# cornell-zhang/GraphLily

Measured on AMD Instinct MI355X. Metric: SpMV effective HBM GB/s (fp32 (+,x), orkut stand-in); BFS GTEPS in `bfs`, higher is better.
Workload: dtype f32; 1 GPU; float32 (+,x) SpMV on orkut stand-in (R-MAT seed 6, n=3072512, nnz=211703799), row-sharded x1; graph=orkut, n=3072512, nnz=211703799

## Files before the change

graphlily_amd/capi.py:

```python
import ctypes
import os

import numpy as np

_HERE = os.path.dirname(os.path.abspath(__file__))
LIB_PATH = os.environ.get("GRAPHLILY_HIP_LIB") or os.path.join(_HERE, "lib", "libgraphlily_hip.so")

GL_OP_MULADD, GL_OP_ANDOR, GL_OP_ADDMIN = 0, 1, 2
GL_NOMASK, GL_MASK_WRITETOZERO, GL_MASK_WRITETOONE = 0, 1, 2

GL_OK = 0
GL_ERR_INVALID_ARG = -1
GL_ERR_HIP = -2
GL_ERR_NOT_INITIALIZED = -3
GL_ERR_IO = -4

IDX_VAL = np.dtype([("index", np.uint32), ("val", np.float32)])

EXPORTS = [
    "gl_init", "gl_host_bind_near_device", "gl_device_count", "gl_set_stream", "gl_reset_stream", "gl_sync", "gl_last_error", "gl_version",
    "gl_graph_begin_capture", "gl_graph_end_capture", "gl_graph_launch", "gl_graph_destroy",
    "gl_bfs_bits_begin", "gl_bfs_bits_push_step", "gl_bfs_bits_pull_step",     "gl_bfs_bits_shard_step", "gl_bfs_bits_shard_finish", "gl_dist_all_gather_bits_tally",
    "gl_buf_d2h_async", "gl_levels_pack", "gl_host_levels_unpack", "gl_host_unpack_threads", "gl_buf_d2h_levels", "gl_sync_levels_unpack",
    "gl_levels_stream_bytes", "gl_levels_stream_arm", "gl_levels_pack_stream", "gl_sync_levels_unpack_stream",
# ... 227 lines not shown
    def __array_finalize__(self, obj):
        if obj is not None and getattr(obj, "_owner", None) is not None:
            self._owner = obj._owner



class DeviceBuffer:

    def __init__(self, nbytes=0, ptr=None, keepalive=None):
        self.nbytes = int(nbytes)
        self._owned = ptr is None
        self.keepalive = keepalive
        if self._owned:
            p = ctypes.c_void_p(0)
            check(lib().gl_buf_alloc(ctypes.byref(p), self.nbytes))
            self.ptr = p.value or 0
        else:
            self.ptr = int(ptr)

    @classmethod
    def from_host(cls, arr):
        arr = np.ascontiguousarray(arr)
        b = cls(arr.nbytes)
        b.write(arr)
        return b

    @classmethod
    def from_torch(cls, t):
        return cls(t.numel() * t.element_size(), ptr=t.data_ptr(), keepalive=t)

    def write(self, arr, offset_bytes=0):
        arr = np.ascontiguousarray(arr)
        assert offset_bytes + arr.nbytes <= self.nbytes, "host array larger than device buffer"
        check(lib().gl_buf_h2d(ctypes.c_void_p(self.ptr + offset_bytes), _np_ptr(arr), arr.nbytes))

    def read(self, dtype, count=None, offset_bytes=0, out=None):
        dtype = np.dtype(dtype)
        if count is None:
            count = (self.nbytes - offset_bytes) // dtype.itemsize
        if out is None:
            out = np.empty(count, dtype=dtype)
        else:
            assert out.dtype == dtype and out.shape[0] >= count and out.flags["C_CONTIGUOUS"]
            out = out[:count]
        assert offset_bytes + out.nbytes <= self.nbytes
        check(lib().gl_buf_d2h(_np_ptr(out), ctypes.c_void_p(self.ptr + offset_bytes), out.nbytes))
        return out

    def read_async(self, out, offset_bytes=0):
        assert out.flags["C_CONTIGUOUS"] and offset_bytes + out.nbytes <= self.nbytes
        check(lib().gl_buf_d2h_async(_np_ptr(out), ctypes.c_void_p(self.ptr + offset_bytes), out.nbytes))
        return out

    def free(self):
        if self._owned and self.ptr:
            lib().gl_buf_free(ctypes.c_void_p(self.ptr))
        self.ptr = 0

    def __del__(self):
        try:
            self.free()
        except Exception:
            pass


def copy_d2d(dst, src, nbytes):
    assert nbytes <= dst.nbytes and nbytes <= src.nbytes
    check(lib().gl_buf_d2d(ctypes.c_void_p(dst.ptr), ctypes.c_void_p(src.ptr), int(nbytes)))


def _p(buf):
    return ctypes.c_void_p(buf.ptr if buf is not None else 0)


GL_PAGERANK_MAX_SLOTS = 65536

GL_PLAN_NO_MULADD = 1
GL_PLAN_BOOLEAN = 2
GL_PLAN_KEEP_VALUES = 4
GL_VAL_FLOAT, GL_VAL_UNSIGNED, GL_VAL_UFIXED_32_8 = 0, 1, 2
GL_PLAN_HOST_FORMAT = 8
GL_PLAN_DEVICE_FORMAT = 16
GL_PLAN_REFERENCE_ORDER = 32
PLAN_ARRAYS = {"entries": 0, "bases": 1, "units": 2, "hub_rows": 3, "spans": 4, "hot": 5, "hot_hdr": 6, "present": 7}
GL_ERR_UNSUPPORTED = -5


class _PlanDesc(ctypes.Structure):
    _fields_ = [("nnz", ctypes.c_uint64), ("device_bytes", ctypes.c_uint64), ("groups", ctypes.c_uint64), ("hot_nnz", ctypes.c_uint64),
                ("num_units", ctypes.c_uint32), ("blocks", ctypes.c_uint32), ("segments", ctypes.c_uint32), ("max_block_rows", ctypes.c_uint32),
                ("hot_columns", ctypes.c_uint32), ("packed_columns", ctypes.c_uint32),
                ("layout", ctypes.c_int), ("mix", ctypes.c_int), ("helper", ctypes.c_int)]


class SpMVPlan:
    def __init__(self, num_rows, num_cols, indptr, indices, data, row_begin=0, row_end=None, flags=0):
        self.indptr = np.ascontiguousarray(indptr, dtype=np.uint32)
        self.indices = np.ascontiguousarray(indices, dtype=np.uint32)
        self.data = np.ascontiguousarray(data, dtype=np.float32)
        row_end = num_rows if row_end is None else row_end
        h = ctypes.c_void_p(0)
        check(lib().gl_spmv_plan_create_ex(ctypes.byref(h), num_rows, num_cols, _np_ptr(self.indptr),
                                           _np_ptr(self.indices), _np_ptr(self.data), row_begin, row_end,
                                           int(flags)))
        self.flags = int(flags)
        self.handle = h.value
        self.num_rows, self.num_cols, self.row_begin, self.row_end = num_rows, num_cols, row_begin, row_end
        self.indptr = self.indices = self.data = None

    def info(self):
        cached = getattr(self, "_info", None)
        if cached is not None:
            return dict(cached)
        d = _PlanDesc()
        check(lib().gl_spmv_plan_describe(ctypes.c_void_p(self.handle), ctypes.byref(d)))
        finite = ctypes.c_int(0)
        check(lib().gl_spmv_plan_values_finite(ctypes.c_void_p(self.handle), ctypes.byref(finite)))
        self._info = {"finite_values": bool(finite.value), "helper": ("gather", "spread", "self-hot", "none")[d.helper], "packed_columns": d.packed_columns,
                      "nnz": d.nnz, "device_bytes": d.device_bytes, "num_units": d.num_units, "blocks": d.blocks,
                      "segments": d.segments, "max_block_rows": d.max_block_rows, "groups": d.groups,
                      "hot_columns": d.hot_columns, "hot_nnz": d.hot_nnz, "mix": d.mix,
                      "layout": ("general", "pattern", "boolean", "reference-order")[d.layout]}
        return dict(self._info)

    def run(self, x, mask, y, op, zero, mask_type):
        check(lib().gl_spmv_run(ctypes.c_void_p(self.handle), _p(x), _p(mask), _p(y), int(op), float(zero),
                                int(mask_type)))

    def run_typed(self, x, mask, y, op, zero_bits, mask_type, val_type):
        check(lib().gl_spmv_run_typed(ctypes.c_void_p(self.handle), _p(x), _p(mask), _p(y), int(op), int(zero_bits), int(mask_type),
                                      int(val_type)))

    def chain(self, on):
        active = ctypes.c_int(0)
        check(lib().gl_spmv_plan_chain(ctypes.c_void_p(self.handle), 1 if on else 0, ctypes.byref(active)))
        return bool(active.value)

    def export(self, name):
        n = ctypes.c_size_t(0)
        check(lib().gl_spmv_plan_export(ctypes.c_void_p(self.handle), PLAN_ARRAYS[name], None, 0, ctypes.byref(n)))
        out = np.empty(n.value // 4, dtype=np.uint32)
        check(lib().gl_spmv_plan_export(ctypes.c_void_p(self.handle), PLAN_ARRAYS[name], _np_ptr(out), out.nbytes, ctypes.byref(n)))
        return out

    def bits_words(self):
        v = ctypes.c_uint64(0)
        check(lib().gl_spmv_plan_bits_words(ctypes.c_void_p(self.handle), ctypes.byref(v)))
        return v.value

    def bfs_pull_step(self, bits_in, bits_out, distance, level):
        check(lib().gl_bfs_pull_step(ctypes.c_void_p(self.handle), _p(bits_in), _p(bits_out), _p(distance), float(level)))

    def bfs_parents(self, distance, parent, orphans=None):
        check(lib().gl_bfs_parents(ctypes.c_void_p(self.handle), _p(distance), _p(parent), _p(orphans)))

    def bfs_parents_entries(self, distance, parent):
        v = ctypes.c_uint64(0)
        check(lib().gl_bfs_parents_entries(ctypes.c_void_p(self.handle), _p(distance), _p(parent), ctypes.byref(v)))
        return v.value

    def cc_labels(self, labels, count=None):
        check(lib().gl_cc_labels(ctypes.c_void_p(self.handle), _p(labels), _p(count)))

    def cc_hook(self, parent):
        check(lib().gl_cc_hook(ctypes.c_void_p(self.handle), _p(parent)))

    def tc_count(self, total, per_vertex=None):
# ... 516 lines not shown
```

graphlily_amd/csrc/gl_format.hip:

```cpp
#include <cstring>

#include "gl_spmv_plan.h"

#include <rocprim/rocprim.hpp>

namespace gl {

struct DevCsr {
    uint32_t row_begin = 0, row_end = 0;
    uint64_t nz0 = 0, nnz = 0;
    uint32_t *d_indptr = nullptr;
    uint32_t *d_indices = nullptr;
    uint32_t *d_data = nullptr;
    uint32_t *d_colbits = nullptr;
    uint32_t num_cols_colbits = 0;
};

namespace {

struct DevMem {
    void *p = nullptr;
    ~DevMem() {
        if (p) (void)hipFree(p);
    }
    int alloc(size_t bytes) {
        GL_HIP(hipMalloc(&p, bytes ? bytes : 16));
        return GL_OK;
    }
    template <typename T>
    T *as() const { return static_cast<T *>(p); }
};

constexpr uint32_t kFmtThreads = 256;

inline unsigned wave_grid(uint64_t rows) {
    const uint64_t want = (rows + 3) / 4;
    const uint64_t cap = (uint64_t)ctx().num_cus * 32u;
    return (unsigned)std::max<uint64_t>(1, std::min(want, cap));
}

__global__ __launch_bounds__(kFmtThreads) void fmt_degree_kernel(const uint32_t *__restrict__ indices, uint64_t nnz, uint32_t num_cols,
                                                                 uint32_t *__restrict__ deg, uint32_t *__restrict__ bad) {
    for (uint64_t i = (uint64_t)blockIdx.x * kFmtThreads + threadIdx.x; i < nnz; i += (uint64_t)gridDim.x * kFmtThreads) {
        const uint32_t c = indices[i];
        if (c < num_cols) atomicAdd(&deg[c], 1u);
        else *bad = 1u;
    }
}

__global__ __launch_bounds__(kFmtThreads) void fmt_non_finite_kernel(const uint32_t *__restrict__ data, uint64_t nnz, uint32_t *__restrict__ found) {
    bool any = false;
    for (uint64_t i = (uint64_t)blockIdx.x * kFmtThreads + threadIdx.x; i < nnz; i += (uint64_t)gridDim.x * kFmtThreads)
        any |= (data[i] & 0x7f800000u) == 0x7f800000u;
    if (any) *found = 1u;
}

__global__ __launch_bounds__(kFmtThreads) void fmt_pattern_pass1_kernel(const uint32_t *__restrict__ indptr, const uint32_t *__restrict__ indices,
                                                                        const uint32_t *__restrict__ data, uint32_t row_begin, uint32_t rows,
                                                                        uint64_t nz0, uint32_t num_cols, uint32_t *__restrict__ colbits) {
    const uint32_t lane = threadIdx.x & 63u, nwaves = gridDim.x * (kFmtThreads / 64u);
    for (uint32_t row = blockIdx.x * (kFmtThreads / 64u) + (threadIdx.x >> 6); row < rows; row += nwaves) {
        const uint32_t r = row_begin + row;
        const uint64_t s = indptr[row] - nz0, e = indptr[row + 1] - nz0;
        for (uint64_t i = s + lane; i < e; i += 64u) {
            const uint32_t c = indices[i];
            if (c < num_cols && c != r) {
                const uint32_t bits = data[i];
                if (colbits[c] != bits) colbits[c] = bits;
            }
        }
    }
}

__global__ __launch_bounds__(kFmtThreads) void fmt_pattern_pass2_kernel(const uint32_t *__restrict__ indptr, const uint32_t *__restrict__ indices,
                                                                        const uint32_t *__restrict__ data, uint32_t row_begin, uint32_t rows,
                                                                        uint64_t nz0, uint32_t num_cols, const uint32_t *__restrict__ colbits,
                                                                        uint32_t *__restrict__ diag_has, uint32_t *__restrict__ diag_val,
                                                                        uint32_t *__restrict__ mismatch, unsigned long long *__restrict__ exceptions) {
    const uint32_t lane = threadIdx.x & 63u, nwaves = gridDim.x * (kFmtThreads / 64u);
    for (uint32_t row = blockIdx.x * (kFmtThreads / 64u) + (threadIdx.x >> 6); row < rows; row += nwaves) {
        const uint32_t r = row_begin + row;
        const uint64_t s = indptr[row] - nz0, e = indptr[row + 1] - nz0;
        uint32_t nexc = 0;
        bool bad = false;
        for (uint64_t i = s + lane; i < e; i += 64u) {
            const uint32_t c = indices[i], bits = data[i];
            if (c >= num_cols) { bad = true; continue; }
            if (colbits[c] == bits) continue;
            if (c != r) { bad = true; continue; }
            nexc++;
            diag_val[row] = bits;
            atomicOr(&diag_has[row >> 5], 1u << (row & 31u));
        }
#pragma unroll
        for (int d = 32; d > 0; d >>= 1) nexc += __shfl_down(nexc, d);
        nexc = __shfl(nexc, 0);
        if (nexc > 1u) bad = true;
        if (__ballot(bad) != 0ull && lane == 0) *mismatch = 1u;
        if (nexc && lane == 0) atomicAdd(exceptions, (unsigned long long)nexc);
    }
}

template <typename K>
__global__ __launch_bounds__(kFmtThreads) void fmt_keys_kernel(const uint32_t *__restrict__ indptr, const uint32_t *__restrict__ indices,
                                                               const uint32_t *__restrict__ data, uint32_t row_begin, uint32_t rows, uint64_t nz0,
                                                               uint32_t num_cols, const uint32_t *__restrict__ bstart, uint32_t nblocks,
                                                               const uint32_t *__restrict__ colmap, const uint32_t *__restrict__ colbits,
                                                               uint32_t cb, uint32_t bb, K *__restrict__ keys, uint2 *__restrict__ payload,
                                                               bool drop_hot) {
    const uint32_t lane = threadIdx.x & 63u, nwaves = gridDim.x * (kFmtThreads / 64u);
    const K drop = (K)1 << (bb + cb + 1u);
    for (uint32_t row = blockIdx.x * (kFmtThreads / 64u) + (threadIdx.x >> 6); row < rows; row += nwaves) {
        const uint32_t r = row_begin + row;
        const uint64_t s = indptr[row] - nz0, e = indptr[row + 1] - nz0;
        if (s == e) continue;
        uint32_t lo = 0, hi = nblocks - 1u;
        while (lo < hi) {
            const uint32_t mid = (lo + hi + 1u) >> 1;
            if (bstart[mid] <= r) lo = mid; else hi = mid - 1u;
        }
        const uint32_t b = lo, r0 = bstart[b];
        for (uint64_t i = s + lane; i < e; i += 64u) {
            const uint32_t c = indices[i], v = data[i];
            K key;
            if (c >= num_cols || (colbits && c == r && v != colbits[c])) {
                key = drop;
            } else {
                const uint32_t cm = colmap[c];
                key = ((K)b << (cb + 1u)) | ((K)(cm >> 31) << cb) | (K)(cm & 0x7fffffffu);
                if (drop_hot && (cm >> 31)) key = drop;
            }
            keys[i] = key;
            payload[i] = make_uint2(r - r0, v);
        }
    }
}

template <typename K>
__global__ __launch_bounds__(kFmtThreads) void fmt_bounds_kernel(const K *__restrict__ keys, uint64_t n, uint32_t count, uint32_t cb,
                                                                 unsigned long long *__restrict__ off) {
    const uint32_t i = blockIdx.x * kFmtThreads + threadIdx.x;
    if (i >= count) return;
    const K target = (K)i << cb;
    uint64_t lo = 0, hi = n;
    while (lo < hi) {
        const uint64_t mid = (lo + hi) >> 1;
        if (keys[mid] < target) lo = mid + 1; else hi = mid;
    }
    off[i] = lo;
}

struct UnitDesc {
    uint32_t cold_begin, cold_end, hot_begin, hot_end;
    uint32_t goff, r0, nrows_direct, hub_off;
    uint32_t nhub, seg, hot_e0, present_off;
    uint32_t nhot_groups, pad0, pad1, pad2;
};

template <typename K>
__global__ __launch_bounds__(kFmtThreads) void fmt_gap_kernel(const K *__restrict__ keys, uint64_t n, uint32_t cb, uint32_t bb, uint32_t *__restrict__ dummies) {
    const K cmask = ((K)1 << cb) - 1, drop = (K)1 << (bb + cb + 1u);
    for (uint64_t i = (uint64_t)blockIdx.x * kFmtThreads + threadIdx.x; i < n; i += (uint64_t)gridDim.x * kFmtThreads) {
        uint32_t d = 0u;
        if (i > 0) {
            const K k = keys[i], kp = keys[i - 1];
            if ((k >> cb) == (kp >> cb) && ((k >> cb) & (K)1) == 0 && !(k & drop)) {
                const uint32_t gap = (uint32_t)(k & cmask) - (uint32_t)(kp & cmask);
                if (gap > kColdMaxDelta) d = (gap - 1u) / kColdMaxDelta;
            }
        }
        dummies[i] = d;
    }
}
__global__ __launch_bounds__(kFmtThreads) void fmt_gap_unit_starts_kernel(const UnitDesc *__restrict__ units, uint32_t nunits, uint32_t *__restrict__ dummies) {
    const uint32_t u = blockIdx.x * kFmtThreads + threadIdx.x;
    if (u < nunits && units[u].cold_begin < units[u].cold_end) dummies[units[u].cold_begin] = 0u;
}

template <typename K, bool PATTERN>
__global__ __launch_bounds__(kThreads) void fmt_emit_cold_kernel(const K *__restrict__ keys, const uint2 *__restrict__ payload,
                                                                 const uint32_t *__restrict__ ahead, const UnitDesc *__restrict__ units,
                                                                 const uint32_t *__restrict__ hub_rows, uint32_t cb,
                                                                 unsigned char *__restrict__ cold, uint32_t *__restrict__ bases,
                                                                 uint4 *__restrict__ plan_units) {
    __shared__ uint8_t hub_of[kMaxBlockRows + 1];
    constexpr uint32_t G = PATTERN ? kColdGroupsPattern : kColdGroupsGeneral;
    constexpr uint32_t EB = PATTERN ? kColdElemBytesPattern : kColdElemBytesGeneral;
    const UnitDesc u = units[blockIdx.x];
    const uint32_t nrows = u.nrows_direct & 0xffffu;
    const K cmask = ((K)1 << cb) - 1;
    if (u.nhub) {
        for (uint32_t i = threadIdx.x; i < nrows; i += kThreads) hub_of[i] = 0xffu;
        __syncthreads();
        if (threadIdx.x < u.nhub) hub_of[hub_rows[u.hub_off + threadIdx.x]] = (uint8_t)threadIdx.x;
        __syncthreads();
    }
    const uint32_t pad0 = nrows + kHubSlots * u.nhub;
    auto put = [&](uint32_t q, uint32_t idx, uint32_t delta, uint32_t slot, uint32_t val) {
        const uint32_t g = u.goff + q / 64u, lane = q % 64u, k = g % G;
        unsigned char *el = cold + (size_t)(g / G) * EB;
        if (!lane) {
            bases[g] = idx;
            delta = 0u;
        }
        if (PATTERN) {
            reinterpret_cast<uint16_t *>(el)[lane * 8u + k] = (uint16_t)slot;
            el[1024u + lane * 8u + k] = (unsigned char)delta;
        } else {
            reinterpret_cast<uint16_t *>(el)[lane * 4u + k] = (uint16_t)slot;
            el[512u + lane * 4u + k] = (unsigned char)delta;
            reinterpret_cast<uint32_t *>(el + 768u)[lane * 4u + k] = val;
        }
    };
    const uint32_t m = u.cold_end - u.cold_begin;
    const uint32_t a0 = m ? ahead[u.cold_begin] : 0u;
    for (uint32_t j = threadIdx.x; j < m; j += kThreads) {
        const uint32_t i = u.cold_begin + j;
        const uint32_t idx = (uint32_t)(keys[i] & cmask);
        const uint32_t before = ahead[i] - a0;
        const uint32_t mine = j ? ahead[i] - ahead[i - 1u] : 0u;
        const uint32_t prev = j ? (uint32_t)(keys[i - 1u] & cmask) : idx;
        const uint32_t q = j + before;
        for (uint32_t t = 1; t <= mine; t++) {
            const uint32_t qd = q - mine + (t - 1u);
            put(qd, prev + kColdMaxDelta * t, kColdMaxDelta, pad0 + qd % 64u, 0u);
        }
        const uint2 pl = payload[i];
        uint32_t slot = pl.x;
        if (u.nhub) {
            const uint32_t hb = hub_of[pl.x];
            if (hb != 0xffu) slot = nrows + kHubSlots * hb + ((q % 64u) & (kHubSlots - 1u));
        }
        put(q, idx, idx - (prev + kColdMaxDelta * mine), slot, pl.y);
    }
    const uint32_t total = m ? m + (ahead[u.cold_end - 1u] - a0) : 0u;
    const uint32_t qend = (total + 64u * G - 1u) / (64u * G) * (64u * G);
    const uint32_t last = m ? (uint32_t)(keys[u.cold_end - 1u] & cmask) : 0u;
    for (uint32_t q = total + threadIdx.x; q < qend; q += kThreads)
        put(q, (q / 64u == (total - 1u) / 64u && total) ? last : 0u, 0u, pad0 + q % 64u, 0u);
    if (threadIdx.x == 0) {
        plan_units[3u * blockIdx.x] = make_uint4(u.goff, qend / 64u, u.r0, u.nrows_direct);
        plan_units[3u * blockIdx.x + 1u] = make_uint4(u.hub_off, u.nhub, u.nhot_groups, u.seg);
    }
}

template <typename K>
__global__ __launch_bounds__(kFmtThreads) void fmt_run_flags_kernel(const K *__restrict__ keys, uint64_t n, uint32_t cb, uint32_t *__restrict__ flags) {
    for (uint64_t i = (uint64_t)blockIdx.x * kFmtThreads + threadIdx.x; i < n; i += (uint64_t)gridDim.x * kFmtThreads) {
        const K k = keys[i];
        flags[i] = (((k >> cb) & (K)1) != 0 && (i == 0 || keys[i - 1] != k)) ? 1u : 0u;
    }
}
__global__ __launch_bounds__(kFmtThreads) void fmt_run_unit_starts_kernel(const UnitDesc *__restrict__ units, uint32_t nunits, uint32_t *__restrict__ flags) {
    const uint32_t u = blockIdx.x * kFmtThreads + threadIdx.x;
    if (u < nunits && units[u].hot_begin < units[u].hot_end) flags[units[u].hot_begin] = 1u;
}

template <typename K>
__global__ __launch_bounds__(kThreads) void fmt_emit_hot_kernel(const K *__restrict__ keys, const uint2 *__restrict__ payload,
                                                                const uint32_t *__restrict__ runs, const UnitDesc *__restrict__ units,
                                                                const uint32_t *__restrict__ hub_rows, uint32_t cb,
                                                                unsigned char *__restrict__ hot, uint32_t *__restrict__ hot_hdr,
                                                                uint16_t *__restrict__ present, uint4 *__restrict__ plan_units) {
    __shared__ uint8_t hub_of[kMaxBlockRows + 1];
    constexpr uint32_t HG = kHotGroupsGeneral;
    constexpr uint32_t EB = kHotElemBytesGeneral;
    const UnitDesc u = units[blockIdx.x];
    const uint32_t nrows = u.nrows_direct & 0xffffu;
    const uint32_t lane = threadIdx.x & 63u, wave = threadIdx.x >> 6;
    const K cmask = ((K)1 << cb) - 1;
    if (u.nhub) {
        for (uint32_t i = threadIdx.x; i < nrows; i += kThreads) hub_of[i] = 0xffu;
        __syncthreads();
        if (threadIdx.x < u.nhub) hub_of[hub_rows[u.hub_off + threadIdx.x]] = (uint8_t)threadIdx.x;
        __syncthreads();
    }
    const uint32_t m = u.hot_end - u.hot_begin, nraw = (m + 63u) / 64u;
    const uint32_t s0 = m ? runs[u.hot_begin] : 0u;
    const uint32_t pad_slot = nrows + kHubSlots * u.nhub + lane;
    for (uint32_t hg = wave; hg < u.nhot_groups; hg += kWaves) {
        const uint32_t st = u.hot_begin + hg * 64u, cnt = hg < nraw ? min(64u, u.hot_end - st) : 0u;
        const size_t e = (size_t)u.hot_e0 + hg / HG;
        const uint32_t k = hg % HG;
        uint32_t local = 0u;
        bool start = false;
        if (lane >= cnt) {
            reinterpret_cast<uint16_t *>(hot + e * EB)[lane * 4u + k] = (uint16_t)pad_slot;
        } else {
            const uint32_t i = st + lane, si = runs[i];
            local = si - s0;
            start = i == u.hot_begin || runs[i - 1u] != si;
            const uint32_t slot_col = (uint32_t)(keys[i] & cmask);
            if (start) present[u.present_off + local] = (uint16_t)slot_col;
            const uint2 pl = payload[i];
            uint32_t slot = pl.x;
            if (u.nhub) {
                const uint32_t hb = hub_of[pl.x];
                if (hb != 0xffu) slot = nrows + kHubSlots * hb + (lane & (kHubSlots - 1u));
            }
            unsigned char *el = hot + e * EB;
            reinterpret_cast<uint16_t *>(el)[lane * 4u + k] = (uint16_t)slot;
            reinterpret_cast<uint32_t *>(el + 512)[lane * 4u + k] = pl.y;
        }
        const unsigned long long mask = __ballot(start && lane >= 1u) >> 1;
        const uint32_t base = __shfl(local, 0);
        if (lane == 0) {
            uint32_t *hd = hot_hdr + e * (kHotHdrWordsPerGroup * HG);
            hd[2u * k] = (uint32_t)mask;
            hd[2u * k + 1u] = (uint32_t)(mask >> 32);
            hd[2u * HG + k] = base;
        }
    }
    if (threadIdx.x == 0)
        plan_units[3u * blockIdx.x + 2u] = make_uint4(u.hot_e0, u.present_off, m ? runs[u.hot_end - 1u] - s0 + 1u : 0u, 0u);
}

__global__ __launch_bounds__(kFmtThreads) void fmt_hot_row_counts_kernel(const uint32_t *__restrict__ indptr, const uint32_t *__restrict__ indices,
                                                                         const uint32_t *__restrict__ data, uint32_t row_begin, uint32_t rows,
                                                                         uint64_t nz0, uint32_t num_cols, const uint32_t *__restrict__ colmap,
                                                                         const uint32_t *__restrict__ colbits, unsigned long long *__restrict__ counts) {
    const uint32_t lane = threadIdx.x & 63u, nwaves = gridDim.x * (kFmtThreads / 64u);
    for (uint32_t row = blockIdx.x * (kFmtThreads / 64u) + (threadIdx.x >> 6); row < rows; row += nwaves) {
        const uint32_t r = row_begin + row;
        const uint64_t s = indptr[row] - nz0, e = indptr[row + 1] - nz0;
        uint32_t h = 0;
        for (uint64_t i = s + lane; i < e; i += 64u) {
            const uint32_t c = indices[i];
            if (c >= num_cols || (colbits && c == r && data[i] != colbits[c])) continue;
            h += colmap[c] >> 31;
        }
#pragma unroll
        for (int d = 32; d > 0; d >>= 1) h += __shfl_xor(h, d);
        if (lane == 0) counts[row] = ((unsigned long long)h << 32) | (unsigned long long)((h + kHotRecEntries - 1u) / kHotRecEntries);
    }
}
__global__ __launch_bounds__(kFmtThreads) void fmt_hot_block_starts_kernel(const unsigned long long *__restrict__ incl, const uint32_t *__restrict__ bstart,
                                                                           uint32_t nblocks, uint32_t row_begin, unsigned long long *__restrict__ out) {
    const uint32_t b = blockIdx.x * kFmtThreads + threadIdx.x;
    if (b > nblocks) return;
    const uint32_t row = bstart[b] - row_begin;
    out[b] = row ? incl[row - 1u] : 0ull;
}
__global__ __launch_bounds__(kThreads) void fmt_fill_hot_rows_kernel(const UnitDesc *__restrict__ units, unsigned char *__restrict__ hot, uint32_t nhot_table,
                                                                     uint4 *__restrict__ plan_units) {
    const UnitDesc u = units[blockIdx.x];
    const uint32_t nrows = u.nrows_direct & 0xffffu, pad0 = nrows + kHubSlots * u.nhub;
    const uint32_t ident = nhot_table | (nhot_table << 16);
    for (uint32_t i = threadIdx.x; i < u.nhot_groups * 64u; i += kThreads) {
        uint4 rec = make_uint4(ident, ident, ident, (nhot_table & 0xffffu) | ((pad0 + (i & 63u)) << 16));
        reinterpret_cast<uint4 *>(hot + (size_t)u.hot_e0 * kHotElemBytesRows)[i] = rec;
    }
    if (threadIdx.x == 0) plan_units[3u * blockIdx.x + 2u] = make_uint4(u.hot_e0, 0u, nhot_table, 0u);
}
__global__ __launch_bounds__(kFmtThreads) void fmt_emit_hot_rows_kernel(const uint32_t *__restrict__ indptr, const uint32_t *__restrict__ indices,
                                                                        const uint32_t *__restrict__ data, uint32_t row_begin, uint32_t rows,
                                                                        uint64_t nz0, uint32_t num_cols, const uint32_t *__restrict__ colmap,
                                                                        const uint32_t *__restrict__ colbits, const uint32_t *__restrict__ bstart,
                                                                        uint32_t nblocks, const unsigned long long *__restrict__ incl,
                                                                        const unsigned long long *__restrict__ block_start,
                                                                        const uint32_t *__restrict__ seg, const uint32_t *__restrict__ unit_of,
                                                                        const UnitDesc *__restrict__ units, const uint32_t *__restrict__ hub_rows,
                                                                        unsigned char *__restrict__ hot) {
    const uint32_t lane = threadIdx.x & 63u, nwaves = gridDim.x * (kFmtThreads / 64u);
    for (uint32_t row = blockIdx.x * (kFmtThreads / 64u) + (threadIdx.x >> 6); row < rows; row += nwaves) {
        const uint32_t r = row_begin + row;
        const uint64_t s = indptr[row] - nz0, e = indptr[row + 1] - nz0;
        const unsigned long long before = row ? incl[row - 1u] : 0ull, mine = incl[row] - before;
        if ((uint32_t)(mine >> 32) == 0u) continue;
        uint32_t lo = 0, hi = nblocks - 1u;
        while (lo < hi) {
            const uint32_t mid = (lo + hi + 1u) >> 1;
            if (bstart[mid] <= r) lo = mid; else hi = mid - 1u;
        }
        const uint32_t b = lo, row_local = r - bstart[b];
        const uint64_t M = (uint32_t)block_start[b + 1u] - (uint32_t)block_start[b];
        const uint64_t rec0 = (uint32_t)before - (uint32_t)block_start[b];
        const uint32_t S = seg[b];
        const UnitDesc u0 = units[unit_of[b]];
        const uint32_t nrows = u0.nrows_direct & 0xffffu;
        int hub = -1;
        for (uint32_t k = 0; k < u0.nhub; k++)
            if (hub_rows[u0.hub_off + k] == row_local) hub = (int)k;
        uint32_t running = 0;
        for (uint64_t i0 = s; i0 < e; i0 += 64u) {
            const uint64_t i = i0 + lane;
            uint32_t cm = 0;
            bool is_hot = false;
            if (i < e) {
                const uint32_t c = indices[i];
                if (c < num_cols && !(colbits && c == r && data[i] != colbits[c])) {
                    cm = colmap[c];
                    is_hot = (cm >> 31) != 0u;
                }
            }
            const unsigned long long bal = __ballot(is_hot);
            const uint32_t rank = running + (uint32_t)__popcll(bal & ((1ull << lane) - 1ull));
            running += (uint32_t)__popcll(bal);
            if (!is_hot) continue;
            const uint64_t j = rec0 + rank / kHotRecEntries;
            const uint32_t f = rank % kHotRecEntries;
            uint64_t guess = S == 1u ? 0u : (j * S + S - 1u) / M;
            uint32_t sg = (uint32_t)(guess < S ? guess : S - 1u);
            while (M * sg / S > j) sg--;
            while (M * (sg + 1u) / S <= j) sg++;
            const UnitDesc u = units[unit_of[(size_t)sg * nblocks + b]];
            const uint32_t jj = (uint32_t)(j - M * sg / S), chunk = u.nhot_groups, l = jj / chunk, el = jj % chunk;
            uint16_t *rec = reinterpret_cast<uint16_t *>(hot + (size_t)(u.hot_e0 + el) * kHotElemBytesRows) + l * 8u;
            rec[f] = (uint16_t)(cm & 0x7fffffffu);
            if (f == 0u) rec[7] = (uint16_t)(hub < 0 ? row_local : nrows + kHubSlots * (uint32_t)hub + (l & (kHubSlots - 1u)));
        }
    }
}

__global__ void fmt_fill_hot_kernel(uint32_t *hot, size_t elems, uint32_t words_per_elem, uint32_t slot_words) {
    for (size_t i = (size_t)blockIdx.x * 256u + threadIdx.x; i < elems * words_per_elem; i += (size_t)gridDim.x * 256u)
        hot[i] = (i % words_per_elem) < slot_words ? (kRowPad | (kRowPad << 16)) : 0u;
}

__global__ void fmt_fill_u32_kernel(uint32_t *dst, uint32_t v, size_t n) {
    for (size_t i = (size_t)blockIdx.x * 256u + threadIdx.x; i < n; i += (size_t)gridDim.x * 256u) dst[i] = v;
}

template <typename K>
int sort_pairs(K *kin, K *kout, uint2 *vin, uint2 *vout, uint64_t n, uint32_t bits, hipStream_t s) {
    size_t tmp_bytes = 0;
    GL_HIP(rocprim::radix_sort_pairs(nullptr, tmp_bytes, kin, kout, vin, vout, (size_t)n, 0u, bits, s));
    DevMem tmp;
    int rc = tmp.alloc(tmp_bytes);
    if (rc != GL_OK) return rc;
    GL_HIP(rocprim::radix_sort_pairs(tmp.p, tmp_bytes, kin, kout, vin, vout, (size_t)n, 0u, bits, s));
    GL_HIP(hipStreamSynchronize(s));
    return GL_OK;
}

template <typename K>
int sort_keys_values_u32(K *kin, K *kout, uint32_t *vin, uint32_t *vout, uint64_t n, uint32_t bits, hipStream_t s) {
    size_t tmp_bytes = 0;
    GL_HIP(rocprim::radix_sort_pairs(nullptr, tmp_bytes, kin, kout, vin, vout, (size_t)n, 0u, bits, s));
    DevMem tmp;
    int rc = tmp.alloc(tmp_bytes);
    if (rc != GL_OK) return rc;
    GL_HIP(rocprim::radix_sort_pairs(tmp.p, tmp_bytes, kin, kout, vin, vout, (size_t)n, 0u, bits, s));
    GL_HIP(hipStreamSynchronize(s));
    return GL_OK;
}

inline uint32_t bits_for(uint64_t count) {
    uint32_t b = 1;
    while ((1ull << b) < count) b++;
    return b;
}

template <typename K>
int emit_general_typed(DevCsr *c, const EmitGeneral &e, gl_spmv_plan p, std::vector<uint32_t> &hub_count, uint64_t *hot_nnz,
                       uint32_t cb, uint32_t bb) {
    hipStream_t s = ctx().stream;
    const BlockPlan &bp = *e.bp;
    const uint32_t nblocks = bp.nblocks, nunits = bp.nunits;
    const uint32_t rows = c->row_end - c->row_begin;
    const uint64_t nnz = c->nnz;
    const bool hot_rows = e.pattern;
    const uint32_t hot_groups = hot_rows ? 1u : kHotGroupsGeneral;
    const uint32_t hot_elem_bytes = hot_rows ? kHotElemBytesRows : kHotElemBytesGeneral;

    DevMem d_bstart, d_colmap, d_keys, d_keys2, d_pl, d_pl2, d_off;
    int rc;
    if ((rc = d_bstart.alloc((size_t)(nblocks + 1) * 4u)) != GL_OK || (rc = d_colmap.alloc((size_t)e.num_cols * 4u)) != GL_OK ||
        (rc = d_keys.alloc(nnz * sizeof(K))) != GL_OK || (rc = d_keys2.alloc(nnz * sizeof(K))) != GL_OK ||
        (rc = d_pl.alloc(nnz * 8u)) != GL_OK || (rc = d_pl2.alloc(nnz * 8u)) != GL_OK ||
        (rc = d_off.alloc((size_t)(2u * nblocks + 1u) * 8u)) != GL_OK)
        return rc;
    GL_HIP(hipMemcpyAsync(d_bstart.p, bp.bstart.data(), (size_t)(nblocks + 1) * 4u, hipMemcpyHostToDevice, s));
    GL_HIP(hipMemcpyAsync(d_colmap.p, e.colmap, (size_t)e.num_cols * 4u, hipMemcpyHostToDevice, s));
    fmt_keys_kernel<K><<<wave_grid(rows), kFmtThreads, 0, s>>>(c->d_indptr, c->d_indices, c->d_data, c->row_begin, rows, c->nz0, e.num_cols,
                                                               d_bstart.as<uint32_t>(), nblocks, d_colmap.as<uint32_t>(),
                                                               e.diag_mode ? c->d_colbits : nullptr, cb, bb, d_keys.as<K>(), d_pl.as<uint2>(), hot_rows);
    GL_LAUNCH_CHECK();
    if ((rc = sort_pairs<K>(d_keys.as<K>(), d_keys2.as<K>(), d_pl.as<uint2>(), d_pl2.as<uint2>(), nnz, bb + cb + 2u, s)) != GL_OK) return rc;
    (void)hipFree(d_keys.p); d_keys.p = nullptr;
    (void)hipFree(d_pl.p); d_pl.p = nullptr;
    const K *keys = d_keys2.as<K>();
    const uint2 *payload = d_pl2.as<uint2>();
    fmt_bounds_kernel<K><<<cdiv(2u * nblocks + 1u, kFmtThreads), kFmtThreads, 0, s>>>(keys, nnz, 2u * nblocks + 1u, cb, d_off.as<unsigned long long>());
    GL_LAUNCH_CHECK();
    std::vector<unsigned long long> off(2u * nblocks + 1u);
    GL_HIP(hipMemcpyAsync(off.data(), d_off.p, off.size() * 8u, hipMemcpyDeviceToHost, s));
    GL_HIP(hipStreamSynchronize(s));

    std::vector<uint32_t> hub_rows((size_t)nblocks * kMaxHubRows, 0u);
    hub_count.assign(nblocks, 0u);
    std::vector<UnitDesc> units(nunits);
    uint64_t hn = 0;
    std::vector<uint64_t> mcs(nblocks), mhs(nblocks), mrec(nblocks, 0);
    for (uint32_t b = 0; b < nblocks; b++) mcs[b] = off[2 * b + 1] - off[2 * b], mhs[b] = off[2 * b + 2] - off[2 * b + 1];
    DevMem d_rowcnt, d_rowincl, d_blockstart;
    if (hot_rows) {
        DevMem d_tmp;
        if ((rc = d_rowcnt.alloc((size_t)std::max(rows, 1u) * 8u)) != GL_OK || (rc = d_rowincl.alloc((size_t)std::max(rows, 1u) * 8u)) != GL_OK ||
            (rc = d_blockstart.alloc((size_t)(nblocks + 1u) * 8u)) != GL_OK)
            return rc;
        fmt_hot_row_counts_kernel<<<wave_grid(rows), kFmtThreads, 0, s>>>(c->d_indptr, c->d_indices, c->d_data, c->row_begin, rows, c->nz0, e.num_cols,
                                                                           d_colmap.as<uint32_t>(), e.diag_mode ? c->d_colbits : nullptr,
                                                                           d_rowcnt.as<unsigned long long>());
        GL_LAUNCH_CHECK();
        size_t tmp_bytes = 0;
        GL_HIP(rocprim::inclusive_scan(nullptr, tmp_bytes, d_rowcnt.as<unsigned long long>(), d_rowincl.as<unsigned long long>(), (size_t)rows,
                                       rocprim::plus<unsigned long long>(), s));
        if ((rc = d_tmp.alloc(tmp_bytes)) != GL_OK) return rc;
        GL_HIP(rocprim::inclusive_scan(d_tmp.p, tmp_bytes, d_rowcnt.as<unsigned long long>(), d_rowincl.as<unsigned long long>(), (size_t)rows,
                                       rocprim::plus<unsigned long long>(), s));
        fmt_hot_block_starts_kernel<<<cdiv(nblocks + 1u, kFmtThreads), kFmtThreads, 0, s>>>(d_rowincl.as<unsigned long long>(), d_bstart.as<uint32_t>(), nblocks,
                                                                                            c->row_begin, d_blockstart.as<unsigned long long>());
        GL_LAUNCH_CHECK();
        std::vector<unsigned long long> bs(nblocks + 1u);
        GL_HIP(hipMemcpyAsync(bs.data(), d_blockstart.p, bs.size() * 8u, hipMemcpyDeviceToHost, s));
        GL_HIP(hipStreamSynchronize(s));
        for (uint32_t b = 0; b < nblocks; b++) {
            mhs[b] = (bs[b + 1] >> 32) - (bs[b] >> 32);
            mrec[b] = (uint64_t)((uint32_t)bs[b + 1] - (uint32_t)bs[b]);
        }
    }
    const UnitLayout ul = layout_units(bp, mcs, mhs, e.dummy_max, hot_groups, e.nhot_table, hot_rows ? &mrec : nullptr);
    const uint64_t total_groups = ul.cold_goff[nunits], hot_elems = ul.hot_e0[nunits];
    if (total_groups >= 0xffffffffull || hot_elems >= 0xffffffffull || ul.present_off[nunits] >= 0xffffffffull)
        return set_error(GL_ERR_UNSUPPORTED, "plan creation: more than 2^32 - 1 groups in a shard");
    for (uint32_t b = 0; b < nblocks; b++) {
        const uint32_t r0 = bp.bstart[b], r1 = bp.bstart[b + 1];
        const uint64_t mc = mcs[b], mh = mhs[b], m = mc + mh;
        hn += mh;
        const uint64_t thr = std::max<uint64_t>(256, m / (uint64_t)e.hub_div);
        uint32_t nh = 0;
        for (uint32_t r = r0; r < r1 && nh < kMaxHubRows; r++) {
            uint64_t cnt = (uint64_t)e.h_indptr[r + 1] - e.h_indptr[r];
            if (cnt < thr) continue;
            if (e.diag_mode) {
                const uint32_t lr = r - c->row_begin;
                if ((e.diag_has[lr >> 5] >> (lr & 31u)) & 1u) cnt--;
            }
            if (cnt >= thr) hub_rows[(size_t)b * kMaxHubRows + nh++] = r - r0;
        }
        hub_count[b] = nh;
        const uint32_t S = bp.seg[b];
        for (uint32_t sg = 0; sg < S; sg++) {
            UnitDesc &u = units[bp.unit_of[sg][b]];
            u.cold_begin = (uint32_t)(off[2 * b] + mc * sg / S);
            u.cold_end = (uint32_t)(off[2 * b] + mc * (sg + 1) / S);
            u.hot_begin = hot_rows ? 0u : (uint32_t)(off[2 * b + 1] + mh * sg / S);
            u.hot_end = hot_rows ? 0u : (uint32_t)(off[2 * b + 1] + mh * (sg + 1) / S);
            const size_t ui = bp.unit_of[sg][b];
            u.goff = (uint32_t)ul.cold_goff[ui];
            u.r0 = r0;
            u.nrows_direct = (r1 - r0) | (bp.all_direct ? 0x80000000u : 0u);
            u.hub_off = (uint32_t)((size_t)b * kMaxHubRows);
            u.nhub = nh;
            u.seg = sg;
            u.hot_e0 = (uint32_t)ul.hot_e0[ui];
            u.present_off = (uint32_t)ul.present_off[ui];
            u.nhot_groups = (uint32_t)(ul.hot_e0[ui + 1] - ul.hot_e0[ui]) * hot_groups;
            u.pad0 = u.pad1 = u.pad2 = 0u;
        }
    }
    *hot_nnz = hn;

    const uint32_t cold_groups = e.pattern ? kColdGroupsPattern : kColdGroupsGeneral;
    const size_t cold_elem_bytes = e.pattern ? kColdElemBytesPattern : kColdElemBytesGeneral;
    const size_t entry_bytes = (size_t)(total_groups / cold_groups) * cold_elem_bytes;
    const size_t tail_bytes = cold_elem_bytes;
    const size_t n_bases = (size_t)total_groups + 8u;
    GL_HIP(hipMalloc((void **)&p->d_entries, entry_bytes + tail_bytes));
    GL_HIP(hipMalloc((void **)&p->d_bases, n_bases * 4u));
    GL_HIP(hipMalloc((void **)&p->d_units, (size_t)nunits * 3u * sizeof(uint4) + 16u));
    GL_HIP(hipMalloc((void **)&p->d_hub_rows, hub_rows.size() * 4u + 16u));
    const size_t hot_bytes = (size_t)(hot_elems + 1u) * hot_elem_bytes;
    const size_t hdr_bytes = hot_rows ? (size_t)32 : (size_t)(hot_elems + 1u) * kHotHdrWordsPerGroup * hot_groups * 4u;
    const size_t present_bytes = (size_t)std::max<uint64_t>(ul.present_off[nunits], 2u) * 2u;
    GL_HIP(hipMalloc((void **)&p->d_hot, hot_bytes));
    GL_HIP(hipMalloc((void **)&p->d_hot_hdr, hdr_bytes));
    GL_HIP(hipMalloc((void **)&p->d_present, present_bytes));
    p->device_bytes += entry_bytes + tail_bytes + n_bases * 4u + (size_t)nunits * 3u * sizeof(uint4) + hub_rows.size() * 4u +
                       hot_bytes + hdr_bytes + present_bytes;
    p->b_entries = entry_bytes + tail_bytes;
    p->b_bases = n_bases * 4u;
    p->b_units = (size_t)nunits * 3u * sizeof(uint4);
    p->b_hub_rows = hub_rows.size() * 4u;
    p->b_hot = hot_bytes;
    p->b_hot_hdr = hdr_bytes;
    p->b_present = present_bytes;
    p->ngroups = total_groups;
    p->nhot_elems = hot_elems;
    GL_HIP(hipMemsetAsync(p->d_hot_hdr, 0, hdr_bytes, s));
    GL_HIP(hipMemsetAsync(p->d_present, 0, present_bytes, s));
    GL_HIP(hipMemsetAsync(p->d_hot, 0, hot_bytes, s));
    fmt_fill_hot_kernel<<<1, 256, 0, s>>>(reinterpret_cast<uint32_t *>(p->d_hot + (size_t)hot_elems * hot_elem_bytes), 1u, hot_elem_bytes / 4u,
                                          hot_rows ? hot_elem_bytes / 4u : hot_groups * 64u * 2u / 4u);
    GL_LAUNCH_CHECK();
    GL_HIP(hipMemsetAsync(p->d_entries, 0, entry_bytes + tail_bytes, s));
    GL_HIP(hipMemsetAsync(p->d_bases, 0, n_bases * 4u, s));
    GL_HIP(hipMemcpyAsync(p->d_hub_rows, hub_rows.data(), hub_rows.size() * 4u, hipMemcpyHostToDevice, s));

    DevMem d_units;
    if ((rc = d_units.alloc((size_t)nunits * sizeof(UnitDesc))) != GL_OK) return rc;
    GL_HIP(hipMemcpyAsync(d_units.p, units.data(), (size_t)nunits * sizeof(UnitDesc), hipMemcpyHostToDevice, s));
    {
        DevMem d_gap, d_ahead, d_tmp;
        if ((rc = d_gap.alloc(std::max<uint64_t>(nnz, 1u) * 4u)) != GL_OK || (rc = d_ahead.alloc(std::max<uint64_t>(nnz, 1u) * 4u)) != GL_OK) return rc;
        fmt_gap_kernel<K><<<std::min<unsigned>(cdiv(std::max<uint64_t>(nnz, 1u), kFmtThreads), (unsigned)ctx().num_cus * 32u), kFmtThreads, 0, s>>>(
            keys, nnz, cb, bb, d_gap.as<uint32_t>());
        GL_LAUNCH_CHECK();
        fmt_gap_unit_starts_kernel<<<cdiv(nunits, kFmtThreads), kFmtThreads, 0, s>>>(d_units.as<UnitDesc>(), nunits, d_gap.as<uint32_t>());
        GL_LAUNCH_CHECK();
        size_t tmp_bytes = 0;
        GL_HIP(rocprim::inclusive_scan(nullptr, tmp_bytes, d_gap.as<uint32_t>(), d_ahead.as<uint32_t>(), (size_t)nnz, rocprim::plus<uint32_t>(), s));
        if ((rc = d_tmp.alloc(tmp_bytes)) != GL_OK) return rc;
        GL_HIP(rocprim::inclusive_scan(d_tmp.p, tmp_bytes, d_gap.as<uint32_t>(), d_ahead.as<uint32_t>(), (size_t)nnz, rocprim::plus<uint32_t>(), s));
        if (e.pattern)
            fmt_emit_cold_kernel<K, true><<<nunits, kThreads, 0, s>>>(keys, payload, d_ahead.as<uint32_t>(), d_units.as<UnitDesc>(), p->d_hub_rows, cb,
                                                                      reinterpret_cast<unsigned char *>(p->d_entries), p->d_bases, p->d_units);
        else
            fmt_emit_cold_kernel<K, false><<<nunits, kThreads, 0, s>>>(keys, payload, d_ahead.as<uint32_t>(), d_units.as<UnitDesc>(), p->d_hub_rows, cb,
                                                                       reinterpret_cast<unsigned char *>(p->d_entries), p->d_bases, p->d_units);
        GL_LAUNCH_CHECK();
        GL_HIP(hipStreamSynchronize(s));
    }
    if (hot_rows) {
        DevMem d_seg, d_unit_of;
        std::vector<uint32_t> unit_of_flat((size_t)bp.Smax * nblocks, 0xffffffffu);
        for (uint32_t sgm = 0; sgm < bp.Smax; sgm++)
            for (uint32_t b = 0; b < nblocks; b++) unit_of_flat[(size_t)sgm * nblocks + b] = bp.unit_of[sgm][b];
        if ((rc = d_seg.alloc((size_t)nblocks * 4u)) != GL_OK || (rc = d_unit_of.alloc(unit_of_flat.size() * 4u)) != GL_OK) return rc;
        GL_HIP(hipMemcpyAsync(d_seg.p, bp.seg.data(), (size_t)nblocks * 4u, hipMemcpyHostToDevice, s));
        GL_HIP(hipMemcpyAsync(d_unit_of.p, unit_of_flat.data(), unit_of_flat.size() * 4u, hipMemcpyHostToDevice, s));
        fmt_fill_hot_rows_kernel<<<nunits, kThreads, 0, s>>>(d_units.as<UnitDesc>(), p->d_hot, e.nhot_table, p->d_units);
        GL_LAUNCH_CHECK();
        if (e.nhot_table) {
            fmt_emit_hot_rows_kernel<<<wave_grid(rows), kFmtThreads, 0, s>>>(c->d_indptr, c->d_indices, c->d_data, c->row_begin, rows, c->nz0, e.num_cols,
                                                                              d_colmap.as<uint32_t>(), e.diag_mode ? c->d_colbits : nullptr,
                                                                              d_bstart.as<uint32_t>(), nblocks, d_rowincl.as<unsigned long long>(),
                                                                              d_blockstart.as<unsigned long long>(), d_seg.as<uint32_t>(),
                                                                              d_unit_of.as<uint32_t>(), d_units.as<UnitDesc>(), p->d_hub_rows, p->d_hot);
            GL_LAUNCH_CHECK();
        }
        GL_HIP(hipStreamSynchronize(s));
        p->nhot_lds = e.nhot_table ? e.nhot_table + 64u : 0u;
        return GL_OK;
    }
    {
        DevMem d_flags, d_runs, d_tmp;
        if ((rc = d_flags.alloc(std::max<uint64_t>(nnz, 1u) * 4u)) != GL_OK || (rc = d_runs.alloc(std::max<uint64_t>(nnz, 1u) * 4u)) != GL_OK) return rc;
        fmt_run_flags_kernel<K><<<std::min<unsigned>(cdiv(std::max<uint64_t>(nnz, 1u), kFmtThreads), (unsigned)ctx().num_cus * 32u), kFmtThreads, 0, s>>>(
            keys, nnz, cb, d_flags.as<uint32_t>());
        GL_LAUNCH_CHECK();
        fmt_run_unit_starts_kernel<<<cdiv(nunits, kFmtThreads), kFmtThreads, 0, s>>>(d_units.as<UnitDesc>(), nunits, d_flags.as<uint32_t>());
        GL_LAUNCH_CHECK();
        size_t tmp_bytes = 0;
        GL_HIP(rocprim::inclusive_scan(nullptr, tmp_bytes, d_flags.as<uint32_t>(), d_runs.as<uint32_t>(), (size_t)nnz, rocprim::plus<uint32_t>(), s));
        if ((rc = d_tmp.alloc(tmp_bytes)) != GL_OK) return rc;
        GL_HIP(rocprim::inclusive_scan(d_tmp.p, tmp_bytes, d_flags.as<uint32_t>(), d_runs.as<uint32_t>(), (size_t)nnz, rocprim::plus<uint32_t>(), s));
        fmt_emit_hot_kernel<K><<<nunits, kThreads, 0, s>>>(keys, payload, d_runs.as<uint32_t>(), d_units.as<UnitDesc>(), p->d_hub_rows, cb,
                                                           p->d_hot, p->d_hot_hdr, p->d_present, p->d_units);
        GL_LAUNCH_CHECK();
        GL_HIP(hipStreamSynchronize(s));
    }
    std::vector<uint4> pu((size_t)nunits * 3u);
    GL_HIP(hipMemcpy(pu.data(), p->d_units, pu.size() * sizeof(uint4), hipMemcpyDeviceToHost));
    uint32_t max_present = 0;
    for (uint32_t u = 0; u < nunits; u++) max_present = std::max(max_present, pu[3u * u + 2u].z);
    p->nhot_lds = (max_present + 63u) / 64u * 64u;
    return GL_OK;
}


template <typename K>
__global__ __launch_bounds__(kFmtThreads) void fmt_bool_keys_kernel(const uint32_t *__restrict__ indptr, const uint32_t *__restrict__ indices,
                                                                    const uint32_t *__restrict__ data, uint32_t row_begin, uint32_t rows, uint64_t nz0,
                                                                    uint32_t num_cols, const uint32_t *__restrict__ bstart, uint32_t nblocks,
                                                                    uint32_t cb, uint32_t bb, K *__restrict__ keys, uint32_t *__restrict__ payload,
                                                                    uint32_t *__restrict__ row_count, uint32_t *__restrict__ bad) {
    const uint32_t lane = threadIdx.x & 63u, nwaves = gridDim.x * (kFmtThreads / 64u);
    const K drop = (K)1 << (bb + cb);
    for (uint32_t row = blockIdx.x * (kFmtThreads / 64u) + (threadIdx.x >> 6); row < rows; row += nwaves) {
        const uint32_t r = row_begin + row;
        const uint64_t s = indptr[row] - nz0, e = indptr[row + 1] - nz0;
        uint32_t kept = 0;
        if (s != e) {
            uint32_t lo = 0, hi = nblocks - 1u;
            while (lo < hi) {
                const uint32_t mid = (lo + hi + 1u) >> 1;
                if (bstart[mid] <= r) lo = mid; else hi = mid - 1u;
            }
            const uint32_t b = lo, r0 = bstart[b];
            for (uint64_t i = s + lane; i < e; i += 64u) {
                const uint32_t c = indices[i];
                if (c >= num_cols) *bad = 1u;
                const bool keep = c < num_cols && __uint_as_float(data[i]) != 0.0f;
                keys[i] = keep ? (((K)b << cb) | (K)c) : drop;
                payload[i] = r - r0;
                kept += keep ? 1u : 0u;
            }
#pragma unroll
            for (int d = 32; d > 0; d >>= 1) kept += __shfl_down(kept, d);
        }
        if (lane == 0) row_count[row] = kept;
    }
}

struct BoolUnitDesc {
    uint32_t begin, end;
    uint32_t tmp_goff, tmp_soff;
    uint32_t goff, soff;
    uint32_t r0, nrows_direct, hub_off, nhub;
    uint32_t pad0, pad1;
};

__device__ __forceinline__ uint32_t bool_phase(uint32_t col) { return col / kBoolPhaseCols; }

template <typename K>
__global__ __launch_bounds__(64) void fmt_bool_group_kernel(const K *__restrict__ keys, const BoolUnitDesc *__restrict__ units, uint32_t cb,
                                                            uint32_t *__restrict__ gstart, uint32_t *__restrict__ gcount,
                                                            uint2 *__restrict__ counts) {
    const BoolUnitDesc u = units[blockIdx.x];
    const uint32_t lane = threadIdx.x;
    const K cmask = ((K)1 << cb) - 1;
// ... 288 lines not shown
    c->d_indptr = nullptr;
    c->d_indices = nullptr;
    return GL_OK;
}

void devcsr_release(DevCsr *c) {
    if (!c) return;
    (void)hipFree(c->d_indptr);
    (void)hipFree(c->d_indices);
    (void)hipFree(c->d_data);
    (void)hipFree(c->d_colbits);
    delete c;
}

int fmt_column_degrees(DevCsr *c, uint32_t num_cols, std::vector<uint32_t> &deg, int *bad_col) {
    hipStream_t s = ctx().stream;
    DevMem d_deg, d_bad;
    int rc;
    if ((rc = d_deg.alloc((size_t)num_cols * 4u)) != GL_OK || (rc = d_bad.alloc(16)) != GL_OK) return rc;
    GL_HIP(hipMemsetAsync(d_deg.p, 0, (size_t)num_cols * 4u, s));
    GL_HIP(hipMemsetAsync(d_bad.p, 0, 16, s));
    const unsigned grid = (unsigned)std::max<uint64_t>(1, std::min<uint64_t>((c->nnz + kFmtThreads - 1) / kFmtThreads, (uint64_t)ctx().num_cus * 16u));
    fmt_degree_kernel<<<grid, kFmtThreads, 0, s>>>(c->d_indices, c->nnz, num_cols, d_deg.as<uint32_t>(), d_bad.as<uint32_t>());
    GL_LAUNCH_CHECK();
    deg.resize(num_cols);
    uint32_t bad = 0;
    GL_HIP(hipMemcpyAsync(deg.data(), d_deg.p, (size_t)num_cols * 4u, hipMemcpyDeviceToHost, s));
    GL_HIP(d2h_word_sync(&bad, d_bad.p, s));
    *bad_col = bad ? 1 : 0;
    return GL_OK;
}

int fmt_values_finite(DevCsr *c, int *finite) {
    hipStream_t s = ctx().stream;
    DevMem d_found;
    int rc;
    if ((rc = d_found.alloc(16)) != GL_OK) return rc;
    GL_HIP(hipMemsetAsync(d_found.p, 0, 16, s));
    const unsigned grid = (unsigned)std::max<uint64_t>(1, std::min<uint64_t>((c->nnz + kFmtThreads - 1) / kFmtThreads, (uint64_t)ctx().num_cus * 16u));
    fmt_non_finite_kernel<<<grid, kFmtThreads, 0, s>>>(c->d_data, c->nnz, d_found.as<uint32_t>());
    GL_LAUNCH_CHECK();
    uint32_t found = 0;
    GL_HIP(d2h_word_sync(&found, d_found.p, s));
    *finite = found ? 0 : 1;
    return GL_OK;
}

int fmt_detect_pattern(DevCsr *c, uint32_t num_cols, std::vector<uint32_t> &colbits, std::vector<uint32_t> &diag_has,
                       std::vector<float> &diag_val, int *mismatch, uint64_t *exceptions) {
    hipStream_t s = ctx().stream;
    const uint32_t rows = c->row_end - c->row_begin;
    const size_t words = ((size_t)rows + 31u) / 32u;
    if (!c->d_colbits) GL_HIP(hipMalloc((void **)&c->d_colbits, (size_t)std::max(num_cols, 1u) * 4u));
    c->num_cols_colbits = num_cols;
    DevMem d_has, d_val, d_flags;
    int rc;
    if ((rc = d_has.alloc(words * 4u)) != GL_OK || (rc = d_val.alloc((size_t)rows * 4u)) != GL_OK || (rc = d_flags.alloc(16)) != GL_OK) return rc;
    GL_HIP(hipMemsetAsync(c->d_colbits, 0, (size_t)num_cols * 4u, s));
    GL_HIP(hipMemsetAsync(d_has.p, 0, words * 4u, s));
    GL_HIP(hipMemsetAsync(d_val.p, 0, (size_t)rows * 4u, s));
    GL_HIP(hipMemsetAsync(d_flags.p, 0, 16, s));
    fmt_pattern_pass1_kernel<<<wave_grid(rows), kFmtThreads, 0, s>>>(c->d_indptr, c->d_indices, c->d_data, c->row_begin, rows, c->nz0, num_cols, c->d_colbits);
    GL_LAUNCH_CHECK();
    fmt_pattern_pass2_kernel<<<wave_grid(rows), kFmtThreads, 0, s>>>(c->d_indptr, c->d_indices, c->d_data, c->row_begin, rows, c->nz0, num_cols,
                                                                  c->d_colbits, d_has.as<uint32_t>(), d_val.as<uint32_t>(), d_flags.as<uint32_t>(),
                                                                  reinterpret_cast<unsigned long long *>(d_flags.as<uint32_t>() + 2));
    GL_LAUNCH_CHECK();
    colbits.resize(num_cols);
    diag_has.resize(words);
    diag_val.resize(rows);
    uint32_t flags[4] = {0, 0, 0, 0};
    GL_HIP(hipMemcpyAsync(colbits.data(), c->d_colbits, (size_t)num_cols * 4u, hipMemcpyDeviceToHost, s));
    if (words) GL_HIP(hipMemcpyAsync(diag_has.data(), d_has.p, words * 4u, hipMemcpyDeviceToHost, s));
    if (rows) GL_HIP(hipMemcpyAsync(diag_val.data(), d_val.p, (size_t)rows * 4u, hipMemcpyDeviceToHost, s));
    GL_HIP(hipMemcpyAsync(flags, d_flags.p, 16, hipMemcpyDeviceToHost, s));
    GL_HIP(hipStreamSynchronize(s));
    *mismatch = flags[0] ? 1 : 0;
    unsigned long long ex;
    memcpy(&ex, &flags[2], 8);
    *exceptions = ex;
    return GL_OK;
}

int fmt_emit_general(DevCsr *c, const EmitGeneral &e, gl_spmv_plan p, std::vector<uint32_t> &hub_count, uint64_t *hot_nnz) {
    const uint32_t cb = bits_for(std::max<uint64_t>(std::max(e.gather_cols, e.nhot_table), 2u));
    const uint32_t bb = bits_for(std::max<uint32_t>(e.bp->nblocks, 2u));
    if (c->nnz >= 0xffffffffull) return set_error(GL_ERR_UNSUPPORTED, "plan creation on the device: more than 2^32 - 1 entries in a shard");
    if (bb + cb + 2u <= 32u) return emit_general_typed<uint32_t>(c, e, p, hub_count, hot_nnz, cb, bb);
    return emit_general_typed<unsigned long long>(c, e, p, hub_count, hot_nnz, cb, bb);
}

namespace {

__global__ __launch_bounds__(kFmtThreads) void fmt_csc_interleave_kernel(const uint32_t *__restrict__ rows, const uint32_t *__restrict__ vals, uint64_t nnz,
                                                                         uint32_t num_rows, uint2 *__restrict__ stream, uint32_t *__restrict__ bad) {
    for (uint64_t i = (uint64_t)blockIdx.x * kFmtThreads + threadIdx.x; i < nnz; i += (uint64_t)gridDim.x * kFmtThreads) {
        const uint32_t r = rows[i];
        if (r >= num_rows) *bad = 1u;
        stream[i] = make_uint2(r, vals[i]);
    }
}

__global__ __launch_bounds__(kFmtThreads) void fmt_csc_count_kernel(const uint32_t *__restrict__ indptr, const uint32_t *__restrict__ rows, uint32_t num_cols,
                                                                    uint32_t num_rows, uint32_t r0, uint32_t r1, uint32_t *__restrict__ cnt,
                                                                    uint32_t *__restrict__ bad) {
    const uint32_t lane = threadIdx.x & 63u, nwaves = gridDim.x * (kFmtThreads / 64u);
    for (uint32_t c = blockIdx.x * (kFmtThreads / 64u) + (threadIdx.x >> 6); c < num_cols; c += nwaves) {
        uint32_t k = 0;
        for (uint64_t i = (uint64_t)indptr[c] + lane; i < indptr[c + 1]; i += 64u) {
            const uint32_t r = rows[i];
            if (r >= num_rows) *bad = 1u;
            k += (r >= r0 && r < r1) ? 1u : 0u;
        }
#pragma unroll
        for (int d = 32; d > 0; d >>= 1) k += __shfl_down(k, d);
        if (lane == 0) cnt[c] = k;
    }
}

__global__ __launch_bounds__(kFmtThreads) void fmt_csc_filter_kernel(const uint32_t *__restrict__ indptr, const uint32_t *__restrict__ rows,
                                                                     const uint32_t *__restrict__ vals, uint32_t num_cols, uint32_t r0, uint32_t r1,
                                                                     const uint32_t *__restrict__ out_ptr, uint2 *__restrict__ stream) {
    const uint32_t lane = threadIdx.x & 63u, nwaves = gridDim.x * (kFmtThreads / 64u);
    for (uint32_t c = blockIdx.x * (kFmtThreads / 64u) + (threadIdx.x >> 6); c < num_cols; c += nwaves) {
        uint32_t at = out_ptr[c];
        const uint64_t e = indptr[c + 1];
        for (uint64_t i0 = indptr[c]; i0 < e; i0 += 64u) {
            const uint64_t i = i0 + lane;
            uint32_t r = 0;
            bool keep = false;
            if (i < e) {
                r = rows[i];
                keep = r >= r0 && r < r1;
            }
            const unsigned long long km = __ballot(keep);
            if (keep) stream[at + (uint32_t)__popcll(km & ((1ull << lane) - 1ull))] = make_uint2(r, vals[i]);
            at += (uint32_t)__popcll(km);
        }
    }
}

__global__ __launch_bounds__(kFmtThreads) void fmt_row_of_kernel(const uint32_t *__restrict__ indptr, uint32_t rows, uint32_t *__restrict__ row_of) {
    const uint32_t lane = threadIdx.x & 63u, nwaves = gridDim.x * (kFmtThreads / 64u);
    for (uint32_t r = blockIdx.x * (kFmtThreads / 64u) + (threadIdx.x >> 6); r < rows; r += nwaves)
        for (uint64_t i = (uint64_t)indptr[r] + lane; i < indptr[r + 1]; i += 64u) row_of[i] = r;
}

__global__ __launch_bounds__(kFmtThreads) void fmt_split_pairs_kernel(const uint2 *__restrict__ pairs, uint64_t nnz, uint32_t *__restrict__ a, uint32_t *__restrict__ b) {
    for (uint64_t i = (uint64_t)blockIdx.x * kFmtThreads + threadIdx.x; i < nnz; i += (uint64_t)gridDim.x * kFmtThreads) {
        const uint2 p = pairs[i];
        a[i] = p.x;
        b[i] = p.y;
    }
}

__global__ __launch_bounds__(kFmtThreads) void fmt_pack_pairs_kernel(const uint32_t *__restrict__ a, const uint32_t *__restrict__ b, uint64_t nnz, uint2 *__restrict__ pairs) {
    for (uint64_t i = (uint64_t)blockIdx.x * kFmtThreads + threadIdx.x; i < nnz; i += (uint64_t)gridDim.x * kFmtThreads) pairs[i] = make_uint2(a[i], b[i]);
}

__global__ __launch_bounds__(kFmtThreads) void fmt_normalize_kernel(const uint32_t *__restrict__ cols, const uint32_t *__restrict__ deg, uint64_t nnz, float *__restrict__ out) {
    for (uint64_t i = (uint64_t)blockIdx.x * kFmtThreads + threadIdx.x; i < nnz; i += (uint64_t)gridDim.x * kFmtThreads)
        out[i] = (float)(1.0 / (double)deg[cols[i]]);
}

inline unsigned flat_grid(uint64_t n) {
    return (unsigned)std::max<uint64_t>(1, std::min<uint64_t>((n + kFmtThreads - 1) / kFmtThreads, (uint64_t)ctx().num_cus * 16u));
}

}

int fmt_spmspv_stream(uint32_t num_rows, uint32_t num_cols, const uint32_t *h_indptr, const uint32_t *h_indices, const float *h_data,
                      uint32_t r0, uint32_t r1, uint32_t **d_indptr_out, uint2 **d_stream_out, std::vector<uint32_t> &indptr_out) {
// ... 196 lines not shown
```

graphlily_amd/csrc/gl_spmv.hip:

```cpp
#include "gl_spmv_plan.h"
#include "gl_tile.h"

namespace gl {

#if defined(GL_UNIT_CLOCKS)
__device__ unsigned long long g_unit_clocks[2 * 4096];
#endif

struct SpmvArgs {
    const unsigned char *entries;
    const uint32_t *bases;
    const uint4 *units;
    const uint32_t *hub_rows;
    const float *hot_x;
    uint32_t nhot;
    uint32_t tile_bytes;
    const unsigned char *hot;
    const uint32_t *hot_hdr;
    const uint16_t *present;
    const float *x;
    const float *mask;
    float *y;
    float zero;
    const float *xg;
    const float *z;
    const float *diag;
    const uint32_t *diag_has;
    const uint32_t *run_flag;
    float *partials;
    uint32_t prow;
    uint32_t row_begin;
    uint32_t tickets;
    const uint32_t *self_hot_cols;
    const uint32_t *chain_map = nullptr;
    const float *chain_colval = nullptr;
    float *chain_packed = nullptr, *chain_hot = nullptr;
};

template <int OP, int MASK>
__device__ __forceinline__ void spmv_unit_epilogue(const SpmvArgs &a, typename Tile<OP>::T *tile, const uint4 d, const uint4 dh) {
    using TL = Tile<OP>;
    using T = typename TL::T;
    const uint32_t row0 = d.z, nrows = d.w & 0xffffu;
    const bool direct = (d.w >> 31) != 0u;
    const uint32_t hub_off = dh.x, nhub = dh.y;
    __syncthreads();
    if (nhub) {
        if (threadIdx.x < nhub) {
            const uint32_t r = a.hub_rows[hub_off + threadIdx.x];
            T acc = tile[r];
#pragma unroll
            for (uint32_t k = 0; k < kHubSlots; k++) acc = TL::comb(acc, tile[nrows + kHubSlots * threadIdx.x + k]);
            tile[r] = acc;
        }
        __syncthreads();
    }

    if (direct) {
        for (uint32_t i = threadIdx.x; i < nrows; i += kThreads) {
            const uint32_t row = row0 + i;
            if (a.diag_has) {
                const uint32_t lr = row - a.row_begin;
                if ((a.diag_has[lr >> 5] >> (lr & 31u)) & 1u)
                    tile[i] = TL::comb(tile[i], TL::lift(Semiring<OP>::mul(a.diag[lr], a.x[row])));
            }
            float out = TL::finish(a.zero, TL::get(tile, i));
            if (MASK != GL_NOMASK) {
                if (!mask_allows_zero<MASK, OP>(a.mask[row])) out = 0.0f;
            }
            a.y[row] = out;
            if (MASK == GL_NOMASK && a.chain_map) {
                const uint32_t m = a.chain_map[row];
                if (m != 0xffffffffu) {
                    const float nx = a.chain_colval ? Semiring<OP>::mul(a.chain_colval[row], out) : out;
                    if (m >> 31) a.chain_hot[m & 0x7fffffffu] = nx;
                    else a.chain_packed[m] = nx;
                }
            }
        }
    } else {
        float *plane = a.partials + (size_t)dh.w * a.prow + (row0 - a.row_begin);
        for (uint32_t i = threadIdx.x; i < nrows; i += kThreads) plane[i] = TL::get(tile, i);
    }
}


enum { kLayWide = 1, kLayQuad = 3, kLayWideKeep = 4, kLayQuadKeep = 5 };

__device__ __forceinline__ uint32_t load_stream_nt4(const uint32_t *p) {
#ifdef GL_STREAM_PLAIN
    return *p;
#else
    return __builtin_nontemporal_load(p);
#endif
}

__device__ __forceinline__ uint32_t wave_scan_pairs(uint32_t v) {
    v += (uint32_t)__builtin_amdgcn_update_dpp(0, (int)v, 0x111, 0xf, 0xf, true);
    v += (uint32_t)__builtin_amdgcn_update_dpp(0, (int)v, 0x112, 0xf, 0xf, true);
    v += (uint32_t)__builtin_amdgcn_update_dpp(0, (int)v, 0x114, 0xf, 0xf, true);
    v += (uint32_t)__builtin_amdgcn_update_dpp(0, (int)v, 0x118, 0xf, 0xf, true);
    v += (uint32_t)__builtin_amdgcn_update_dpp(0, (int)v, 0x142, 0xa, 0xf, false);
    v += (uint32_t)__builtin_amdgcn_update_dpp(0, (int)v, 0x143, 0xc, 0xf, false);
    return v;
}

template <int H>
__device__ __forceinline__ uint32_t half_shl(uint32_t w, uint32_t sh) {
    uint32_t r;
    if (H == 0) asm("v_lshlrev_b32_sdwa %0, %1, %2 dst_sel:DWORD dst_unused:UNUSED_PAD src0_sel:DWORD src1_sel:WORD_0" : "=v"(r) : "v"(sh), "v"(w));
    else asm("v_lshlrev_b32_sdwa %0, %1, %2 dst_sel:DWORD dst_unused:UNUSED_PAD src0_sel:DWORD src1_sel:WORD_1" : "=v"(r) : "v"(sh), "v"(w));
    return r;
}
template <int H>
__device__ __forceinline__ uint32_t half_add(uint32_t w, uint32_t scalar) {
    uint32_t r;
    if (H == 0) asm("v_add_u32_sdwa %0, %1, %2 dst_sel:DWORD dst_unused:UNUSED_PAD src0_sel:WORD_0 src1_sel:DWORD" : "=v"(r) : "v"(w), "s"(scalar));
    else asm("v_add_u32_sdwa %0, %1, %2 dst_sel:DWORD dst_unused:UNUSED_PAD src0_sel:WORD_1 src1_sel:DWORD" : "=v"(r) : "v"(w), "s"(scalar));
    return r;
}

template <int L>
struct Lay;

template <>
struct Lay<kLayWide> {
    static constexpr int G = (int)kColdGroupsGeneral;
    static constexpr bool kValues = true;
    static constexpr bool kHotRows = false;
    struct E {
        uint2 slots;
        uint32_t deltas;
        uint4 vals;
    };
    template <bool KEEP>
    __device__ static E load_cold(const unsigned char *cold, size_t e, uint32_t lane) {
        const unsigned char *p = cold + e * kColdElemBytesGeneral;
        E c;
        c.slots = KEEP ? load_stream_keep(reinterpret_cast<const uint2 *>(p) + lane) : load_stream_nt(reinterpret_cast<const uint2 *>(p) + lane);
        c.deltas = KEEP ? reinterpret_cast<const uint32_t *>(p + 512)[lane] : load_stream_nt4(reinterpret_cast<const uint32_t *>(p + 512) + lane);
        c.vals = KEEP ? load_stream_keep16(reinterpret_cast<const uint4 *>(p + 768) + lane) : load_stream_nt16(reinterpret_cast<const uint4 *>(p + 768) + lane);
        return c;
    }
    __device__ static E load(const unsigned char *cold, size_t e, uint32_t lane) { return load_cold<false>(cold, e, lane); }
    __device__ static void offsets(const E &c, uint32_t (&pk)[G / 2]) {
        pk[0] = wave_scan_pairs((c.deltas << 2) & 0x03fc03fcu), pk[1] = wave_scan_pairs((c.deltas >> 6) & 0x03fc03fcu);
    }
    __device__ static uint32_t gather_off(const uint32_t (&pk)[G / 2], int k, uint32_t base4) {
        return (k >> 1) ? half_add<1>(pk[k & 1], base4) : half_add<0>(pk[k & 1], base4);
    }
    __device__ static uint32_t slot_w(const E &c, int k) { return k < 2 ? c.slots.x : c.slots.y; }
    __device__ static uint32_t slot(const E &c, int k) {
        const uint32_t w = k < 2 ? c.slots.x : c.slots.y;
        return (k & 1) ? w >> 16 : w & 0xffffu;
    }
    __device__ static float val(const E &c, int k) { return __uint_as_float(k == 0 ? c.vals.x : k == 1 ? c.vals.y : k == 2 ? c.vals.z : c.vals.w); }
    struct H {
        uint2 rows;
        uint4 vals;
    };
    static constexpr int HG = (int)kHotGroupsGeneral;
    __device__ static H load_hot(const unsigned char *hot, size_t e, uint32_t lane) {
        const unsigned char *p = hot + e * kHotElemBytesGeneral;
        H h;
        h.rows = load_stream_nt(reinterpret_cast<const uint2 *>(p) + lane);
// ... 190 lines not shown
                                                                : half_shl<0>(LY::hot_slot_w(r.eh[u], k), kTileShift<OP>));
                if (LY::kValues) TL::acc(at, 0u, LY::hot_val(r.eh[u], k), hv[k]);
                else TL::accz(at, 0u, hv[k]);
#endif
            }
        }
    }
#pragma unroll
    for (int u = 0; u < UC; u++) {
        if (r.ic + u * kWaves < sg.nc) {
#pragma unroll
            for (int k = 0; k < G; k++) {
#ifdef GL_ABLATE_ACC
                asm volatile("" ::"v"(LY::slot(r.ec[u], k)), "v"(LY::val(r.ec[u], k)), "v"(xc[u][k]));
#else
                typename TL::T *at = slot_ptr<OP>(tile, (k & 1) ? half_shl<1>(LY::slot_w(r.ec[u], k), kTileShift<OP>)
                                                                : half_shl<0>(LY::slot_w(r.ec[u], k), kTileShift<OP>));
                if (LY::kValues) TL::acc(at, 0u, LY::val(r.ec[u], k), xc[u][k]);
                else TL::accz(at, 0u, xc[u][k]);
#endif
            }
        }
    }
}

template <int OP, int L, int UC, int UH>
__device__ __forceinline__ uint32_t spmv_phase(const SpmvArgs &a, typename Tile<OP>::T *tile, const float *hot_x, const float *xsrc,
                                               const StreamGeom &sg, uint32_t lane, uint32_t it, uint32_t n, uint32_t *next_slot) {
    if (it >= n) return it;
    auto cold_of = [](uint32_t i) { return i / kWaves * (kWaves * UC) + i % kWaves; };
    auto hot_of = [](uint32_t i) { return i / kWaves * (kWaves * UH) + i % kWaves; };
    constexpr bool PIPE = Lay<L>::kValues;
    if (!PIPE) {
        while (it < n) {
            SlotRegs<L, UC, UH> r;
            slot_load<L, UC, UH>(a, sg, lane, cold_of(it), hot_of(it), r);
            uint32_t ticket = 0;
            if (a.tickets && lane == 0) ticket = __hip_atomic_fetch_add(next_slot, 1u, __ATOMIC_RELAXED, __HIP_MEMORY_SCOPE_WORKGROUP);
            float xc[UC > 0 ? UC : 1][Lay<L>::G];
            slot_gather<L, UC, UH>(xsrc, r, xc);
            slot_accumulate<OP, L, UC, UH>(tile, hot_x, sg, r, xc);
            it = a.tickets ? __builtin_amdgcn_readfirstlane(ticket) : it + kWaves;
        }
        return it;
    }
    SlotRegs<L, UC, UH> cur;
    slot_load<L, UC, UH>(a, sg, lane, cold_of(it), hot_of(it), cur);
    while (true) {
        uint32_t ticket = 0;
        if (a.tickets && lane == 0) ticket = __hip_atomic_fetch_add(next_slot, 1u, __ATOMIC_RELAXED, __HIP_MEMORY_SCOPE_WORKGROUP);
        float xc[UC > 0 ? UC : 1][Lay<L>::G];
        slot_gather<L, UC, UH>(xsrc, cur, xc);
        __builtin_amdgcn_sched_barrier(0);
        const uint32_t nxt = a.tickets ? __builtin_amdgcn_readfirstlane(ticket) : it + kWaves;
        SlotRegs<L, UC, UH> nx;
        slot_load<L, UC, UH>(a, sg, lane, cold_of(nxt), hot_of(nxt), nx);
        __builtin_amdgcn_sched_barrier(0);
        slot_accumulate<OP, L, UC, UH>(tile, hot_x, sg, cur, xc);
        it = nxt;
        if (it >= n) break;
        cur = nx;
    }
    return it;
}

template <int OP, int MASK, int L, int UC, int UH>
__global__ __launch_bounds__(kThreads) void spmv_rbcs_kernel(SpmvArgs a) {
    using TL = Tile<OP>;
    using T = typename TL::T;
    using LY = Lay<L>;
    constexpr int G = LY::G, HG = LY::HG;
    extern __shared__ __attribute__((aligned(16))) unsigned char lds_raw[];
    T *tile = reinterpret_cast<T *>(__builtin_assume_aligned(lds_raw, 16));
    if ((uint32_t)(uintptr_t)((__attribute__((address_space(3))) unsigned char *)lds_raw) != 0u) __builtin_trap();
    float *hot_x = reinterpret_cast<float *>(__builtin_assume_aligned(lds_raw + a.tile_bytes, 16));

    if (a.run_flag && *a.run_flag == 0u) return;
#if defined(GL_UNIT_CLOCKS)
    const unsigned long long unit_t0 = wall_clock64();
#endif
    const uint32_t unit = __builtin_amdgcn_readfirstlane(blockIdx.x);
    const uint4 d = load_const(a.units + 3u * unit), dh = load_const(a.units + 3u * unit + 1u);
    const uint4 dp = load_const(a.units + 3u * unit + 2u);
    const uint32_t g0 = d.x, ncold = d.y, nrows = d.w & 0xffffu;
    const uint32_t nhub = dh.y, nhotg = dh.z;
    const uint32_t nslots = nrows + kHubSlots * nhub;
    const uint32_t lane = threadIdx.x & 63u;
    const uint32_t wave = __builtin_amdgcn_readfirstlane(threadIdx.x >> 6);

    uint32_t &next_iter = *reinterpret_cast<uint32_t *>(lds_raw + a.tile_bytes + (size_t)a.nhot * 4u);
    if (threadIdx.x == 0) next_iter = kWaves;
    if (UH > 0 && LY::kHotRows) {
        for (uint32_t i = threadIdx.x; i < dp.z; i += kThreads) hot_x[i] = a.hot_x[i];
        if (threadIdx.x < 64u) hot_x[dp.z + threadIdx.x] = TL::zident();
    } else if (UH > 0) {
        const uint16_t *pres = a.present + dp.y;
        if (a.self_hot_cols) {
            for (uint32_t i = threadIdx.x; i < dp.z; i += kThreads) hot_x[i] = a.x[a.self_hot_cols[pres[i]]];
        } else {
            for (uint32_t i = threadIdx.x; i < dp.z; i += kThreads) hot_x[i] = a.hot_x[pres[i]];
        }
    }
    for (uint32_t i = threadIdx.x; i < nslots + kPadSlots; i += kThreads) tile[i] = TL::ident();
    __syncthreads();

    const float *xsrc = LY::kValues ? a.xg : a.z;
    StreamGeom sg;
    sg.g0 = g0;
    sg.c0 = g0 / G, sg.nc = ncold / G, sg.h0 = dp.x, sg.nh = nhotg / HG;
    sg.nc_last = max(sg.nc, 1u) - 1u, sg.nh_last = max(sg.nh, 1u) - 1u;
    const uint32_t rc = (sg.nc + kWaves * UC - 1) / (kWaves * UC), rh = UH > 0 ? (sg.nh + kWaves * UH - 1) / (kWaves * UH) : 0u;
    const uint32_t n_both = min(rc, rh) * kWaves, n_all = max(rc, rh) * kWaves;
    uint32_t it = wave;
    it = spmv_phase<OP, L, UC, UH>(a, tile, hot_x, xsrc, sg, lane, it, n_both, &next_iter);
    if (rc > rh) it = spmv_phase<OP, L, UC, 0>(a, tile, hot_x, xsrc, sg, lane, it, n_all, &next_iter);
    else if (UH > 0) it = spmv_phase<OP, L, 0, UH>(a, tile, hot_x, xsrc, sg, lane, it, n_all, &next_iter);
    spmv_unit_epilogue<OP, MASK>(a, tile, d, dh);
#if defined(GL_UNIT_CLOCKS)
    asm volatile("s_waitcnt vmcnt(0)" ::: "memory");
    __syncthreads();
    if (threadIdx.x == 0 && unit < 4096u) {
        g_unit_clocks[2u * unit] = unit_t0;
        g_unit_clocks[2u * unit + 1u] = wall_clock64();
    }
#endif
}

template <int OP>
__global__ __launch_bounds__(256) void spmv_prescale_kernel(const float *__restrict__ x, const uint32_t *__restrict__ zcols,
                                                            const float *__restrict__ zcolval, float *__restrict__ z, uint32_t nz,
                                                            uint32_t num_cols,
                                                            const uint32_t *__restrict__ hot_cols, const float *__restrict__ hot_colval,
                                                            float *__restrict__ hot_x, uint32_t nhot,
                                                            const uint32_t *__restrict__ run_flag) {
    if (run_flag && *run_flag == 0u) return;
    const uint32_t i = blockIdx.x * 256u + threadIdx.x;
    if (4u * i < nz) {
        const float4 v = reinterpret_cast<const float4 *>(zcolval)[i];
        float4 xv;
        if (zcols) {
            const uint4 c = reinterpret_cast<const uint4 *>(zcols)[i];
            xv = make_float4(x[c.x], x[c.y], x[c.z], x[c.w]);
        } else {
            const uint32_t c = 4u * i, last = num_cols - 1u;
            xv = make_float4(x[c], x[min(c + 1u, last)], x[min(c + 2u, last)], x[min(c + 3u, last)]);
        }
        reinterpret_cast<float4 *>(z)[i] = make_float4(Semiring<OP>::mul(v.x, xv.x), Semiring<OP>::mul(v.y, xv.y),
                                                       Semiring<OP>::mul(v.z, xv.z), Semiring<OP>::mul(v.w, xv.w));
    }
    if (i < nhot) hot_x[i] = Semiring<OP>::mul(hot_colval[i], x[hot_cols[i]]);
}

__global__ __launch_bounds__(256) void spmv_hot_gather_kernel(const float *__restrict__ x, const uint32_t *__restrict__ hot_cols,
                                                              float *__restrict__ hot_x, uint32_t nhot,
                                                              const uint32_t *__restrict__ ccols, float *__restrict__ xc, uint32_t ncompact,
                                                              const uint32_t *__restrict__ run_flag) {
    if (run_flag && *run_flag == 0u) return;
    const uint32_t i = blockIdx.x * 256u + threadIdx.x;
    if (i < nhot) hot_x[i] = x[hot_cols[i]];
    if (ncompact == 0u) return;
    const uint32_t n4 = (ncompact + 3u) / 4u, base = blockIdx.x * 1024u + threadIdx.x;
    uint4 c[4];
#pragma unroll
    for (int k = 0; k < 4; k++) c[k] = reinterpret_cast<const uint4 *>(ccols)[min(base + k * 256u, n4 - 1u)];
    float4 v[4];
#pragma unroll
    for (int k = 0; k < 4; k++) v[k] = make_float4(x[c[k].x], x[c[k].y], x[c[k].z], x[c[k].w]);
#pragma unroll
    for (int k = 0; k < 4; k++)
        if (base + k * 256u < n4) reinterpret_cast<float4 *>(xc)[base + k * 256u] = v[k];
}

template <int OP, bool PATTERN>
__global__ __launch_bounds__(256) void spmv_spread_x_kernel(const float *__restrict__ x, const uint32_t *__restrict__ colmap,
                                                            const float *__restrict__ colval_bycol, float *__restrict__ packed,
                                                            float *__restrict__ hot_x, uint32_t num_cols,
                                                            const uint32_t *__restrict__ run_flag) {
    if (run_flag && *run_flag == 0u) return;
    const uint32_t cb = blockIdx.x * 1024u + threadIdx.x, last = num_cols - 1u;
    uint32_t m[4];
    float v[4], kv[4];
#pragma unroll
    for (int k = 0; k < 4; k++) {
        const uint32_t c = cb + 256u * k, cc = min(c, last);
        m[k] = c < num_cols ? colmap[cc] : 0xffffffffu;
        v[k] = x[cc];
        kv[k] = PATTERN ? colval_bycol[cc] : 0.0f;
    }
#pragma unroll
    for (int k = 0; k < 4; k++) {
        if (m[k] == 0xffffffffu) continue;
        const float out = PATTERN ? Semiring<OP>::mul(kv[k], v[k]) : v[k];
        if (m[k] >> 31) hot_x[m[k] & 0x7fffffffu] = out;
        else packed[m[k]] = out;
    }
}

template <int OP, int MASK>
__global__ __launch_bounds__(256) void spmv_init_kernel(uint32_t r0, uint32_t r1, const float *__restrict__ mask,
                                                        float *__restrict__ y, float zero) {
// ... 335 lines not shown
    return gl::bool_plan_bfs_step(p, d_bits_in, d_bits_out, d_distance, level, gl::ctx().stream, nullptr, 0u, GL_GATE_EQ, nullptr, 0u, 0.0f, 0,
                                  &c, may_push ? gl::spmspv_plan_indptr(csc) : nullptr, gl::spmspv_plan_num_cols(csc),
                                  gl::spmspv_plan_bfs_acc(csc), deferred);
}

int gl_spmv_run(gl_spmv_plan p, const float *d_x, const float *d_mask, float *d_y, int op, float zero,
                int mask_type) {
    GL_TRACE();
    GL_REQUIRE_INIT();
    GL_ARG(p != nullptr && d_y != nullptr);
    GL_ARG(d_x != nullptr || p->nnz == 0);
    GL_ARG(mask_type == GL_NOMASK || d_mask != nullptr);
    if (p->reference_order) return gl::spmv_run_reference_order(p, d_x, d_mask, d_y, op, zero, mask_type, gl::ctx().stream);
    if (p->boolean) {
        if (op != GL_OP_ANDOR)
            return gl::set_error(GL_ERR_UNSUPPORTED, "gl_spmv_run: this plan was created with GL_PLAN_BOOLEAN and "
                                 "holds the sparsity pattern only; semiring op %d needs a plan without it", op);
        return gl::bool_plan_run(p, d_x, nullptr, d_mask, d_y, zero, mask_type, gl::ctx().stream);
    }
    return gl::spmv_run_general(p, d_x, d_mask, d_y, op, zero, mask_type, nullptr);
}

int gl_spmv_plan_chain(gl_spmv_plan p, int on, int *active) {
    GL_REQUIRE_INIT();
    GL_ARG(p != nullptr);
    if (active) *active = 0;
    p->chain_ptr = nullptr;
    p->chain_on = false;
    if (!on) return GL_OK;
    if (p->boolean || p->reference_order || !p->d_colmap || p->segments > 1 || p->row_begin != 0 || p->row_end != p->num_rows ||
        p->num_rows != p->num_cols || p->packed_len == 0)
        return GL_OK;
    if (!p->d_packed_twin) {
        hipError_t e = hipMalloc((void **)&p->d_packed_twin, p->packed_len * sizeof(float));
        if (e == hipSuccess) e = hipMemsetAsync(p->d_packed_twin, 0, p->packed_len * sizeof(float), gl::ctx().stream);
        if (e == hipSuccess && p->hot_x_len) {
            e = hipMalloc((void **)&p->d_hot_x_twin, p->hot_x_len * sizeof(float));
            if (e == hipSuccess) e = hipMemsetAsync(p->d_hot_x_twin, 0, p->hot_x_len * sizeof(float), gl::ctx().stream);
        }
        if (e != hipSuccess) {
            (void)hipFree(p->d_packed_twin);
            (void)hipFree(p->d_hot_x_twin);
            p->d_packed_twin = p->d_hot_x_twin = nullptr;
            return gl::set_error(GL_ERR_HIP, "gl_spmv_plan_chain: %s", hipGetErrorString(e));
        }
        p->device_bytes += (p->packed_len + p->hot_x_len) * sizeof(float);
    }
    p->chain_on = true;
    if (active) *active = 1;
    return GL_OK;
}

int gl_spmv_run_typed(gl_spmv_plan p, const void *d_x, const void *d_mask, void *d_y, int op, uint32_t zero_bits, int mask_type,
                      int val_type) {
    GL_REQUIRE_INIT();
    GL_ARG(p != nullptr && d_y != nullptr);
    GL_ARG(d_x != nullptr || p->nnz == 0);
    GL_ARG(mask_type == GL_NOMASK || d_mask != nullptr);
    GL_ARG(op == GL_OP_MULADD || op == GL_OP_ANDOR || op == GL_OP_ADDMIN);
    const float zero = __builtin_bit_cast(float, zero_bits);
    if (val_type == GL_VAL_FLOAT) return gl_spmv_run(p, (const float *)d_x, (const float *)d_mask, (float *)d_y, op, zero, mask_type);
    if (val_type != GL_VAL_UNSIGNED && val_type != GL_VAL_UFIXED_32_8)
        return gl::set_error(GL_ERR_INVALID_ARG, "gl_spmv_run_typed: unknown value type %d", val_type);
    if (p->boolean || p->reference_order)
        return gl::set_error(GL_ERR_UNSUPPORTED, "gl_spmv_run_typed: GL_PLAN_BOOLEAN / GL_PLAN_REFERENCE_ORDER plans serve float only; create the plan without the flag");
    return gl::spmv_run_general(p, (const float *)d_x, (const float *)d_mask, (float *)d_y, op + 3 * val_type, zero, mask_type, nullptr);
}

}

namespace gl {
int spmv_run_general(gl_spmv_plan p, const float *d_x, const float *d_mask, float *d_y, int op, float zero, int mask_type,
                     const uint32_t *run_flag) {
    if (p->boolean || p->reference_order) return set_error(GL_ERR_UNSUPPORTED, "spmv_run_general: boolean / reference-order layout");
    if ((p->flags & (GL_PLAN_BOOLEAN | GL_PLAN_NO_MULADD)) && (op == GL_OP_MULADD || op == gl::kOpFixMulAdd) && p->nhot_lds &&
        (size_t)p->nhot_lds * 4u + ((size_t)p->max_block_rows + gl::kPadSlots) * sizeof(gl::Tile<GL_OP_MULADD>::T) > gl::kLdsBudget)
        return gl::set_error(GL_ERR_UNSUPPORTED, "gl_spmv_run: this plan was created with GL_PLAN_NO_MULADD "
                             "(hot-column table sized for 4-byte accumulators); (+,x) needs a plan without it");
    gl::SpmvArgs a;
    a.entries = reinterpret_cast<const unsigned char *>(p->d_entries);
    a.bases = p->d_bases;
    a.units = p->d_units;
    a.hub_rows = p->d_hub_rows;
    a.hot_x = p->d_hot_x;
    a.nhot = p->nhot_lds;
    a.hot = p->d_hot;
    a.hot_hdr = p->d_hot_hdr;
    a.present = p->d_present;
    a.x = d_x;
    a.xg = p->ncompact ? p->d_xc : d_x;
    a.mask = d_mask;
    a.y = d_y;
    a.zero = zero;
    a.run_flag = run_flag;
    a.z = p->d_z;
    a.diag = p->d_diag;
    a.diag_has = p->d_diag_has;
    a.partials = p->d_partials;
    a.prow = p->row_end - p->row_begin;
    a.row_begin = p->row_begin;
    static const uint32_t tickets = 1u;
    a.tickets = tickets;
    a.self_hot_cols = p->self_hot ? p->d_hot_cols : nullptr;
    hipStream_t s = gl::ctx().stream;
    int rc;
    switch (op) {
        case GL_OP_MULADD: rc = gl::dispatch_mask<GL_OP_MULADD>(mask_type, p, a, s); break;
        case GL_OP_ANDOR: rc = gl::dispatch_mask<GL_OP_ANDOR>(mask_type, p, a, s); break;
        case GL_OP_ADDMIN: rc = gl::dispatch_mask<GL_OP_ADDMIN>(mask_type, p, a, s); break;
        case gl::kOpU32MulAdd: rc = gl::dispatch_mask<gl::kOpU32MulAdd>(mask_type, p, a, s); break;
        case gl::kOpU32AndOr: rc = gl::dispatch_mask<gl::kOpU32AndOr>(mask_type, p, a, s); break;
        case gl::kOpU32AddMin: rc = gl::dispatch_mask<gl::kOpU32AddMin>(mask_type, p, a, s); break;
        case gl::kOpFixMulAdd: rc = gl::dispatch_mask<gl::kOpFixMulAdd>(mask_type, p, a, s); break;
        case gl::kOpFixAndOr: rc = gl::dispatch_mask<gl::kOpFixAndOr>(mask_type, p, a, s); break;
        case gl::kOpFixAddMin: rc = gl::dispatch_mask<gl::kOpFixAddMin>(mask_type, p, a, s); break;
        default: rc = gl::set_error(GL_ERR_INVALID_ARG, "gl_spmv_run: invalid semiring op %d", op); break;
    }
    return rc;
}

}

namespace gl {
int preload_spmv() {
    hipFuncAttributes attr;
    GL_HIP(hipFuncGetAttributes(&attr, (const void *)spmv_hot_gather_kernel));
    return GL_OK;
}
}

#if defined(GL_UNIT_CLOCKS)
extern "C" int gl_debug_unit_clocks(unsigned long long *out) {
    return hipMemcpyFromSymbol(out, HIP_SYMBOL(gl::g_unit_clocks), sizeof(gl::g_unit_clocks)) == hipSuccess ? 0 : 1;
}
#endif
```

graphlily_amd/csrc/gl_spmv_plan.cpp:

```cpp
#include "gl_spmv_plan.h"

#include <climits>
#include <memory>

namespace gl {

static double stream_rate(double gap) {
    static const double gx[] = {2.5, 5.0, 10.0, 13.0, 26.0, 52.0, 104.0};
    static const double gy[] = {5.85, 5.45, 4.9, 4.5, 3.8, 3.0, 2.3};
    if (gap <= gx[0]) return gy[0];
    for (int i = 1; i < 7; i++)
        if (gap <= gx[i]) {
            double t = (std::log(gap) - std::log(gx[i - 1])) / (std::log(gx[i]) - std::log(gx[i - 1]));
            return gy[i - 1] + t * (gy[i] - gy[i - 1]);
        }
    return gy[6];
}

static Shape choose_shape(uint64_t rows, uint64_t cols, uint64_t nnz, int num_cus) {
    Shape best{1, 1};
    if (rows == 0 || nnz == 0) return best;
    const double deg = (double)nnz / (double)rows;
    const uint64_t rmax = kMaxPlainRows - 64;
    double best_cost = 1e300;
// ... 38 lines not shown
                if (e < r + 1) e = r + 1;
                if (align > 1u && e < row_end) {
                    uint32_t ea = e / align * align;
                    if (ea <= r) ea = std::min<uint64_t>(row_end, (uint64_t)(r / align + 1u) * align);
                    e = ea;
                }
                if (out) out->push_back(e);
                r = e;
                made++;
            }
            return made;
        };
        uint64_t lo = (nnz + shape.blocks - 1) / shape.blocks, hi = nnz;
        if (cut(hi, nullptr) > shape.blocks) {
            lo = hi;
            const uint32_t forced = cut(hi, nullptr);
            uint64_t l2 = (nnz + forced - 1) / forced, h2 = nnz;
            while (l2 < h2) {
                const uint64_t mid = (l2 + h2) / 2;
                if (cut(mid, nullptr) <= forced) h2 = mid; else l2 = mid + 1;
            }
            lo = l2;
        } else {
            while (lo < hi) {
                const uint64_t mid = (lo + hi) / 2;
                if (cut(mid, nullptr) <= shape.blocks) hi = mid; else lo = mid + 1;
            }
        }
        cut(lo, &bstart);
    } else if (nnz > 0) {
        const double target = (double)nnz / (double)shape.blocks;
        uint32_t r = row_begin, made = 0;
        while (r < row_end) {
            made++;
            const uint32_t hi = (uint32_t)std::min<uint64_t>(row_end, (uint64_t)r + max_rows);
            uint32_t e;
            if (made >= shape.blocks && hi == row_end) {
                e = row_end;
            } else {
                const uint64_t want64 = nz0 + (uint64_t)std::llround(target * made);
                const uint32_t want = (uint32_t)std::min<uint64_t>(want64, nz1);
                const uint32_t *ub = std::upper_bound(h_indptr + r + 1, h_indptr + hi + 1, want);
                e = (uint32_t)(ub - h_indptr) - 1u;
                if (e < r + 1) e = r + 1;
                if (align > 1u) {
                    uint32_t ea = (e + align / 2u) / align * align;
                    if (ea <= r) ea = r - r % align + align;
                    if (ea >= hi) ea = (hi == row_end) ? row_end : hi / align * align;
                    e = ea;
                }
            }
            bstart.push_back(e);
            r = e;
        }
    }
    const uint32_t nblocks = bp.nblocks = (uint32_t)bstart.size() - 1;
    bp.seg.assign(nblocks, 1);
    if (nblocks && shape.segments > 1) {
        const uint32_t cus = (uint32_t)ctx().num_cus;
        uint64_t budget = (uint64_t)shape.blocks * shape.segments;
        budget = std::max<uint64_t>(cus, budget / cus * cus);
        if (budget < nblocks) budget = nblocks;
        const double per_unit = (double)nnz / (double)budget;
        uint64_t used = 0;
        std::vector<std::pair<double, uint32_t>> frac;
        for (uint32_t b = 0; b < nblocks; b++) {
            const double want = (double)((uint64_t)h_indptr[bstart[b + 1]] - h_indptr[bstart[b]]) / per_unit;
            bp.seg[b] = std::max<uint32_t>(1u, (uint32_t)want);
            used += bp.seg[b];
            frac.push_back({want - (double)bp.seg[b], b});
        }
        std::sort(frac.begin(), frac.end(), [](const std::pair<double, uint32_t> &x, const std::pair<double, uint32_t> &y) { return x.first > y.first; });
        for (size_t i = 0; used < budget && i < frac.size(); i++, used++) bp.seg[frac[i].second]++;
        for (uint32_t b = 0; b < nblocks; b++) bp.Smax = std::max(bp.Smax, bp.seg[b]);
    }
    bp.all_direct = (bp.Smax == 1);
    bp.unit_of.assign(bp.Smax, std::vector<uint32_t>(nblocks, 0xffffffffu));
    for (uint32_t sgm = 0; sgm < bp.Smax; sgm++)
        for (uint32_t b = 0; b < nblocks; b++)
            if (bp.seg[b] > sgm) bp.unit_of[sgm][b] = bp.nunits++;
    return bp;
}

struct PlanDeleter {
    void operator()(gl_spmv_plan p) const { gl_spmv_plan_destroy(p); }
};
using PlanOwner = std::unique_ptr<gl_spmv_plan_s, PlanDeleter>;

struct Knobs {
    long pattern = debug_knob("spmv_pattern", 1);
    long hot = debug_knob("spmv_hot", 1);
    long hot_floor = debug_knob("spmv_hot_floor", LONG_MIN);
    long helper = debug_knob("spmv_helper", -1);
    long compact = debug_knob("spmv_compact", 1);
    long hub_div = debug_knob("spmv_hub_div", 48);
    long mix = debug_knob("spmv_mix", -1);
    long boolean = debug_knob("spmv_bool", 1);
};

struct HostCsr {
    const uint32_t *indptr, *indices;
    const float *data;
    uint32_t num_cols, row_begin, row_end;
    uint64_t nnz;
};

static int column_error(uint32_t num_cols) {
    return set_error(GL_ERR_INVALID_ARG, "gl_spmv_plan_create: column index out of range (num_cols %u)", num_cols);
}

static int plan_reference_order(gl_spmv_plan p, const HostCsr &a) {
    const uint64_t nz0 = a.indptr[a.row_begin], nnz = a.nnz;
    for (uint64_t i = nz0; i < nz0 + nnz; i++)
        if (a.indices[i] >= a.num_cols) return column_error(a.num_cols);
    p->reference_order = true;
    const uint32_t rows = a.row_end - a.row_begin;
    std::vector<uint32_t> ip((size_t)rows + 1u);
    for (uint32_t r = 0; r <= rows; r++) ip[r] = (uint32_t)(a.indptr[a.row_begin + r] - nz0);
    hipError_t e = hipMalloc((void **)&p->d_csr_indptr, ip.size() * 4u);
    if (e == hipSuccess) e = hipMalloc((void **)&p->d_csr_indices, std::max<uint64_t>(nnz, 1u) * 4u);
    if (e == hipSuccess) e = hipMalloc((void **)&p->d_csr_data, std::max<uint64_t>(nnz, 1u) * 4u);
    if (e == hipSuccess) e = hipMemcpy(p->d_csr_indptr, ip.data(), ip.size() * 4u, hipMemcpyHostToDevice);
    if (e == hipSuccess && nnz) e = hipMemcpy(p->d_csr_indices, a.indices + nz0, nnz * 4u, hipMemcpyHostToDevice);
    if (e == hipSuccess && nnz) e = hipMemcpy(p->d_csr_data, a.data + nz0, nnz * 4u, hipMemcpyHostToDevice);
    if (e != hipSuccess) return set_error(GL_ERR_HIP, "gl_spmv_plan_create: reference-order plan: %s", hipGetErrorString(e));
    p->device_bytes = ip.size() * 4u + nnz * 8u;
    return GL_OK;
}

static int detect_pattern_host(const HostCsr &a, std::vector<uint32_t> &colbits, std::vector<uint32_t> &diag_has,
                               std::vector<float> &diag_val, int *mismatch_out, uint64_t *exceptions_out) {
    const uint32_t num_cols = a.num_cols, row_begin = a.row_begin, row_end = a.row_end, rows = row_end - row_begin;
    const uint32_t *h_indptr = a.indptr, *h_indices = a.indices;
    const float *h_data = a.data;
    int mismatch = 0;
    uint64_t exceptions = 0;
    colbits.assign(num_cols, 0u);
    diag_has.assign((size_t)(rows + 31) / 32, 0u);
    diag_val.assign(rows, 0.0f);
#pragma omp parallel for schedule(static, 4096)
    for (int64_t r = row_begin; r < (int64_t)row_end; r++)
        for (uint64_t i = h_indptr[r]; i < h_indptr[r + 1]; i++) {
            const uint32_t c = h_indices[i];
            if (c < num_cols && c != (uint32_t)r) {
                const uint32_t bits = __builtin_bit_cast(uint32_t, h_data[i]);
                if (__atomic_load_n(&colbits[c], __ATOMIC_RELAXED) != bits) __atomic_store_n(&colbits[c], bits, __ATOMIC_RELAXED);
            }
        }
#pragma omp parallel for schedule(static, 4096) reduction(| : mismatch) reduction(+ : exceptions)
    for (int64_t r = row_begin; r < (int64_t)row_end; r++) {
        uint32_t nexc = 0;
        for (uint64_t i = h_indptr[r]; i < h_indptr[r + 1]; i++) {
            const uint32_t c = h_indices[i], bits = __builtin_bit_cast(uint32_t, h_data[i]);
            if (c >= num_cols) { mismatch = 1; continue; }
            if (colbits[c] == bits) continue;
            if (c != (uint32_t)r) { mismatch = 1; continue; }
            nexc++;
            diag_val[r - row_begin] = h_data[i];
            diag_has[(r - row_begin) >> 5] |= 1u << ((r - row_begin) & 31);
        }
        if (nexc > 1) mismatch = 1;
        exceptions += nexc;
    }
    *mismatch_out = mismatch;
    *exceptions_out = exceptions;
    return GL_OK;
}

static bool values_finite_host(const HostCsr &a) {
    const uint64_t nz0 = a.nnz ? a.indptr[a.row_begin] : 0;
    int found = 0;
#pragma omp parallel for schedule(static) reduction(| : found)
    for (int64_t i = 0; i < (int64_t)a.nnz; i++)
        found |= (__builtin_bit_cast(uint32_t, a.data[nz0 + i]) & 0x7f800000u) == 0x7f800000u;
    return !found;
}

static int column_degrees_host(const HostCsr &a, std::vector<uint32_t> &deg, int *bad_col) {
    const uint64_t nz0 = a.indptr[a.row_begin];
    deg.assign(a.num_cols, 0);
    for (uint64_t i = nz0; i < nz0 + a.nnz; i++) {
        if (a.indices[i] < a.num_cols) deg[a.indices[i]]++;
        else *bad_col = 1;
    }
    return GL_OK;
}

static void choose_hot_columns(const Knobs &k, uint32_t flags, uint64_t nnz, const std::vector<uint32_t> &deg, uint32_t tallest,
                               uint32_t nblocks, bool pattern, std::vector<uint32_t> &hot_cols, std::vector<uint32_t> &colmap) {
    const uint32_t num_cols = (uint32_t)deg.size();
    const size_t elem = (flags & (GL_PLAN_NO_MULADD | GL_PLAN_BOOLEAN)) ? sizeof(float) : sizeof(double);
    const size_t tile_bytes = ((size_t)tallest + kHubSlots * kMaxHubRows + kPadSlots) * elem;
    uint32_t room = 0;
    if (tile_bytes + 4096u <= kLdsBudget)
        room = std::min<uint32_t>(1u << 15, (uint32_t)((kLdsBudget - tile_bytes - 320u) / 4u / 64u * 64u));
    uint32_t H = room;
    if (nnz <= (16ull << 20) && (uint64_t)num_cols * 4u <= (1ull << 20)) H = 0;
    if (k.hot > 1) H = std::min<uint32_t>(room, (uint32_t)k.hot);
    if (!H) return;
    const uint32_t dmax = num_cols ? *std::max_element(deg.begin(), deg.end()) : 0u;
    std::vector<uint32_t> hist((size_t)dmax + 2, 0);
    for (uint32_t c = 0; c < num_cols; c++) hist[deg[c]]++;
    const long floor_knob = k.hot_floor != LONG_MIN ? k.hot_floor : (pattern ? 1 : 4);
    const uint32_t floor_deg = std::max<uint32_t>(8u, (uint32_t)floor_knob * nblocks);
    uint64_t seen = 0;
    uint32_t thr = dmax + 1;
    while (thr > floor_deg && seen + hist[thr - 1] <= H) { thr--; seen += hist[thr]; }
    std::vector<uint32_t> hot;
    for (uint32_t c = 0; c < num_cols; c++)
        if (deg[c] >= thr && hot.size() < H) hot.push_back(c);
    uint64_t hn = 0;
    for (uint32_t c : hot) hn += deg[c];
    if (hot.empty() || (double)hn < 0.05 * (double)nnz) return;
    for (uint32_t j = 0; j < (uint32_t)hot.size(); j++) colmap[hot[j]] = 0x80000000u | j;
    hot_cols.swap(hot);
}

static void order_packed_columns(const std::vector<uint32_t> &deg, const BlockPlan &bp, bool by_class, std::vector<uint32_t> &ccols,
                                 std::vector<uint32_t> &colmap) {
    const uint32_t num_cols = (uint32_t)deg.size(), nb = bp.nblocks;
    const uint32_t edge[3] = {std::max(nb / 4u, 1u), std::max(nb / 16u, 1u), std::max(nb / 64u, 1u)};
    auto cls = [&](uint32_t c) -> int {
        if (deg[c] == 0 || (colmap[c] >> 31)) return -1;
        if (!by_class) return 0;
        return deg[c] >= edge[0] ? 0 : deg[c] >= edge[1] ? 1 : deg[c] >= edge[2] ? 2 : 3;
    };
    uint32_t start[5] = {0, 0, 0, 0, 0};
    for (uint32_t c = 0; c < num_cols; c++) {
        const int k = cls(c);
        if (k >= 0) start[k + 1]++;
    }
    for (int k = 0; k < 4; k++) start[k + 1] += start[k];
    const uint32_t gathered = start[4];
    ccols.assign(std::max(gathered, 1u), 0u);
    for (uint32_t c = 0; c < num_cols; c++) {
        const int k = cls(c);
        if (k >= 0) {
            colmap[c] = start[k];
            ccols[start[k]++] = c;
        } else if (!(colmap[c] >> 31)) {
            colmap[c] = 0xffffffffu;
        }
    }
}

static int emit_general_host(const HostCsr &a, const EmitGeneral &eg, gl_spmv_plan p, std::vector<uint32_t> &hub_count, uint64_t *hot_nnz_out) {
    const uint32_t *h_indptr = a.indptr, *h_indices = a.indices, *colmap = eg.colmap, *colbits = eg.colbits;
    const float *h_data = a.data;
    const BlockPlan &bp = *eg.bp;
    const std::vector<uint32_t> &bstart = bp.bstart, &seg = bp.seg;
    const std::vector<std::vector<uint32_t>> &unit_of = bp.unit_of;
    const uint32_t nblocks = bp.nblocks, nunits = bp.nunits, gather_cols = eg.gather_cols, nhot_table = eg.nhot_table;
    const bool all_direct = bp.all_direct, pattern = eg.pattern, diag_mode = eg.diag_mode;
    const uint32_t cold_groups = pattern ? kColdGroupsPattern : kColdGroupsGeneral;
    const uint32_t cold_elem_bytes = pattern ? kColdElemBytesPattern : kColdElemBytesGeneral;
    const bool hot_rows = pattern;
    const uint32_t hot_groups = hot_rows ? 1u : kHotGroupsGeneral;
    const uint32_t hot_elem_bytes = hot_rows ? kHotElemBytesRows : kHotElemBytesGeneral;
    const uint32_t hot_hdr_words = hot_rows ? 0u : kHotHdrWordsPerGroup * hot_groups;

    std::vector<uint64_t> mc(nblocks, 0), mh(nblocks, 0), mrec(nblocks, 0);
#pragma omp parallel for schedule(dynamic, 1)
    for (int64_t b = 0; b < (int64_t)nblocks; b++) {
        uint64_t nc = 0, nh = 0, nrec = 0;
        for (uint32_t r = bstart[b]; r < bstart[b + 1]; r++) {
            uint64_t hr = 0;
            for (uint64_t i = h_indptr[r]; i < h_indptr[r + 1]; i++) {
                const uint32_t c = h_indices[i];
                if (diag_mode && c == r && __builtin_bit_cast(uint32_t, h_data[i]) != colbits[c]) continue;
                if (colmap[c] >> 31) hr++; else nc++;
            }
            nh += hr;
            nrec += (hr + kHotRecEntries - 1u) / kHotRecEntries;
        }
        mc[b] = nc, mh[b] = nh, mrec[b] = nrec;
    }
    const UnitLayout ul = layout_units(bp, mc, mh, eg.dummy_max, hot_groups, nhot_table, hot_rows ? &mrec : nullptr);
    const uint64_t total_groups = ul.cold_goff[nunits], hot_elems = ul.hot_e0[nunits];
    if (!(total_groups < 0xffffffffull && hot_elems < 0xffffffffull && ul.present_off[nunits] < 0xffffffffull))
        return set_error(GL_ERR_INVALID_ARG, "gl_spmv_plan_create_ex: invalid argument: total_groups < 0xffffffffull && "
                         "hot_elems < 0xffffffffull && ul.present_off[nunits] < 0xffffffffull");
    std::vector<unsigned char> entries((size_t)(total_groups / cold_groups + 1) * cold_elem_bytes, 0);
    std::vector<uint32_t> bases(total_groups, 0u);
    std::vector<uint4> units((size_t)nunits * 3);
    std::vector<uint32_t> hub_rows((size_t)nblocks * kMaxHubRows, 0);
    std::vector<unsigned char> hot_bytes((size_t)(hot_elems + 1) * hot_elem_bytes, 0);
    {
        uint16_t *rows16 = reinterpret_cast<uint16_t *>(hot_bytes.data() + (size_t)hot_elems * hot_elem_bytes);
        for (uint32_t k = 0; k < (hot_rows ? hot_elem_bytes / 2u : 64u * hot_groups); k++) rows16[k] = (uint16_t)kRowPad;
    }
    std::vector<uint32_t> hot_hdr(hot_rows ? (size_t)8 : (size_t)(hot_elems + 1) * hot_hdr_words, 0u);
    std::vector<uint16_t> present((size_t)std::max<uint64_t>(ul.present_off[nunits], 2u), 0);
    uint32_t max_present = 0;
    uint64_t hot_nnz = 0;
#pragma omp parallel reduction(+ : hot_nnz) reduction(max : max_present)
    {
        std::vector<Rec> recs, tmp, hot;
        std::vector<uint64_t> rec_of_hot;
#pragma omp for schedule(dynamic, 1)
        for (int64_t b = 0; b < (int64_t)nblocks; b++) {
            const uint32_t r0 = bstart[b], r1 = bstart[b + 1];
            recs.clear();
            hot.clear();
            for (uint32_t r = r0; r < r1; r++)
                for (uint64_t i = h_indptr[r]; i < h_indptr[r + 1]; i++) {
                    const uint32_t c = h_indices[i];
                    const uint32_t v = __builtin_bit_cast(uint32_t, h_data[i]);
                    if (diag_mode && c == r && v != colbits[c]) continue;
                    if (colmap[c] >> 31) hot.push_back(Rec{colmap[c] & 0x7fffffffu, r - r0, v});
                    else recs.push_back(Rec{colmap[c], r - r0, v});
                }
            sort_by_col(recs, tmp, gather_cols);
            if (!hot_rows) sort_by_col(hot, tmp, nhot_table ? nhot_table : 1u);
            hot_nnz += hot.size();
            const uint64_t mcb = recs.size(), m = mcb + hot.size();
            std::vector<uint32_t> cnt(r1 - r0, 0);
            for (const Rec &rc : recs) cnt[rc.row_local]++;
            for (const Rec &rc : hot) cnt[rc.row_local]++;
            std::vector<int> hub_of(r1 - r0, -1);
            {
                const uint64_t thr = std::max<uint64_t>(256, m / (uint64_t)eg.hub_div);
                uint32_t nh = 0;
                for (uint32_t i = 0; i < r1 - r0 && nh < kMaxHubRows; i++)
                    if (cnt[i] >= thr) {
                        hub_of[i] = (int)nh;
                        hub_rows[(size_t)b * kMaxHubRows + nh] = i;
                        nh++;
                    }
                hub_count[b] = nh;
            }
            const uint32_t nrows_b = r1 - r0;
            const uint32_t pad_slot = nrows_b + kHubSlots * hub_count[b];
            auto slot_of = [&](const Rec &rc, uint32_t fill) -> uint32_t {
                const int hb = hub_of[rc.row_local];
                return hb < 0 ? rc.row_local : nrows_b + kHubSlots * (uint32_t)hb + (fill & (kHubSlots - 1u));
            };
            const uint32_t S = seg[b];
            for (uint32_t s = 0; s < S; s++) {
                const size_t u = unit_of[s][b];
                const uint64_t goff = ul.cold_goff[u];
                uint64_t q = 0;
                uint32_t prev = 0;
                auto put = [&](uint32_t idx, uint32_t slot, uint32_t val) {
                    const uint64_t g = goff + q / 64;
                    const uint32_t lane = (uint32_t)(q % 64), k = (uint32_t)(g % cold_groups);
                    unsigned char *el = entries.data() + (size_t)(g / cold_groups) * cold_elem_bytes;
                    const uint32_t delta = lane ? idx - prev : 0u;
                    if (!lane) bases[g] = idx;
                    if (pattern) {
                        reinterpret_cast<uint16_t *>(el)[lane * 8u + k] = (uint16_t)slot;
                        el[1024u + lane * 8u + k] = (unsigned char)delta;
                    } else {
                        reinterpret_cast<uint16_t *>(el)[lane * 4u + k] = (uint16_t)slot;
                        el[512u + lane * 4u + k] = (unsigned char)delta;
                        reinterpret_cast<uint32_t *>(el + 768u)[lane * 4u + k] = val;
                    }
                    prev = idx;
                    q++;
                };
                for (uint64_t i = mcb * s / S; i < mcb * (s + 1) / S; i++) {
                    const Rec &rc = recs[i];
                    if (q)
                        while (rc.col - prev > kColdMaxDelta) put(prev + kColdMaxDelta, pad_slot + (uint32_t)(q % 64), 0u);
                    put(rc.col, slot_of(rc, (uint32_t)(q % 64)), rc.val);
                }
                const uint64_t qend = (q + 64u * cold_groups - 1) / (64u * cold_groups) * (64u * cold_groups);
                while (q < qend) {
                    if (q % 64 == 0) prev = 0;
                    put(prev, pad_slot + (uint32_t)(q % 64), 0u);
                }
                const uint64_t g = goff + q / 64;
                const uint32_t ncold = (uint32_t)(g - goff);
                if (hot_rows) {
                    const uint64_t M = mrec[b], j0 = M * s / S, j1 = M * (s + 1) / S, e0 = ul.hot_e0[u];
                    const uint32_t nel = (uint32_t)(ul.hot_e0[u + 1] - e0), chunk = nel;
                    for (uint32_t e = 0; e < nel; e++) {
                        uint16_t *el = reinterpret_cast<uint16_t *>(hot_bytes.data() + (size_t)(e0 + e) * hot_elem_bytes);
                        for (uint32_t l = 0; l < 64u; l++) {
                            for (uint32_t k = 0; k < kHotRecEntries; k++) el[l * 8u + k] = (uint16_t)nhot_table;
                            el[l * 8u + 7u] = (uint16_t)(pad_slot + l);
                        }
                    }
                    if (s == 0) {
                        rec_of_hot.clear();
                        uint64_t j = 0;
                        for (size_t i = 0; i < hot.size();) {
                            size_t i1 = i;
                            while (i1 < hot.size() && hot[i1].row_local == hot[i].row_local) i1++;
                            for (size_t q = i; q < i1; q++) rec_of_hot.push_back(j + (q - i) / kHotRecEntries);
                            j += (i1 - i + kHotRecEntries - 1u) / kHotRecEntries;
                            i = i1;
                        }
                    }
                    for (size_t i = 0, f = 0; i < hot.size(); i++) {
                        const uint64_t j = rec_of_hot[i];
                        f = (i > 0 && rec_of_hot[i - 1] == j) ? f + 1 : 0;
                        if (j < j0 || j >= j1) continue;
                        const uint32_t jj = (uint32_t)(j - j0), l = jj / chunk, e = jj % chunk;
                        uint16_t *rec = reinterpret_cast<uint16_t *>(hot_bytes.data() + (size_t)(e0 + e) * hot_elem_bytes) + l * 8u;
                        rec[f] = (uint16_t)hot[i].col;
                        if (f == 0) rec[7] = (uint16_t)slot_of(hot[i], l);
                    }
                    units[3 * u] = make_uint4((uint32_t)goff, ncold, r0, (r1 - r0) | (all_direct ? 0x80000000u : 0u));
                    units[3 * u + 1] = make_uint4((uint32_t)((size_t)b * kMaxHubRows), hub_count[b], nel, s);
                    units[3 * u + 2] = make_uint4((uint32_t)e0, 0u, nhot_table, 0u);
                    continue;
                }
                const uint64_t h0 = hot.size() * s / S, h1 = hot.size() * (s + 1) / S, e0 = ul.hot_e0[u];
                uint16_t *pres = present.data() + ul.present_off[u];
                uint32_t np = 0;
                for (size_t e = (size_t)e0; e < (size_t)ul.hot_e0[u + 1]; e++) {
                    uint16_t *rows16 = reinterpret_cast<uint16_t *>(hot_bytes.data() + e * hot_elem_bytes);
                    for (uint32_t k = 0; k < 64u * hot_groups; k++) rows16[k] = (uint16_t)(pad_slot + k / hot_groups);
                }
                for (uint64_t i = h0; i < h1; i++) {
                    const uint64_t j = i - h0, hg = j / 64;
                    const uint32_t l = (uint32_t)(j % 64), k = (uint32_t)(hg % hot_groups);
                    const size_t e = (size_t)(e0 + hg / hot_groups);
                    const bool start = i == h0 || hot[i].col != hot[i - 1].col;
                    if (start) pres[np++] = (uint16_t)hot[i].col;
                    uint32_t *hd = hot_hdr.data() + e * hot_hdr_words;
                    if (l == 0) hd[2 * hot_groups + k] = np - 1u;
                    else if (start) hd[2 * k + ((l - 1u) >> 5)] |= 1u << ((l - 1u) & 31u);
                    unsigned char *el = hot_bytes.data() + e * hot_elem_bytes;
                    const uint16_t slot16 = (uint16_t)slot_of(hot[i], l);
                    if (pattern) {
                        reinterpret_cast<uint16_t *>(el)[l * 8u + k] = slot16;
                    } else {
                        reinterpret_cast<uint16_t *>(el)[l * 4u + k] = slot16;
                        reinterpret_cast<uint32_t *>(el + 512)[l * 4u + k] = hot[i].val;
                    }
                }
                max_present = std::max(max_present, np);
                const uint32_t nhotg = (uint32_t)(ul.hot_e0[u + 1] - e0) * hot_groups;
                units[3 * u] = make_uint4((uint32_t)goff, ncold, r0, (r1 - r0) | (all_direct ? 0x80000000u : 0u));
                units[3 * u + 1] = make_uint4((uint32_t)((size_t)b * kMaxHubRows), hub_count[b], nhotg, s);
                units[3 * u + 2] = make_uint4((uint32_t)e0, (uint32_t)ul.present_off[u], np, 0u);
            }
        }
    }
    p->nhot_elems = hot_elems;
    p->nhot_lds = hot_rows ? (nhot_table ? nhot_table + 64u : 0u) : (max_present + 63u) / 64u * 64u;
    p->ngroups = total_groups;
    *hot_nnz_out = hot_nnz;
    bases.insert(bases.end(), 8, 0u);
    int rc;
    if ((rc = plan_upload(p, p->d_entries, entries.data(), entries.size())) != GL_OK ||
        (rc = plan_upload(p, p->d_bases, bases.data(), bases.size() * sizeof(uint32_t))) != GL_OK ||
        (rc = plan_upload(p, p->d_units, units.data(), units.size() * sizeof(uint4))) != GL_OK ||
        (rc = plan_upload(p, p->d_hub_rows, hub_rows.data(), hub_rows.size() * sizeof(uint32_t))) != GL_OK ||
        (rc = plan_upload(p, p->d_hot, hot_bytes.data(), hot_bytes.size())) != GL_OK ||
        (rc = plan_upload(p, p->d_hot_hdr, hot_hdr.data(), hot_hdr.size() * sizeof(uint32_t))) != GL_OK ||
        (rc = plan_upload(p, p->d_present, present.data(), present.size() * sizeof(uint16_t))) != GL_OK)
        return rc;
    p->b_entries = entries.size();
    p->b_bases = bases.size() * sizeof(uint32_t);
    p->b_units = units.size() * sizeof(uint4);
    p->b_hub_rows = hub_rows.size() * sizeof(uint32_t);
    p->b_hot = hot_bytes.size();
    p->b_hot_hdr = hot_hdr.size() * sizeof(uint32_t);
    p->b_present = present.size() * sizeof(uint16_t);
    return GL_OK;
}

static int choose_mix(const Knobs &k, bool pattern, bool have_hot, uint64_t hot_nnz, uint64_t nnz) {
    const double hot_frac = nnz ? (double)hot_nnz / (double)nnz : 0.0;
    const int mix = (pattern || hot_frac >= 0.42) ? 3 : 2;
    return !have_hot ? 0 : (k.mix > 0 ? (int)k.mix : mix);
}

static bool self_hot_rule(long helper_mode, uint64_t nnz, uint32_t nhot_table) {
    return (helper_mode == 2 || (helper_mode < 0 && nnz <= (16ull << 20))) && nhot_table <= 4096u;
}

struct Helper {
    bool self_hot, spread;
};
static Helper choose_helper(long mode, bool self_hot_ok, bool pattern, bool compact, uint32_t Smax, uint32_t gather_cols,
                            uint32_t nhot_table, uint32_t num_cols) {
    Helper h;
    h.self_hot = self_hot_ok && !pattern && !compact;
    h.spread = compact && (mode == 1 || (mode < 0 && Smax == 1 && 4ull * ((uint64_t)gather_cols + nhot_table) >= num_cols));
    return h;
}

static int upload_plan(gl_spmv_plan p, const BlockPlan &bp, const std::vector<uint32_t> &hot_cols, std::vector<uint32_t> &ccols,
                       uint32_t gather_cols, const std::vector<uint32_t> *spread_colmap, const std::vector<uint32_t> &colbits,
                       bool diag_mode, const std::vector<float> &diag_val, const std::vector<uint32_t> &diag_has) {
    std::vector<uint4> blocks(bp.nblocks);
    for (uint32_t b = 0; b < bp.nblocks; b++) blocks[b] = make_uint4(bp.bstart[b], bp.bstart[b + 1] - bp.bstart[b], bp.seg[b], 0u);
    int rc;
    if ((rc = plan_upload(p, p->d_hot_cols, hot_cols.data(), hot_cols.size() * sizeof(uint32_t))) != GL_OK ||
        (rc = plan_upload(p, p->d_blocks, blocks.data(), blocks.size() * sizeof(uint4))) != GL_OK)
        return rc;
    if (p->pattern) {
        std::vector<uint32_t> zval(((size_t)gather_cols + 3) / 4 * 4, 0u), hval(hot_cols.size());
        for (uint32_t j = 0; j < gather_cols; j++) zval[j] = colbits[p->ncompact ? ccols[j] : j];
        for (size_t j = 0; j < hot_cols.size(); j++) hval[j] = colbits[hot_cols[j]];
        if ((rc = plan_upload(p, p->d_colval, zval.data(), zval.size() * 4u)) != GL_OK ||
            (rc = plan_upload(p, p->d_hot_colval, hval.data(), hval.size() * 4u)) != GL_OK ||
            (rc = plan_alloc(p, p->d_z, ((size_t)gather_cols + 4u) * sizeof(float), (size_t)gather_cols * sizeof(float), "z")) != GL_OK)
            return rc;
        p->packed_len = (size_t)gather_cols + 4u;
    }
    if (p->ncompact) {
        while (ccols.size() % 4u) ccols.push_back(ccols.back());
        if ((rc = plan_upload(p, p->d_ccols, ccols.data(), ccols.size() * sizeof(uint32_t))) != GL_OK) return rc;
        if (!p->pattern) {
            if ((rc = plan_alloc(p, p->d_xc, ((size_t)gather_cols + 4u) * sizeof(float), (size_t)gather_cols * sizeof(float), "xc")) != GL_OK)
                return rc;
            p->packed_len = (size_t)gather_cols + 4u;
        }
    }
    if (spread_colmap) {
        if ((rc = plan_upload(p, p->d_colmap, spread_colmap->data(), spread_colmap->size() * 4u)) != GL_OK) return rc;
        if (p->pattern && (rc = plan_upload(p, p->d_colval_bycol, colbits.data(), (size_t)p->num_cols * 4u)) != GL_OK) return rc;
    }
    if (diag_mode) {
        if ((rc = plan_upload(p, p->d_diag, diag_val.data(), diag_val.size() * sizeof(float))) != GL_OK ||
            (rc = plan_upload(p, p->d_diag_has, diag_has.data(), diag_has.size() * sizeof(uint32_t))) != GL_OK)
            return rc;
    }
    if (p->segments > 1) {
        const size_t bytes = (size_t)p->segments * (p->row_end - p->row_begin) * sizeof(float);
        if ((rc = plan_alloc(p, p->d_partials, bytes, bytes, "partials")) != GL_OK) return rc;
    }
    p->hot_x_len = p->nhot;
    return plan_alloc(p, p->d_hot_x, std::max<size_t>((size_t)p->nhot * sizeof(float), 16u), 0u, "hot_x", true);
}

static int plan_general(gl_spmv_plan p, const HostCsr &a, const Knobs &k) {
    const uint32_t num_cols = a.num_cols;
    const uint64_t nnz = a.nnz;
    StagedCsr staged;
    const bool on_device = nnz > 0 && format_on_device(p->flags, nnz);
    int rc;
    if (on_device && (rc = devcsr_stage(&staged.c, a.indptr, a.indices, a.data, a.row_begin, a.row_end)) != GL_OK) return rc;

    const Shape shape = choose_shape(a.row_end - a.row_begin, num_cols, nnz, ctx().num_cus);
    const BlockPlan bp = plan_blocks(shape, a.indptr, a.row_begin, a.row_end, kMaxPlainRows);
    for (uint32_t b = 0; b < bp.nblocks; b++) p->max_plain_rows = std::max(p->max_plain_rows, bp.bstart[b + 1] - bp.bstart[b]);

    if (on_device) {
        int finite = 1;
        if ((rc = fmt_values_finite(staged.c, &finite)) != GL_OK) return rc;
        p->values_finite = finite != 0;
    } else {
        p->values_finite = values_finite_host(a);
    }

    std::vector<uint32_t> colbits, diag_has;
    std::vector<float> diag_val;
    bool diag_mode = false;
    if (nnz > 0 && !(p->flags & GL_PLAN_KEEP_VALUES) && k.pattern != 0) {
        int mismatch = 0;
        uint64_t exceptions = 0;
        rc = on_device ? fmt_detect_pattern(staged.c, num_cols, colbits, diag_has, diag_val, &mismatch, &exceptions)
                       : detect_pattern_host(a, colbits, diag_has, diag_val, &mismatch, &exceptions);
        if (rc != GL_OK) return rc;
        p->pattern = !mismatch;
        diag_mode = p->pattern && exceptions > 0;
    }

    std::vector<uint32_t> deg, hot_cols, ccols, colmap(num_cols);
    for (uint32_t c = 0; c < num_cols; c++) colmap[c] = c;
    if (nnz > 0) {
        int bad = 0;
        rc = on_device ? fmt_column_degrees(staged.c, num_cols, deg, &bad) : column_degrees_host(a, deg, &bad);
        if (rc != GL_OK) return rc;
        if (bad) return column_error(num_cols);
        if (k.hot != 0) choose_hot_columns(k, p->flags, nnz, deg, p->max_plain_rows, bp.nblocks, p->pattern, hot_cols, colmap);
    }
    const uint32_t nhot_table = (uint32_t)((hot_cols.size() + 63) / 64 * 64);
    if (nhot_table) hot_cols.resize(nhot_table, hot_cols[0]);
    const bool self_hot_ok = self_hot_rule(k.helper, nnz, nhot_table);
    if (nnz > 0 && k.compact != 0 && (!self_hot_ok || k.compact == 3))
        order_packed_columns(deg, bp, bp.Smax == 1 && k.compact != 2, ccols, colmap);
    const bool compact = !ccols.empty();
    const uint32_t gather_cols = compact ? (uint32_t)ccols.size() : num_cols;

    EmitGeneral eg;
    eg.bp = &bp;
    eg.dummy_max = gather_cols / kColdMaxDelta + 1u;
    eg.colmap = colmap.data();
    eg.gather_cols = gather_cols, eg.nhot_table = nhot_table;
    eg.diag_mode = diag_mode, eg.colbits = colbits.data(), eg.diag_has = diag_has.data();
    eg.pattern = p->pattern;
    eg.group_mult = p->pattern ? kColdGroupsPattern : kColdGroupsGeneral;
    eg.hub_div = (uint32_t)std::max<long>(1, k.hub_div);
    eg.h_indptr = a.indptr, eg.num_cols = num_cols;
    std::vector<uint32_t> hub_count(bp.nblocks, 0);
    uint64_t hot_nnz = 0;
    rc = on_device ? fmt_emit_general(staged.c, eg, p, hub_count, &hot_nnz) : emit_general_host(a, eg, p, hub_count, &hot_nnz);
    if (rc != GL_OK) return rc;

    p->nblocks = bp.nblocks;
    p->segments = bp.Smax;
    p->nunits = bp.nunits;
    for (uint32_t b = 0; b < bp.nblocks; b++)
        p->max_block_rows = std::max(p->max_block_rows, bp.bstart[b + 1] - bp.bstart[b] + kHubSlots * hub_count[b]);
    p->nhot = nhot_table;
    p->hot_nnz = hot_nnz;
    p->ncompact = compact ? gather_cols : 0u;
    p->mix = choose_mix(k, p->pattern, nhot_table != 0, hot_nnz, nnz);
    const Helper h = choose_helper(k.helper, self_hot_ok, p->pattern, compact, bp.Smax, gather_cols, nhot_table, num_cols);
    p->self_hot = h.self_hot;
    return upload_plan(p, bp, hot_cols, ccols, gather_cols, h.spread ? &colmap : nullptr, colbits, diag_mode, diag_val, diag_has);
}

}

extern "C" {

int gl_spmv_plan_create(gl_spmv_plan *plan, uint32_t num_rows, uint32_t num_cols,
                        const uint32_t *h_indptr, const uint32_t *h_indices, const float *h_data,
                        uint32_t row_begin, uint32_t row_end) {
    return gl_spmv_plan_create_ex(plan, num_rows, num_cols, h_indptr, h_indices, h_data, row_begin, row_end, 0u);
}

int gl_spmv_plan_create_ex(gl_spmv_plan *plan, uint32_t num_rows, uint32_t num_cols,
                           const uint32_t *h_indptr, const uint32_t *h_indices, const float *h_data,
                           uint32_t row_begin, uint32_t row_end, uint32_t flags) {
    GL_TRACE();
    GL_REQUIRE_INIT();
    GL_ARG(plan != nullptr && h_indptr != nullptr);
    GL_ARG(row_begin <= row_end && row_end <= num_rows);
    GL_ARG(num_cols < 0x40000000u);
    const uint64_t nz0 = h_indptr[row_begin], nz1 = h_indptr[row_end];
    GL_ARG(nz1 >= nz0);
    const uint64_t nnz = nz1 - nz0;
    GL_ARG(nnz == 0 || (h_indices != nullptr && h_data != nullptr));
    for (uint32_t r = row_begin; r < row_end; r++) GL_ARG(h_indptr[r + 1] >= h_indptr[r]);

    const gl::Knobs k;
    const gl::HostCsr a{h_indptr, h_indices, h_data, num_cols, row_begin, row_end, nnz};
    gl::PlanOwner p(new gl_spmv_plan_s());
    p->num_rows = num_rows;
    p->num_cols = num_cols;
    p->row_begin = row_begin;
    p->row_end = row_end;
    p->nnz = nnz;
    p->flags = flags;
    int rc;
    if (flags & GL_PLAN_REFERENCE_ORDER) {
        p->values_finite = gl::values_finite_host(a);
        rc = gl::plan_reference_order(p.get(), a);
    } else if ((flags & GL_PLAN_BOOLEAN) && nnz > 0 && gl::cdiv(num_cols, gl::kBoolPhaseCols) <= gl::kBoolMaxPhases && k.boolean != 0) {
        p->values_finite = gl::values_finite_host(a);
        rc = gl::bool_plan_build(p.get(), h_indptr, h_indices, h_data);
        if (rc == GL_OK) rc = gl::bool_plan_compress(p.get());
        const long keep = gl::debug_knob("bool_keep", -1);
        p->bool_keep = (keep == 0 || keep == 1) ? (int8_t)keep : (int8_t)-1;
    } else {
        rc = gl::plan_general(p.get(), a, k);
    }
    if (rc != GL_OK) return rc;
    *plan = p.release();
    return GL_OK;
}

int gl_spmv_plan_destroy(gl_spmv_plan p) {
    if (!p) return GL_OK;
    gl::spmspv_detach_everywhere(p);
    (void)hipFree(p->d_entries);
    (void)hipFree(p->d_bases);
    (void)hipFree(p->d_units);
    (void)hipFree(p->d_hub_rows);
    (void)hipFree(p->d_hot);
    (void)hipFree(p->d_hot_hdr);
    (void)hipFree(p->d_present);
    (void)hipFree(p->d_hot_cols);
    (void)hipFree(p->d_hot_x);
    (void)hipFree(p->d_spans);
    (void)hipFree(p->d_blocks);
    (void)hipFree(p->d_colval);
    (void)hipFree(p->d_hot_colval);
    (void)hipFree(p->d_ccols);
    (void)hipFree(p->d_colmap);
    (void)hipFree(p->d_packed_twin);
    (void)hipFree(p->d_hot_x_twin);
    (void)hipFree(p->d_colval_bycol);
    (void)hipFree(p->d_xc);
    (void)hipFree(p->d_diag);
    (void)hipFree(p->d_diag_has);
    (void)hipFree(p->d_z);
    (void)hipFree(p->d_partials);
    (void)hipFree(p->d_xbits);
    (void)hipFree(p->d_csr_indptr);
    (void)hipFree(p->d_csr_indices);
    (void)hipFree(p->d_parents_scratch);
    (void)hipFree(p->d_cc_scratch);
    (void)hipFree(p->d_tc_scratch);
    (void)hipFree(p->d_kcore_scratch);
    (void)hipFree(p->d_color_scratch);
    (void)hipFree(p->d_truss_scratch);
    (void)hipFree(p->d_msf_scratch);
    (void)hipFree(p->d_match_scratch);
    (void)hipFree(p->d_lpa_scratch);
    (void)hipFree(p->d_scc_scratch);
    (void)hipFree(p->d_bc_scratch);
    if (p->h_bc_pinned) (void)hipHostFree(p->h_bc_pinned);
    (void)hipFree(p->d_csr_data);
    delete p;
    return GL_OK;
}

int gl_spmv_plan_describe(gl_spmv_plan p, gl_spmv_plan_desc *out) {
    GL_ARG(p != nullptr && out != nullptr);
    out->nnz = p->nnz;
    out->device_bytes = p->device_bytes;
    out->groups = p->ngroups;
    out->hot_nnz = p->hot_nnz;
    out->num_units = p->nunits;
    out->blocks = p->nblocks;
    out->segments = p->segments;
    out->max_block_rows = p->max_block_rows;
    out->hot_columns = p->nhot;
    out->packed_columns = p->ncompact;
    out->layout = p->reference_order ? GL_LAYOUT_REFERENCE_ORDER : p->boolean ? GL_LAYOUT_BOOLEAN : (p->pattern ? GL_LAYOUT_PATTERN : GL_LAYOUT_GENERAL);
    out->mix = p->mix;
    out->helper = p->boolean ? GL_HELPER_NONE : p->self_hot ? GL_HELPER_SELF_HOT : p->d_colmap ? GL_HELPER_SPREAD
                  : (p->pattern || p->nhot || p->ncompact) ? GL_HELPER_GATHER : GL_HELPER_NONE;
    return GL_OK;
}

int gl_spmv_plan_values_finite(gl_spmv_plan p, int *finite) {
    GL_ARG(p != nullptr && finite != nullptr);
    *finite = p->values_finite ? 1 : 0;
    return GL_OK;
}

int gl_spmv_plan_export(gl_spmv_plan p, int array, void *h_dst, size_t capacity, size_t *bytes) {
    GL_REQUIRE_INIT();
    GL_ARG(p != nullptr && bytes != nullptr);
    const void *src = nullptr;
    size_t n = 0;
    switch (array) {
        case GL_PLAN_ARRAY_ENTRIES: src = p->d_entries, n = p->b_entries; break;
        case GL_PLAN_ARRAY_BASES: src = p->d_bases, n = p->b_bases; break;
        case GL_PLAN_ARRAY_UNITS: src = p->d_units, n = p->b_units; break;
        case GL_PLAN_ARRAY_HUB_ROWS: src = p->d_hub_rows, n = p->b_hub_rows; break;
        case GL_PLAN_ARRAY_SPANS: src = p->d_spans, n = p->b_spans; break;
        case GL_PLAN_ARRAY_HOT: src = p->d_hot, n = p->b_hot; break;
        case GL_PLAN_ARRAY_HOT_HDR: src = p->d_hot_hdr, n = p->b_hot_hdr; break;
        case GL_PLAN_ARRAY_PRESENT: src = p->d_present, n = p->b_present; break;
        default: return gl::set_error(GL_ERR_INVALID_ARG, "gl_spmv_plan_export: unknown array %d", array);
    }
    *bytes = n;
    if (!h_dst) return GL_OK;
    GL_ARG(capacity >= n);
    if (n) {
        GL_HIP(hipStreamSynchronize(gl::ctx().stream));
        GL_HIP(hipMemcpy(h_dst, src, n, hipMemcpyDeviceToHost));
    }
    return GL_OK;
}

}
```

graphlily_amd/csrc/gl_spmv_plan.h:

```cpp
#ifndef GL_SPMV_PLAN_H_
#define GL_SPMV_PLAN_H_

#include "gl_common.h"

#include <algorithm>
#include <atomic>
#include <cmath>
#include <cstdlib>
#include <cstring>
#include <vector>

namespace gl {

constexpr uint32_t kRowBits = 14;
constexpr uint32_t kRowPad = (1u << kRowBits) - 1u;
constexpr uint32_t kMaxBlockRows = kRowPad;
constexpr uint32_t kColOffBits = 32 - kRowBits;
constexpr uint32_t kHubSlots = 16;
constexpr uint32_t kMaxHubRows = 64;
constexpr uint32_t kPadSlots = 64;
constexpr uint32_t kMaxPlainRows = kMaxBlockRows - kHubSlots * kMaxHubRows - kPadSlots;
constexpr uint32_t kBoolMaxPhases = 8;
constexpr uint32_t kLdsBudget = 160u * 1024u - 512u;
constexpr uint32_t kThreads = 1024;
constexpr uint32_t kWaves = kThreads / 64;

constexpr uint32_t kBoolPhaseWords = 36864;
constexpr uint32_t kBoolPhaseCols = kBoolPhaseWords * 32u;
#ifndef GL_BOOL_GROUP
#define GL_BOOL_GROUP 256
#endif
constexpr uint32_t kBoolGroup = GL_BOOL_GROUP;
constexpr uint32_t kBoolTileWords = (kMaxBlockRows + 1u) / 32u;
constexpr uint32_t kBoolHubSlots = 32;
constexpr uint32_t kBoolHubMax = 31;
constexpr uint32_t kBoolHubBit0 = (kBoolTileWords - kBoolHubSlots) * 32u;

constexpr uint32_t kColdGroupsGeneral = 4, kColdGroupsPattern = 8;
constexpr uint32_t kColdElemBytesGeneral = kColdGroupsGeneral * 64u * 7u;
constexpr uint32_t kColdElemBytesPattern = kColdGroupsPattern * 64u * 3u;
constexpr uint32_t kColdMaxDelta = 255;

constexpr uint32_t kHotRecEntries = 7;
constexpr uint32_t kHotElemBytesRows = 64u * 16u;

constexpr uint32_t kHotGroupsGeneral = 4;
constexpr uint32_t kHotElemBytesGeneral = kHotGroupsGeneral * 64u * 6u;
constexpr uint32_t kHotHdrWordsPerGroup = 3;

struct Shape {
    uint32_t blocks, segments;
};

struct Rec {
    uint32_t col, row_local, val;
};

static inline void sort_by_col(std::vector<Rec> &a, std::vector<Rec> &tmp, uint32_t num_cols) {
    const size_t n = a.size();
    tmp.resize(n);
    int bits = 1;
    while ((1ull << bits) < num_cols) bits++;
    const int passes = (bits + 10) / 11;
    for (int p = 0; p < passes; p++) {
        const int sh = 11 * p;
        size_t cnt[2049] = {0};
        for (size_t i = 0; i < n; i++) cnt[((a[i].col >> sh) & 2047u) + 1]++;
        for (int i = 0; i < 2048; i++) cnt[i + 1] += cnt[i];
        for (size_t i = 0; i < n; i++) tmp[cnt[(a[i].col >> sh) & 2047u]++] = a[i];
        a.swap(tmp);
    }
}

struct BlockPlan {
    std::vector<uint32_t> bstart;
    std::vector<uint32_t> seg;
    std::vector<std::vector<uint32_t>> unit_of;
    uint32_t nblocks = 0, nunits = 0, Smax = 1;
    bool all_direct = true;
};

BlockPlan plan_blocks(Shape shape, const uint32_t *h_indptr, uint32_t row_begin, uint32_t row_end, uint32_t max_rows,
                      uint32_t align = 1);

struct UnitLayout {
    std::vector<uint64_t> cold_goff;
    std::vector<uint64_t> hot_e0;
    std::vector<uint64_t> present_off;
};
inline UnitLayout layout_units(const BlockPlan &bp, const std::vector<uint64_t> &mc, const std::vector<uint64_t> &mh, uint32_t dummy_max,
                               uint32_t hot_groups, uint32_t nhot_table, const std::vector<uint64_t> *mrec = nullptr) {
    UnitLayout ul;
    ul.cold_goff.assign((size_t)bp.nunits + 1, 0);
    ul.hot_e0.assign((size_t)bp.nunits + 1, 0);
    ul.present_off.assign((size_t)bp.nunits + 1, 0);
    for (uint32_t b = 0; b < bp.nblocks; b++) {
        const uint32_t S = bp.seg[b];
        for (uint32_t s = 0; s < S; s++) {
            const size_t u = bp.unit_of[s][b];
            const uint64_t c = mc[b] * (s + 1) / S - mc[b] * s / S, h = mh[b] * (s + 1) / S - mh[b] * s / S;
            ul.cold_goff[u + 1] = c ? ((c + dummy_max + 63) / 64 + 7u) / 8u * 8u : 0u;
            if (mrec) {
                const uint64_t rc = (*mrec)[b] * (s + 1) / S - (*mrec)[b] * s / S;
                ul.hot_e0[u + 1] = (rc + 63) / 64;
                ul.present_off[u + 1] = 0;
            } else {
                ul.hot_e0[u + 1] = ((h + 63) / 64 + hot_groups - 1u) / hot_groups;
                ul.present_off[u + 1] = (std::min<uint64_t>(h, nhot_table) + 1u) / 2u * 2u;
            }
        }
    }
    for (size_t u = 0; u < bp.nunits; u++) {
        ul.cold_goff[u + 1] += ul.cold_goff[u];
        ul.hot_e0[u + 1] += ul.hot_e0[u];
        ul.present_off[u + 1] += ul.present_off[u];
    }
    return ul;
}

}

namespace gl {
inline uint64_t plan_uid() {
    static std::atomic<uint64_t> next{0};
    return ++next;
}
}

struct gl_spmv_plan_s {
    uint32_t num_rows = 0, num_cols = 0, row_begin = 0, row_end = 0;
    uint64_t nnz = 0;
    uint32_t nunits = 0, nblocks = 0, segments = 1, max_block_rows = 0;
    uint64_t ngroups = 0;
    uint2 *d_entries = nullptr;
    uint32_t *d_bases = nullptr;
    uint4 *d_units = nullptr;
    unsigned char *d_hot = nullptr;
    uint32_t *d_hot_hdr = nullptr;
    uint16_t *d_present = nullptr;
    uint32_t nhot_lds = 0;
    uint64_t nhot_elems = 0;
    uint32_t *d_hub_rows = nullptr;
    uint32_t flags = 0;
    uint32_t nhot = 0;
    uint64_t hot_nnz = 0;
    int mix = 0;
    uint32_t *d_hot_cols = nullptr;
    float *d_hot_x = nullptr;
    float *d_hot_colval = nullptr;
    uint32_t ncompact = 0;
    uint32_t *d_ccols = nullptr;
    float *d_xc = nullptr;
    float *d_packed_twin = nullptr, *d_hot_x_twin = nullptr;
    size_t packed_len = 0, hot_x_len = 0;
    bool chain_on = false;
    const float *chain_ptr = nullptr;
    int chain_sel = 0, chain_op = -1;
    uint32_t *d_colmap = nullptr;
    float *d_colval_bycol = nullptr;
    bool self_hot = false;
    bool pattern = false;
    bool values_finite = true;
    float *d_colval = nullptr, *d_z = nullptr;
    float *d_diag = nullptr;
    uint32_t *d_diag_has = nullptr;
    uint4 *d_blocks = nullptr;
    float *d_partials = nullptr;
    uint32_t max_plain_rows = 0;
    bool boolean = false;
    int bool_compressed = 0;
    int8_t bool_keep = -1;
    uint32_t nphases = 0;
    uint4 *d_spans = nullptr;
    uint32_t *d_xbits = nullptr;
    uint32_t *d_csr_indptr = nullptr, *d_csr_indices = nullptr;
    uint32_t csr_nz_base = 0;
    int rows_sorted = -1;
    int rows_are_sets = -1;
    int rows_symmetric = -1;
    unsigned char *d_parents_scratch = nullptr;
    uint32_t *d_cc_scratch = nullptr;
    unsigned char *d_tc_scratch = nullptr;
    uint32_t tc_items[4] = {0, 0, 0, 0}, tc_cap[3] = {0, 0, 0};
    unsigned char *d_kcore_scratch = nullptr;
    unsigned char *d_color_scratch = nullptr;
    unsigned char *d_truss_scratch = nullptr;
    int64_t truss_edges = -1;
    unsigned char *d_msf_scratch = nullptr;
    unsigned char *d_match_scratch = nullptr;
    unsigned char *d_lpa_scratch = nullptr;
    unsigned char *d_scc_scratch = nullptr;
    uint64_t uid = gl::plan_uid();
    unsigned char *d_bc_scratch = nullptr;
    uint32_t *h_bc_pinned = nullptr;
    size_t bc_pinned_words = 0;
    const gl_spmv_plan_s *bc_partner = nullptr;
    uint64_t bc_partner_uid = 0;
    int bc_transpose_ok = -1;
    bool reference_order = false;
    float *d_csr_data = nullptr;
    uint64_t device_bytes = 0;
    size_t b_entries = 0, b_bases = 0, b_units = 0, b_hub_rows = 0, b_spans = 0;
    size_t b_hot = 0, b_hot_hdr = 0, b_present = 0;
};

namespace gl {
template <typename T>
int plan_upload(gl_spmv_plan p, T *&d, const void *h, size_t bytes) {
    GL_HIP(hipMalloc((void **)&d, bytes ? bytes : 16));
    if (bytes) GL_HIP(hipMemcpy(d, h, bytes, hipMemcpyHostToDevice));
    p->device_bytes += bytes;
    return GL_OK;
}
template <typename T>
int plan_alloc(gl_spmv_plan p, T *&d, size_t bytes, size_t counted, const char *what, bool zero = false) {
    hipError_t e = hipMalloc((void **)&d, bytes);
    if (e == hipSuccess && zero) e = hipMemsetAsync(d, 0, bytes, ctx().stream);
    if (e != hipSuccess) return set_error(GL_ERR_HIP, "gl_spmv_plan_create: hipMalloc(%s): %s", what, hipGetErrorString(e));
    p->device_bytes += counted;
    return GL_OK;
}

struct DevCsr;
int devcsr_stage(DevCsr **out, const uint32_t *h_indptr, const uint32_t *h_indices, const float *h_data,
                 uint32_t row_begin, uint32_t row_end);
void devcsr_release(DevCsr *c);
struct StagedCsr {
    DevCsr *c = nullptr;
    ~StagedCsr() { devcsr_release(c); }
};
int devcsr_adopt_rows(DevCsr *c, uint32_t **d_indptr, uint32_t **d_indices);
bool format_on_device(uint32_t flags, uint64_t nnz);
int fmt_column_degrees(DevCsr *c, uint32_t num_cols, std::vector<uint32_t> &deg, int *bad_col);
int fmt_values_finite(DevCsr *c, int *finite);
int fmt_detect_pattern(DevCsr *c, uint32_t num_cols, std::vector<uint32_t> &colbits, std::vector<uint32_t> &diag_has,
                       std::vector<float> &diag_val, int *mismatch, uint64_t *exceptions);

struct EmitGeneral {
    const BlockPlan *bp;
    uint32_t dummy_max;
    const uint32_t *colmap;
    uint32_t gather_cols, nhot_table;
    bool diag_mode;
    const uint32_t *colbits;
    const uint32_t *diag_has;
    bool pattern;
    uint32_t group_mult;
    uint32_t hub_div;
    const uint32_t *h_indptr;
    uint32_t num_cols;
};
int fmt_emit_general(DevCsr *c, const EmitGeneral &e, gl_spmv_plan p, std::vector<uint32_t> &hub_count, uint64_t *hot_nnz);
struct EmitBool {
    const BlockPlan *bp;
    const uint32_t *h_indptr;
    uint32_t num_cols;
};
int fmt_emit_bool(DevCsr *c, const EmitBool &e, gl_spmv_plan p, uint32_t *max_rows);

int fmt_spmspv_stream(uint32_t num_rows, uint32_t num_cols, const uint32_t *h_indptr, const uint32_t *h_indices, const float *h_data,
                      uint32_t r0, uint32_t r1, uint32_t **d_indptr_out, uint2 **d_stream_out, std::vector<uint32_t> &indptr_out);
int fmt_csr2csc(uint32_t num_rows, uint32_t num_cols, const uint32_t *h_indptr, const uint32_t *h_indices, const float *h_data,
                uint32_t *csc_indptr, uint32_t *csc_indices, float *csc_data);
int fmt_normalize_by_outdegree(uint32_t num_rows, uint32_t num_cols, const uint32_t *h_indptr, const uint32_t *h_indices, float *h_data);

int bool_plan_build(gl_spmv_plan p, const uint32_t *h_indptr, const uint32_t *h_indices, const float *h_data);
int bool_plan_compress(gl_spmv_plan p);
int bool_plan_run(gl_spmv_plan p, const float *d_x, const uint32_t *bits, const float *d_mask, float *d_y, float zero,
                  int mask_type, hipStream_t s);
int pack_bits(const float *d_x, uint32_t n, uint32_t *d_bits, hipStream_t s);
int unpack_bits(const uint32_t *d_bits, uint32_t n, float *d_x, hipStream_t s);
int bfs_bits_begin_from(uint32_t *d_ctl, uint32_t ctl_words, const float *d_x, uint32_t n, uint32_t *d_bits, uint32_t words, hipStream_t s,
                        const float *d_distance, gl_spmv_plan rows);
int bool_plan_bfs_step(gl_spmv_plan p, const uint32_t *bits_in, uint32_t *bits_out, float *d_distance, float level, hipStream_t s,
                       const uint32_t *gate = nullptr, uint32_t gate_value = 0, int gate_op = GL_GATE_EQ, uint32_t *back_ctl = nullptr,
                       uint32_t back_slot = 0, float back_threshold = 0.0f, int back_may_continue = 0, const BfsBitsCtl *v2 = nullptr,
                       const uint32_t *v2_indptr = nullptr, uint32_t v2_ncols = 0, uint32_t *v2_push_acc = nullptr, bool v2_deferred = false);
int bool_plan_run_bits(gl_spmv_plan p, float *d_y, const uint32_t *run_flag, hipStream_t s, const uint32_t *xbits = nullptr);
struct BfsPushArgs;
struct BfsShardArgs;
int bool_plan_bfs_shard_step(gl_spmv_plan p, BfsPushArgs pa, BfsShardArgs sa, hipStream_t s);
int bits_to_sparse_gated(const uint32_t *d_bits, uint32_t n, gl_idx_val *d_out, uint32_t *d_counts, const uint32_t *gate_word,
                         uint32_t gate_value, hipStream_t s);
uint32_t *bool_plan_xbits(gl_spmv_plan p);
size_t bool_plan_xbits_bytes(gl_spmv_plan p);
int spmv_run_general(gl_spmv_plan p, const float *d_x, const float *d_mask, float *d_y, int op, float zero, int mask_type,
                     const uint32_t *run_flag);
unsigned long long spmspv_heavy_work(gl_spmspv_plan p);
unsigned long long spmspv_bottom_up_limit(gl_spmspv_plan p);
unsigned long long spmspv_plan_nnz(gl_spmspv_plan p);
const void *spmspv_plan_bfs_rows(gl_spmspv_plan p);
const uint32_t *spmspv_plan_indptr(gl_spmspv_plan p);
uint32_t spmspv_plan_num_cols(gl_spmspv_plan p);
uint32_t *spmspv_plan_bfs_acc(gl_spmspv_plan p);
bool spmspv_plan_whole(gl_spmspv_plan p, uint32_t num_rows);
struct SpmspvCsc {
    const uint32_t *indptr;
    const uint2 *stream;
    uint32_t num_cols, row_begin, row_end;
    uint32_t **ctl;
};
SpmspvCsc spmspv_plan_csc(gl_spmspv_plan p);
void spmspv_detach_everywhere(gl_spmv_plan dying);
int spmv_init_rows(int op, int mask_type, uint32_t r0, uint32_t r1, const float *mask, float *y, float zero, hipStream_t s);
}

#endif
```

include/graphlily_hip.h:

```cpp
#ifndef GRAPHLILY_HIP_H_
#define GRAPHLILY_HIP_H_

#include <stddef.h>
#include <stdint.h>

#ifdef __cplusplus
extern "C" {
#endif

typedef enum gl_status {
    GL_OK = 0,
    GL_ERR_INVALID_ARG = -1,
    GL_ERR_HIP = -2,
    GL_ERR_NOT_INITIALIZED = -3,
    GL_ERR_IO = -4,
    GL_ERR_UNSUPPORTED = -5
} gl_status;

typedef enum gl_op { GL_OP_MULADD = 0, GL_OP_ANDOR = 1, GL_OP_ADDMIN = 2 } gl_op;
typedef enum gl_mask { GL_NOMASK = 0, GL_MASK_WRITETOZERO = 1, GL_MASK_WRITETOONE = 2 } gl_mask;

typedef struct gl_idx_val { uint32_t index; float val; } gl_idx_val;

typedef struct gl_spmv_plan_s *gl_spmv_plan;
typedef struct gl_spmspv_plan_s *gl_spmspv_plan;

int gl_init(int device);
int gl_host_bind_near_device(int *numa_node, int *cpus);
int gl_device_count(int *count);
int gl_set_stream(void *hip_stream);
int gl_reset_stream(void);
int gl_sync(void);
typedef struct gl_graph_s *gl_graph;
int gl_graph_begin_capture(void);
int gl_graph_end_capture(gl_graph *graph);
int gl_graph_launch(gl_graph graph);
int gl_graph_destroy(gl_graph graph);
const char *gl_last_error(void);
const char *gl_version(void);

int gl_buf_alloc(void **d_ptr, size_t bytes);
int gl_buf_free(void *d_ptr);
int gl_buf_h2d(void *d_dst, const void *h_src, size_t bytes);
int gl_buf_d2h(void *h_dst, const void *d_src, size_t bytes);
int gl_buf_d2h_async(void *h_dst, const void *d_src, size_t bytes);
int gl_levels_pack(const float *d_levels, uint32_t n, int bits, const uint32_t *d_tail, uint32_t tail_words, void *d_out);
int gl_host_unpack_threads(void);
int gl_sync_levels_unpack(float *h_dst, const void *h_src, size_t n, int bits);
int gl_host_levels_unpack(float *h_dst, const void *h_src, size_t n, int bits);
#define GL_LEVELS_CHUNK_WORDS 2048u
#define GL_LEVELS_FLAG_STRIDE_WORDS 16u
int gl_levels_stream_bytes(uint32_t n, int bits, uint32_t tail_words, size_t *bytes);
int gl_levels_stream_arm(void *h_block, uint32_t n, int bits, uint32_t tail_words);
int gl_levels_pack_stream(const float *d_levels, uint32_t n, int bits, const uint32_t *d_tail, uint32_t tail_words, void *h_block);
int gl_sync_levels_unpack_stream(float *h_dst, const void *h_block, size_t n, int bits, uint32_t *h_tail, uint32_t tail_words);
int gl_buf_d2h_levels(float *h_dst, const float *d_src, size_t n, float max_level, int *packed);
int gl_buf_d2d(void *d_dst, const void *d_src, size_t bytes);
int gl_buf_fill_f32(float *d_dst, float value, size_t count);
int gl_buf_fill_u32(uint32_t *d_dst, uint32_t value, size_t count);
int gl_host_alloc(void **h_ptr, size_t bytes);
int gl_host_free(void *h_ptr);
int gl_host_pool_reserve(size_t bytes, uint32_t count);
int gl_host_fill_u32(void *h_dst, uint32_t word, size_t count);
int gl_host_sparse_to_dense(const gl_idx_val *h_sparse, uint32_t range, uint32_t zero_bits, void *h_dense);
int gl_host_pool_alloc(void **h_ptr, size_t bytes);
int gl_host_pool_free(void *h_ptr);
int gl_pool_trim(void);
int gl_pool_stats(uint64_t *live_blocks, uint64_t *cached_bytes, uint32_t *slabs);

int gl_spmv_plan_create(gl_spmv_plan *plan,
                        uint32_t num_rows, uint32_t num_cols,
                        const uint32_t *h_indptr, const uint32_t *h_indices, const float *h_data,
                        uint32_t row_begin, uint32_t row_end);
#define GL_PLAN_NO_MULADD 1u
#define GL_PLAN_BOOLEAN 2u
#define GL_PLAN_KEEP_VALUES 4u
#define GL_PLAN_HOST_FORMAT 8u
#define GL_PLAN_DEVICE_FORMAT 16u
#define GL_PLAN_REFERENCE_ORDER 32u
int gl_spmv_plan_create_ex(gl_spmv_plan *plan,
                           uint32_t num_rows, uint32_t num_cols,
                           const uint32_t *h_indptr, const uint32_t *h_indices, const float *h_data,
                           uint32_t row_begin, uint32_t row_end, uint32_t flags);
int gl_spmv_plan_destroy(gl_spmv_plan plan);
#define GL_LAYOUT_GENERAL 0
#define GL_LAYOUT_PATTERN 1
#define GL_LAYOUT_BOOLEAN 2
#define GL_LAYOUT_REFERENCE_ORDER 3
#define GL_HELPER_GATHER 0
#define GL_HELPER_SPREAD 1
#define GL_HELPER_SELF_HOT 2
#define GL_HELPER_NONE 3
typedef struct gl_spmv_plan_desc {
    uint64_t nnz, device_bytes, groups, hot_nnz;
    uint32_t num_units, blocks, segments, max_block_rows, hot_columns, packed_columns;
    int layout, mix, helper;
} gl_spmv_plan_desc;
int gl_spmv_plan_describe(gl_spmv_plan plan, gl_spmv_plan_desc *out);
int gl_spmv_plan_values_finite(gl_spmv_plan plan, int *finite);
#define GL_PLAN_ARRAY_ENTRIES 0
#define GL_PLAN_ARRAY_BASES 1
#define GL_PLAN_ARRAY_UNITS 2
#define GL_PLAN_ARRAY_HUB_ROWS 3
#define GL_PLAN_ARRAY_SPANS 4
#define GL_PLAN_ARRAY_HOT 5
#define GL_PLAN_ARRAY_HOT_HDR 6
#define GL_PLAN_ARRAY_PRESENT 7
int gl_spmv_plan_export(gl_spmv_plan plan, int array, void *h_dst, size_t capacity, size_t *bytes);
int gl_spmv_plan_bits_words(gl_spmv_plan plan, uint64_t *words);
int gl_pack_bits(const float *d_x, uint32_t n, uint32_t *d_bits);
int gl_unpack_bits(const uint32_t *d_bits, uint32_t n, float *d_x);
int gl_spmv_run_bits(gl_spmv_plan plan, const uint32_t *d_bits, const float *d_mask, float *d_y, float zero,
                     int mask_type);
int gl_bfs_pull_step(gl_spmv_plan plan, const uint32_t *d_bits_in, uint32_t *d_bits_out, float *d_distance, float level);
int gl_bfs_parents(gl_spmv_plan plan, const float *d_distance, uint32_t *d_parent, uint32_t *d_orphans);
int gl_bfs_parents_entries(gl_spmv_plan plan, const float *d_distance, uint32_t *d_parent, uint64_t *entries_read);
int gl_spmv_plan_rows_sorted(gl_spmv_plan plan, int *sorted);
int gl_cc_begin(uint32_t *d_parent, uint32_t n);
int gl_cc_hook(gl_spmv_plan plan, uint32_t *d_parent);
int gl_cc_finish(uint32_t *d_parent, uint32_t n, uint32_t *d_labels, uint32_t *d_count );
int gl_cc_labels(gl_spmv_plan plan, uint32_t *d_labels, uint32_t *d_count );
int gl_tc_count(gl_spmv_plan plan, uint64_t *d_total, uint64_t *d_per_vertex );
int gl_kcore(gl_spmv_plan plan, uint32_t *d_core, uint32_t *d_order , uint32_t *h_stats );
int gl_bc_accumulate(gl_spmv_plan plan_in, gl_spmv_plan plan_out, const float *d_level, double *d_bc, double scale, int accumulate,
                     double *d_sigma ,
                     uint32_t *h_stats );
int gl_spmv_run(gl_spmv_plan plan, const float *d_x, const float *d_mask, float *d_y,
                int op, float zero, int mask_type);
int gl_spmv_plan_chain(gl_spmv_plan plan, int on, int *active);

int gl_prof_begin(uint32_t max_launches, uint32_t every);
int gl_prof_end(double *total_ms, uint32_t *launches);
int gl_span_begin(void);
int gl_span_end(double *ms);

int gl_spmspv_plan_create(gl_spmspv_plan *plan,
                          uint32_t num_rows, uint32_t num_cols,
                          const uint32_t *h_indptr, const uint32_t *h_indices, const float *h_data,
                          uint32_t row_begin, uint32_t row_end);
int gl_spmspv_plan_destroy(gl_spmspv_plan plan);
int gl_spmspv_plan_info(gl_spmspv_plan plan, uint64_t *nnz, uint64_t *device_bytes);

int gl_spmspv_run(gl_spmspv_plan plan, const gl_idx_val *d_vector, const float *d_mask,
                  gl_idx_val *d_result, int op, float zero, int mask_type);
int gl_spmspv_wait(gl_spmspv_plan plan, uint32_t *nnz);
int gl_spmspv_failed_runs(gl_spmspv_plan plan, uint32_t *count);
int gl_spmspv_run_assign(gl_spmspv_plan plan, const gl_idx_val *d_vector, const float *d_mask,
                         gl_idx_val *d_result, int op, float zero, int mask_type, float *d_inout, float val);
int gl_sssp_parents(gl_spmspv_plan plan, const float *d_distance, float unreached, uint32_t source,
                    uint32_t *d_parent, uint32_t *d_orphans );
int gl_sssp_parents_entries(gl_spmspv_plan plan, const float *d_distance, float unreached, uint32_t source,
                            uint32_t *d_parent, uint64_t *entries_read);

int gl_bfs_bits_begin(uint32_t *d_ctl, uint32_t ctl_words, float *d_distance, uint32_t n, uint32_t *d_bits, uint32_t bits_words,
                      uint32_t nvec, uint32_t first_pull_slot);
#define GL_BFS_TALLY_HEAD_WORDS 64
#define GL_BFS_TALLY_RANK_WORDS 64
#define GL_BFS_TALLY_WORDS(slots, world) (GL_BFS_TALLY_HEAD_WORDS + (size_t)(slots) * (size_t)(world) * GL_BFS_TALLY_RANK_WORDS)
int gl_bfs_bits_shard_step(gl_spmspv_plan csc, gl_spmv_plan rows, const uint32_t *d_bits_in, uint32_t *d_bits_out, uint32_t bits_words,
                           float *d_distance, float level, uint32_t *d_ctl, uint32_t *d_tally, const uint32_t *d_tally_in, uint32_t slot,
                           int rank, int world_size, const uint32_t *d_col_len, uint64_t nnz_global, float threshold,
                           int may_continue_prev, float back_threshold);
int gl_bfs_bits_shard_finish(gl_spmspv_plan csc, gl_spmv_plan rows, uint32_t *d_ctl, uint32_t *d_tally, const uint32_t *d_tally_in,
                             uint32_t last_slot, int rank, int world_size, uint64_t nnz_global, float threshold, int may_continue_last,
                             float back_threshold);
int gl_bfs_bits_begin_from(uint32_t *d_ctl, uint32_t ctl_words, const float *d_x, uint32_t n, uint32_t *d_bits, uint32_t bits_words,
                           const float *d_distance, gl_spmv_plan rows);
int gl_bfs_bits_push_step(gl_spmspv_plan csc, gl_spmv_plan rows, const uint32_t *d_bits_in, uint32_t *d_bits_out, uint32_t *d_bits_spare,
                          uint32_t bits_words, float *d_distance, float level, uint32_t *d_ctl, uint32_t slot, float threshold,
                          int may_continue);
int gl_bfs_bits_pull_step(gl_spmv_plan plan, gl_spmspv_plan csc, const uint32_t *d_bits_in, uint32_t *d_bits_out, float *d_distance,
                          float level, uint32_t *d_ctl, uint32_t slot, float threshold, int may_continue, float back_threshold);
int gl_spmspv_plan_attach_pull(gl_spmspv_plan plan, gl_spmv_plan pull);
int gl_spmspv_plan_hint(gl_spmspv_plan plan, uint32_t vector_nnz_upper_bound);
int gl_spmspv_plan_hint_work(gl_spmspv_plan plan, uint32_t vector_nnz, uint64_t work, uint32_t longest_column);
int gl_spmspv_last_direction(gl_spmspv_plan plan, int *row_wise);

int gl_sparse_nnz(const gl_idx_val *d_sparse, uint32_t *nnz);

int gl_ewise_add(const float *d_in, float *d_out, uint32_t len, float val);

#define GL_PAGERANK_MAX_GROUPS 1024u
#define GL_PAGERANK_MAX_SLOTS 65536u
int gl_pagerank_ctl_bytes(uint32_t slots, size_t *bytes);
int gl_pagerank_begin(const float *d_p, uint32_t n, const uint32_t *d_dangling_bits, float *d_x, void *d_ctl, uint32_t slots);
int gl_pagerank_update(float *d_y_inout, const float *d_x, const float *d_p, const uint32_t *d_dangling_bits, uint32_t n,
                       float damping, double tol, void *d_ctl, uint32_t slot);

int gl_assign_dense(const float *d_mask, float *d_inout, uint32_t len, float val, int mask_type);

// ... 52 lines not shown
```

Before: 6575 GB/s.

## Compact per-block row accumulator tiles to live (nonempty) rows via bitmap rank

Adds a live-row map per block (bitmap plus 16-bit rank) so the accumulator tile in shared memory only holds slots for rows that have entries, plus hub slots. Plan formatting now writes compact slot indices into entries, and the epilogue turns each row into a slot with popcount, using the identity for empty rows. This shrinks the tile, which can raise occupancy or allow larger blocks and hot-column tables. The cost is an extra bitmap/rank load and popcount per row in the epilogue, plus more complex plan building.

Result: no change. 6565 GB/s (-0.1%).

```diff
diff --git a/graphlily_amd/capi.py b/graphlily_amd/capi.py
--- a/graphlily_amd/capi.py
+++ b/graphlily_amd/capi.py
@@ -333,7 +333,8 @@
 GL_PLAN_HOST_FORMAT = 8
 GL_PLAN_DEVICE_FORMAT = 16
 GL_PLAN_REFERENCE_ORDER = 32
-PLAN_ARRAYS = {"entries": 0, "bases": 1, "units": 2, "hub_rows": 3, "spans": 4, "hot": 5, "hot_hdr": 6, "present": 7}
+PLAN_ARRAYS = {"entries": 0, "bases": 1, "units": 2, "hub_rows": 3, "spans": 4, "hot": 5, "hot_hdr": 6, "present": 7,
+               "live_bits": 8, "live_rank": 9}
 GL_ERR_UNSUPPORTED = -5
 
 
diff --git a/graphlily_amd/csrc/gl_format.hip b/graphlily_amd/csrc/gl_format.hip
--- a/graphlily_amd/csrc/gl_format.hip
+++ b/graphlily_amd/csrc/gl_format.hip
@@ -106,8 +106,8 @@
                                                                const uint32_t *__restrict__ data, uint32_t row_begin, uint32_t rows, uint64_t nz0,
                                                                uint32_t num_cols, const uint32_t *__restrict__ bstart, uint32_t nblocks,
                                                                const uint32_t *__restrict__ colmap, const uint32_t *__restrict__ colbits,
-                                                               uint32_t cb, uint32_t bb, K *__restrict__ keys, uint2 *__restrict__ payload,
-                                                               bool drop_hot) {
+                                                               const uint32_t *__restrict__ row_slot, uint32_t cb, uint32_t bb,
+                                                               K *__restrict__ keys, uint2 *__restrict__ payload, bool drop_hot) {
     const uint32_t lane = threadIdx.x & 63u, nwaves = gridDim.x * (kFmtThreads / 64u);
     const K drop = (K)1 << (bb + cb + 1u);
     for (uint32_t row = blockIdx.x * (kFmtThreads / 64u) + (threadIdx.x >> 6); row < rows; row += nwaves) {
@@ -119,7 +119,7 @@
             const uint32_t mid = (lo + hi + 1u) >> 1;
             if (bstart[mid] <= r) lo = mid; else hi = mid - 1u;
         }
-        const uint32_t b = lo, r0 = bstart[b];
+        const uint32_t b = lo, slot = row_slot[row];
         for (uint64_t i = s + lane; i < e; i += 64u) {
             const uint32_t c = indices[i], v = data[i];
             K key;
@@ -131,7 +131,7 @@
                 if (drop_hot && (cm >> 31)) key = drop;
             }
             keys[i] = key;
-            payload[i] = make_uint2(r - r0, v);
+            payload[i] = make_uint2(slot, v);
         }
     }
 }
@@ -154,7 +154,7 @@
     uint32_t cold_begin, cold_end, hot_begin, hot_end;
     uint32_t goff, r0, nrows_direct, hub_off;
     uint32_t nhub, seg, hot_e0, present_off;
-    uint32_t nhot_groups, pad0, pad1, pad2;
+    uint32_t nhot_groups, nlive, pad1, pad2;
 };
 
 template <typename K>
@@ -187,7 +187,7 @@
     constexpr uint32_t G = PATTERN ? kColdGroupsPattern : kColdGroupsGeneral;
     constexpr uint32_t EB = PATTERN ? kColdElemBytesPattern : kColdElemBytesGeneral;
     const UnitDesc u = units[blockIdx.x];
-    const uint32_t nrows = u.nrows_direct & 0xffffu;
+    const uint32_t nrows = u.nlive;
     const K cmask = ((K)1 << cb) - 1;
     if (u.nhub) {
         for (uint32_t i = threadIdx.x; i < nrows; i += kThreads) hub_of[i] = 0xffu;
@@ -266,7 +266,7 @@
     constexpr uint32_t HG = kHotGroupsGeneral;
     constexpr uint32_t EB = kHotElemBytesGeneral;
     const UnitDesc u = units[blockIdx.x];
-    const uint32_t nrows = u.nrows_direct & 0xffffu;
+    const uint32_t nrows = u.nlive;
     const uint32_t lane = threadIdx.x & 63u, wave = threadIdx.x >> 6;
     const K cmask = ((K)1 << cb) - 1;
     if (u.nhub) {
@@ -312,7 +312,7 @@
         }
     }
     if (threadIdx.x == 0)
-        plan_units[3u * blockIdx.x + 2u] = make_uint4(u.hot_e0, u.present_off, m ? runs[u.hot_end - 1u] - s0 + 1u : 0u, 0u);
+        plan_units[3u * blockIdx.x + 2u] = make_uint4(u.hot_e0, u.present_off, m ? runs[u.hot_end - 1u] - s0 + 1u : 0u, u.nlive);
 }
 
 __global__ __launch_bounds__(kFmtThreads) void fmt_hot_row_counts_kernel(const uint32_t *__restrict__ indptr, const uint32_t *__restrict__ indices,
@@ -344,13 +344,13 @@
 __global__ __launch_bounds__(kThreads) void fmt_fill_hot_rows_kernel(const UnitDesc *__restrict__ units, unsigned char *__restrict__ hot, uint32_t nhot_table,
                                                                      uint4 *__restrict__ plan_units) {
     const UnitDesc u = units[blockIdx.x];
-    const uint32_t nrows = u.nrows_direct & 0xffffu, pad0 = nrows + kHubSlots * u.nhub;
+    const uint32_t pad0 = u.nlive + kHubSlots * u.nhub;
     const uint32_t ident = nhot_table | (nhot_table << 16);
     for (uint32_t i = threadIdx.x; i < u.nhot_groups * 64u; i += kThreads) {
         uint4 rec = make_uint4(ident, ident, ident, (nhot_table & 0xffffu) | ((pad0 + (i & 63u)) << 16));
         reinterpret_cast<uint4 *>(hot + (size_t)u.hot_e0 * kHotElemBytesRows)[i] = rec;
     }
-    if (threadIdx.x == 0) plan_units[3u * blockIdx.x + 2u] = make_uint4(u.hot_e0, 0u, nhot_table, 0u);
+    if (threadIdx.x == 0) plan_units[3u * blockIdx.x + 2u] = make_uint4(u.hot_e0, 0u, nhot_table, u.nlive);
 }
 __global__ __launch_bounds__(kFmtThreads) void fmt_emit_hot_rows_kernel(const uint32_t *__restrict__ indptr, const uint32_t *__restrict__ indices,
                                                                         const uint32_t *__restrict__ data, uint32_t row_begin, uint32_t rows,
@@ -360,7 +360,7 @@
                                                                         const unsigned long long *__restrict__ block_start,
                                                                         const uint32_t *__restrict__ seg, const uint32_t *__restrict__ unit_of,
                                                                         const UnitDesc *__restrict__ units, const uint32_t *__restrict__ hub_rows,
-                                                                        unsigned char *__restrict__ hot) {
+                                                                        const uint32_t *__restrict__ row_slot, unsigned char *__restrict__ hot) {
     const uint32_t lane = threadIdx.x & 63u, nwaves = gridDim.x * (kFmtThreads / 64u);
     for (uint32_t row = blockIdx.x * (kFmtThreads / 64u) + (threadIdx.x >> 6); row < rows; row += nwaves) {
         const uint32_t r = row_begin + row;
@@ -372,12 +372,12 @@
             const uint32_t mid = (lo + hi + 1u) >> 1;
             if (bstart[mid] <= r) lo = mid; else hi = mid - 1u;
         }
-        const uint32_t b = lo, row_local = r - bstart[b];
+        const uint32_t b = lo, row_local = row_slot[row];
         const uint64_t M = (uint32_t)block_start[b + 1u] - (uint32_t)block_start[b];
         const uint64_t rec0 = (uint32_t)before - (uint32_t)block_start[b];
         const uint32_t S = seg[b];
         const UnitDesc u0 = units[unit_of[b]];
-        const uint32_t nrows = u0.nrows_direct & 0xffffu;
+        const uint32_t nrows = u0.nlive;
         int hub = -1;
         for (uint32_t k = 0; k < u0.nhub; k++)
             if (hub_rows[u0.hub_off + k] == row_local) hub = (int)k;
@@ -452,8 +452,7 @@
 }
 
 template <typename K>
-int emit_general_typed(DevCsr *c, const EmitGeneral &e, gl_spmv_plan p, std::vector<uint32_t> &hub_count, uint64_t *hot_nnz,
-                       uint32_t cb, uint32_t bb) {
+int emit_general_typed(DevCsr *c, const EmitGeneral &e, gl_spmv_plan p, uint64_t *hot_nnz, uint32_t cb, uint32_t bb) {
     hipStream_t s = ctx().stream;
     const BlockPlan &bp = *e.bp;
     const uint32_t nblocks = bp.nblocks, nunits = bp.nunits;
@@ -463,18 +462,21 @@
     const uint32_t hot_groups = hot_rows ? 1u : kHotGroupsGeneral;
     const uint32_t hot_elem_bytes = hot_rows ? kHotElemBytesRows : kHotElemBytesGeneral;
 
-    DevMem d_bstart, d_colmap, d_keys, d_keys2, d_pl, d_pl2, d_off;
+    DevMem d_bstart, d_colmap, d_keys, d_keys2, d_pl, d_pl2, d_off, d_rowslot;
     int rc;
     if ((rc = d_bstart.alloc((size_t)(nblocks + 1) * 4u)) != GL_OK || (rc = d_colmap.alloc((size_t)e.num_cols * 4u)) != GL_OK ||
+        (rc = d_rowslot.alloc((size_t)rows * 4u)) != GL_OK ||
         (rc = d_keys.alloc(nnz * sizeof(K))) != GL_OK || (rc = d_keys2.alloc(nnz * sizeof(K))) != GL_OK ||
         (rc = d_pl.alloc(nnz * 8u)) != GL_OK || (rc = d_pl2.alloc(nnz * 8u)) != GL_OK ||
         (rc = d_off.alloc((size_t)(2u * nblocks + 1u) * 8u)) != GL_OK)
         return rc;
     GL_HIP(hipMemcpyAsync(d_bstart.p, bp.bstart.data(), (size_t)(nblocks + 1) * 4u, hipMemcpyHostToDevice, s));
     GL_HIP(hipMemcpyAsync(d_colmap.p, e.colmap, (size_t)e.num_cols * 4u, hipMemcpyHostToDevice, s));
+    if (rows) GL_HIP(hipMemcpyAsync(d_rowslot.p, e.live->slot.data(), (size_t)rows * 4u, hipMemcpyHostToDevice, s));
     fmt_keys_kernel<K><<<wave_grid(rows), kFmtThreads, 0, s>>>(c->d_indptr, c->d_indices, c->d_data, c->row_begin, rows, c->nz0, e.num_cols,
                                                                d_bstart.as<uint32_t>(), nblocks, d_colmap.as<uint32_t>(),
-                                                               e.diag_mode ? c->d_colbits : nullptr, cb, bb, d_keys.as<K>(), d_pl.as<uint2>(), hot_rows);
+                                                               e.diag_mode ? c->d_colbits : nullptr, d_rowslot.as<uint32_t>(), cb, bb, d_keys.as<K>(),
+                                                               d_pl.as<uint2>(), hot_rows);
     GL_LAUNCH_CHECK();
     if ((rc = sort_pairs<K>(d_keys.as<K>(), d_keys2.as<K>(), d_pl.as<uint2>(), d_pl2.as<uint2>(), nnz, bb + cb + 2u, s)) != GL_OK) return rc;
     (void)hipFree(d_keys.p); d_keys.p = nullptr;
@@ -487,8 +489,7 @@
     GL_HIP(hipMemcpyAsync(off.data(), d_off.p, off.size() * 8u, hipMemcpyDeviceToHost, s));
     GL_HIP(hipStreamSynchronize(s));
 
-    std::vector<uint32_t> hub_rows((size_t)nblocks * kMaxHubRows, 0u);
-    hub_count.assign(nblocks, 0u);
+    const std::vector<uint32_t> &hub_rows = e.live->hub_rows;
     std::vector<UnitDesc> units(nunits);
     uint64_t hn = 0;
     std::vector<uint64_t> mcs(nblocks), mhs(nblocks), mrec(nblocks, 0);
@@ -526,20 +527,9 @@
         return set_error(GL_ERR_UNSUPPORTED, "plan creation: more than 2^32 - 1 groups in a shard");
     for (uint32_t b = 0; b < nblocks; b++) {
         const uint32_t r0 = bp.bstart[b], r1 = bp.bstart[b + 1];
-        const uint64_t mc = mcs[b], mh = mhs[b], m = mc + mh;
+        const uint64_t mc = mcs[b], mh = mhs[b];
         hn += mh;
-        const uint64_t thr = std::max<uint64_t>(256, m / (uint64_t)e.hub_div);
-        uint32_t nh = 0;
-        for (uint32_t r = r0; r < r1 && nh < kMaxHubRows; r++) {
-            uint64_t cnt = (uint64_t)e.h_indptr[r + 1] - e.h_indptr[r];
-            if (cnt < thr) continue;
-            if (e.diag_mode) {
-                const uint32_t lr = r - c->row_begin;
-                if ((e.diag_has[lr >> 5] >> (lr & 31u)) & 1u) cnt--;
-            }
-            if (cnt >= thr) hub_rows[(size_t)b * kMaxHubRows + nh++] = r - r0;
-        }
-        hub_count[b] = nh;
+        const uint32_t nh = e.live->hub_count[b];
         const uint32_t S = bp.seg[b];
         for (uint32_t sg = 0; sg < S; sg++) {
             UnitDesc &u = units[bp.unit_of[sg][b]];
@@ -557,7 +547,8 @@
             u.hot_e0 = (uint32_t)ul.hot_e0[ui];
             u.present_off = (uint32_t)ul.present_off[ui];
             u.nhot_groups = (uint32_t)(ul.hot_e0[ui + 1] - ul.hot_e0[ui]) * hot_groups;
-            u.pad0 = u.pad1 = u.pad2 = 0u;
+            u.nlive = e.live->nlive[b];
+            u.pad1 = u.pad2 = 0u;
         }
     }
     *hot_nnz = hn;
@@ -637,7 +628,8 @@
                                                                               d_colmap.as<uint32_t>(), e.diag_mode ? c->d_colbits : nullptr,
                                                                               d_bstart.as<uint32_t>(), nblocks, d_rowincl.as<unsigned long long>(),
                                                                               d_blockstart.as<unsigned long long>(), d_seg.as<uint32_t>(),
-                                                                              d_unit_of.as<uint32_t>(), d_units.as<UnitDesc>(), p->d_hub_rows, p->d_hot);
+                                                                              d_unit_of.as<uint32_t>(), d_units.as<UnitDesc>(), p->d_hub_rows,
+                                                                              d_rowslot.as<uint32_t>(), p->d_hot);
             GL_LAUNCH_CHECK();
         }
         GL_HIP(hipStreamSynchronize(s));
@@ -1092,12 +1084,12 @@
     return GL_OK;
 }
 
-int fmt_emit_general(DevCsr *c, const EmitGeneral &e, gl_spmv_plan p, std::vector<uint32_t> &hub_count, uint64_t *hot_nnz) {
+int fmt_emit_general(DevCsr *c, const EmitGeneral &e, gl_spmv_plan p, uint64_t *hot_nnz) {
     const uint32_t cb = bits_for(std::max<uint64_t>(std::max(e.gather_cols, e.nhot_table), 2u));
     const uint32_t bb = bits_for(std::max<uint32_t>(e.bp->nblocks, 2u));
     if (c->nnz >= 0xffffffffull) return set_error(GL_ERR_UNSUPPORTED, "plan creation on the device: more than 2^32 - 1 entries in a shard");
-    if (bb + cb + 2u <= 32u) return emit_general_typed<uint32_t>(c, e, p, hub_count, hot_nnz, cb, bb);
-    return emit_general_typed<unsigned long long>(c, e, p, hub_count, hot_nnz, cb, bb);
+    if (bb + cb + 2u <= 32u) return emit_general_typed<uint32_t>(c, e, p, hot_nnz, cb, bb);
+    return emit_general_typed<unsigned long long>(c, e, p, hot_nnz, cb, bb);
 }
 
 namespace {
diff --git a/graphlily_amd/csrc/gl_spmv.hip b/graphlily_amd/csrc/gl_spmv.hip
--- a/graphlily_amd/csrc/gl_spmv.hip
+++ b/graphlily_amd/csrc/gl_spmv.hip
@@ -12,6 +12,8 @@
     const uint32_t *bases;
     const uint4 *units;
     const uint32_t *hub_rows;
+    const uint32_t *live_bits;
+    const uint16_t *live_rank;
     const float *hot_x;
     uint32_t nhot;
     uint32_t tile_bytes;
@@ -37,8 +39,29 @@
     float *chain_packed = nullptr, *chain_hot = nullptr;
 };
 
+constexpr uint32_t kRowsPerThread = (kMaxPlainRows + kThreads - 1u) / kThreads;
+constexpr uint32_t kNoSlot = 0xffffffffu;
+__device__ __forceinline__ void row_slots_load(const SpmvArgs &a, const uint4 d, const uint4 dh, uint32_t (&lword)[kRowsPerThread],
+                                               uint32_t (&lrk)[kRowsPerThread]) {
+    const uint32_t nrows = d.w & 0xffffu;
+    const uint32_t w0 = live_word0(d.z - a.row_begin, dh.x / kMaxHubRows);
+#pragma unroll
+    for (uint32_t k = 0; k < kRowsPerThread; k++) {
+        const uint32_t wi = w0 + (min(threadIdx.x + k * kThreads, nrows - 1u) >> 5);
+        lword[k] = a.live_bits[wi];
+        lrk[k] = a.live_rank[wi];
+    }
+}
+__device__ __forceinline__ void row_slots(const uint32_t (&lword)[kRowsPerThread], const uint32_t (&lrk)[kRowsPerThread],
+                                          uint32_t (&rslot)[kRowsPerThread]) {
+    const uint32_t bit = threadIdx.x & 31u;
+#pragma unroll
+    for (uint32_t k = 0; k < kRowsPerThread; k++)
+        rslot[k] = ((lword[k] >> bit) & 1u) ? lrk[k] + (uint32_t)__popc(lword[k] & ((1u << bit) - 1u)) : kNoSlot;
+}
 template <int OP, int MASK>
-__device__ __forceinline__ void spmv_unit_epilogue(const SpmvArgs &a, typename Tile<OP>::T *tile, const uint4 d, const uint4 dh) {
+__device__ __forceinline__ void spmv_unit_epilogue(const SpmvArgs &a, typename Tile<OP>::T *tile, const uint4 d, const uint4 dh, uint32_t nlive,
+                                                   const uint32_t (&rslot)[kRowsPerThread]) {
     using TL = Tile<OP>;
     using T = typename TL::T;
     const uint32_t row0 = d.z, nrows = d.w & 0xffffu;
@@ -50,21 +73,26 @@
             const uint32_t r = a.hub_rows[hub_off + threadIdx.x];
             T acc = tile[r];
 #pragma unroll
-            for (uint32_t k = 0; k < kHubSlots; k++) acc = TL::comb(acc, tile[nrows + kHubSlots * threadIdx.x + k]);
+            for (uint32_t k = 0; k < kHubSlots; k++) acc = TL::comb(acc, tile[nlive + kHubSlots * threadIdx.x + k]);
             tile[r] = acc;
         }
         __syncthreads();
     }
+    auto row_acc = [&](uint32_t slot) -> T { return slot == kNoSlot ? TL::ident() : tile[slot]; };
 
     if (direct) {
-        for (uint32_t i = threadIdx.x; i < nrows; i += kThreads) {
+#pragma unroll
+        for (uint32_t k = 0; k < kRowsPerThread; k++) {
+            const uint32_t i = threadIdx.x + k * kThreads;
+            if (i >= nrows) break;
             const uint32_t row = row0 + i;
+            T acc = row_acc(rslot[k]);
             if (a.diag_has) {
                 const uint32_t lr = row - a.row_begin;
                 if ((a.diag_has[lr >> 5] >> (lr & 31u)) & 1u)
-                    tile[i] = TL::comb(tile[i], TL::lift(Semiring<OP>::mul(a.diag[lr], a.x[row])));
+                    acc = TL::comb(acc, TL::lift(Semiring<OP>::mul(a.diag[lr], a.x[row])));
             }
-            float out = TL::finish(a.zero, TL::get(tile, i));
+            float out = TL::finish(a.zero, TL::get(&acc, 0u));
             if (MASK != GL_NOMASK) {
                 if (!mask_allows_zero<MASK, OP>(a.mask[row])) out = 0.0f;
             }
@@ -80,7 +108,13 @@
         }
     } else {
         float *plane = a.partials + (size_t)dh.w * a.prow + (row0 - a.row_begin);
-        for (uint32_t i = threadIdx.x; i < nrows; i += kThreads) plane[i] = TL::get(tile, i);
+#pragma unroll
+        for (uint32_t k = 0; k < kRowsPerThread; k++) {
+            const uint32_t i = threadIdx.x + k * kThreads;
+            if (i >= nrows) break;
+            const T acc = row_acc(rslot[k]);
+            plane[i] = TL::get(&acc, 0u);
+        }
     }
 }
 
@@ -437,26 +471,50 @@
     const uint32_t unit = __builtin_amdgcn_readfirstlane(blockIdx.x);
     const uint4 d = load_const(a.units + 3u * unit), dh = load_const(a.units + 3u * unit + 1u);
     const uint4 dp = load_const(a.units + 3u * unit + 2u);
-    const uint32_t g0 = d.x, ncold = d.y, nrows = d.w & 0xffffu;
+    const uint32_t g0 = d.x, ncold = d.y, nlive = dp.w;
     const uint32_t nhub = dh.y, nhotg = dh.z;
-    const uint32_t nslots = nrows + kHubSlots * nhub;
+    const uint32_t nslots = nlive + kHubSlots * nhub;
     const uint32_t lane = threadIdx.x & 63u;
     const uint32_t wave = __builtin_amdgcn_readfirstlane(threadIdx.x >> 6);
 
     uint32_t &next_iter = *reinterpret_cast<uint32_t *>(lds_raw + a.tile_bytes + (size_t)a.nhot * 4u);
     if (threadIdx.x == 0) next_iter = kWaves;
+    uint32_t lword[kRowsPerThread], lrk[kRowsPerThread], rslot[kRowsPerThread];
+    row_slots_load(a, d, dh, lword, lrk);
     if (UH > 0 && LY::kHotRows) {
-        for (uint32_t i = threadIdx.x; i < dp.z; i += kThreads) hot_x[i] = a.hot_x[i];
+        const uint32_t n4 = dp.z >> 2;
+        const float4 *src4 = reinterpret_cast<const float4 *>(a.hot_x);
+        float4 *dst4 = reinterpret_cast<float4 *>(hot_x);
+        for (uint32_t i0 = threadIdx.x; i0 < n4; i0 += 4u * kThreads) {
+            float4 v[4];
+#pragma unroll
+            for (uint32_t k = 0; k < 4u; k++) v[k] = src4[min(i0 + k * kThreads, n4 - 1u)];
+#pragma unroll
+            for (uint32_t k = 0; k < 4u; k++)
+                if (i0 + k * kThreads < n4) dst4[i0 + k * kThreads] = v[k];
+        }
         if (threadIdx.x < 64u) hot_x[dp.z + threadIdx.x] = TL::zident();
     } else if (UH > 0) {
         const uint16_t *pres = a.present + dp.y;
-        if (a.self_hot_cols) {
-            for (uint32_t i = threadIdx.x; i < dp.z; i += kThreads) hot_x[i] = a.x[a.self_hot_cols[pres[i]]];
-        } else {
-            for (uint32_t i = threadIdx.x; i < dp.z; i += kThreads) hot_x[i] = a.hot_x[pres[i]];
+        const float *src = a.self_hot_cols ? a.x : a.hot_x;
+        for (uint32_t i0 = threadIdx.x; i0 < dp.z; i0 += 8u * kThreads) {
+            uint32_t s[8];
+            float v[8];
+#pragma unroll
+            for (uint32_t k = 0; k < 8u; k++) s[k] = pres[min(i0 + k * kThreads, dp.z - 1u)];
+            if (a.self_hot_cols) {
+#pragma unroll
+                for (uint32_t k = 0; k < 8u; k++) s[k] = a.self_hot_cols[s[k]];
+            }
+#pragma unroll
+            for (uint32_t k = 0; k < 8u; k++) v[k] = src[s[k]];
+#pragma unroll
+            for (uint32_t k = 0; k < 8u; k++)
+                if (i0 + k * kThreads < dp.z) hot_x[i0 + k * kThreads] = v[k];
         }
     }
     for (uint32_t i = threadIdx.x; i < nslots + kPadSlots; i += kThreads) tile[i] = TL::ident();
+    row_slots(lword, lrk, rslot);
     __syncthreads();
 
     const float *xsrc = LY::kValues ? a.xg : a.z;
@@ -470,7 +528,7 @@
     it = spmv_phase<OP, L, UC, UH>(a, tile, hot_x, xsrc, sg, lane, it, n_both, &next_iter);
     if (rc > rh) it = spmv_phase<OP, L, UC, 0>(a, tile, hot_x, xsrc, sg, lane, it, n_all, &next_iter);
     else if (UH > 0) it = spmv_phase<OP, L, 0, UH>(a, tile, hot_x, xsrc, sg, lane, it, n_all, &next_iter);
-    spmv_unit_epilogue<OP, MASK>(a, tile, d, dh);
+    spmv_unit_epilogue<OP, MASK>(a, tile, d, dh, nlive, rslot);
 #if defined(GL_UNIT_CLOCKS)
     asm volatile("s_waitcnt vmcnt(0)" ::: "memory");
     __syncthreads();
@@ -972,6 +1030,8 @@
     a.bases = p->d_bases;
     a.units = p->d_units;
     a.hub_rows = p->d_hub_rows;
+    a.live_bits = p->d_live_bits;
+    a.live_rank = p->d_live_rank;
     a.hot_x = p->d_hot_x;
     a.nhot = p->nhot_lds;
     a.hot = p->d_hot;
diff --git a/graphlily_amd/csrc/gl_spmv_plan.cpp b/graphlily_amd/csrc/gl_spmv_plan.cpp
--- a/graphlily_amd/csrc/gl_spmv_plan.cpp
+++ b/graphlily_amd/csrc/gl_spmv_plan.cpp
@@ -144,6 +144,46 @@
     return bp;
 }
 
+LiveRows live_rows(const BlockPlan &bp, const uint32_t *h_indptr, uint32_t row_begin, uint32_t row_end, const uint32_t *diag_has,
+                   uint32_t hub_div) {
+    LiveRows lv;
+    const uint32_t nblocks = bp.nblocks;
+    lv.slot.assign(row_end - row_begin, 0u);
+    lv.nlive.assign(nblocks, 0u);
+    lv.hub_rows.assign((size_t)nblocks * kMaxHubRows, 0u);
+    lv.hub_count.assign(nblocks, 0u);
+    const size_t words = ((size_t)live_word0(row_end - row_begin, nblocks) + 2u) / 2u * 2u;
+    lv.bits.assign(words, 0u);
+    lv.rank.assign(words, 0);
+    auto dropped = [&](uint32_t r) -> uint32_t {
+        const uint32_t lr = r - row_begin;
+        return diag_has ? (diag_has[lr >> 5] >> (lr & 31u)) & 1u : 0u;
+    };
+    for (uint32_t b = 0; b < nblocks; b++) {
+        const uint32_t r0 = bp.bstart[b], r1 = bp.bstart[b + 1], w0 = live_word0(r0 - row_begin, b);
+        uint64_t m = (uint64_t)h_indptr[r1] - h_indptr[r0];
+        uint32_t n = 0;
+        for (uint32_t r = r0; r < r1; r++) {
+            const uint32_t i = r - r0;
+            if ((i & 31u) == 0u) lv.rank[w0 + (i >> 5)] = (uint16_t)n;
+            lv.slot[r - row_begin] = n;
+            m -= dropped(r);
+            if (h_indptr[r + 1] > h_indptr[r]) {
+                lv.bits[w0 + (i >> 5)] |= 1u << (i & 31u);
+                n++;
+            }
+        }
+        lv.nlive[b] = n;
+        const uint64_t thr = std::max<uint64_t>(256, m / (uint64_t)hub_div);
+        uint32_t nh = 0;
+        for (uint32_t r = r0; r < r1 && nh < kMaxHubRows; r++)
+            if ((uint64_t)h_indptr[r + 1] - h_indptr[r] - dropped(r) >= thr) lv.hub_rows[(size_t)b * kMaxHubRows + nh++] = lv.slot[r - row_begin];
+        lv.hub_count[b] = nh;
+        lv.max_slots = std::max(lv.max_slots, n + kHubSlots * nh);
+    }
+    return lv;
+}
+
 struct PlanDeleter {
     void operator()(gl_spmv_plan p) const { gl_spmv_plan_destroy(p); }
 };
@@ -248,11 +288,11 @@
     return GL_OK;
 }
 
-static void choose_hot_columns(const Knobs &k, uint32_t flags, uint64_t nnz, const std::vector<uint32_t> &deg, uint32_t tallest,
+static void choose_hot_columns(const Knobs &k, uint32_t flags, uint64_t nnz, const std::vector<uint32_t> &deg, uint32_t tile_slots,
                                uint32_t nblocks, bool pattern, std::vector<uint32_t> &hot_cols, std::vector<uint32_t> &colmap) {
     const uint32_t num_cols = (uint32_t)deg.size();
     const size_t elem = (flags & (GL_PLAN_NO_MULADD | GL_PLAN_BOOLEAN)) ? sizeof(float) : sizeof(double);
-    const size_t tile_bytes = ((size_t)tallest + kHubSlots * kMaxHubRows + kPadSlots) * elem;
+    const size_t tile_bytes = ((size_t)tile_slots + kPadSlots) * elem;
     uint32_t room = 0;
     if (tile_bytes + 4096u <= kLdsBudget)
         room = std::min<uint32_t>(1u << 15, (uint32_t)((kLdsBudget - tile_bytes - 320u) / 4u / 64u * 64u));
@@ -306,10 +346,13 @@
     }
 }
 
-static int emit_general_host(const HostCsr &a, const EmitGeneral &eg, gl_spmv_plan p, std::vector<uint32_t> &hub_count, uint64_t *hot_nnz_out) {
+static int emit_general_host(const HostCsr &a, const EmitGeneral &eg, gl_spmv_plan p, uint64_t *hot_nnz_out) {
     const uint32_t *h_indptr = a.indptr, *h_indices = a.indices, *colmap = eg.colmap, *colbits = eg.colbits;
     const float *h_data = a.data;
     const BlockPlan &bp = *eg.bp;
+    const LiveRows &lv = *eg.live;
+    const std::vector<uint32_t> &hub_rows = lv.hub_rows, &hub_count = lv.hub_count;
+    const uint32_t *row_slot = lv.slot.data();
     const std::vector<uint32_t> &bstart = bp.bstart, &seg = bp.seg;
     const std::vector<std::vector<uint32_t>> &unit_of = bp.unit_of;
     const uint32_t nblocks = bp.nblocks, nunits = bp.nunits, gather_cols = eg.gather_cols, nhot_table = eg.nhot_table;
@@ -345,7 +388,6 @@
     std::vector<unsigned char> entries((size_t)(total_groups / cold_groups + 1) * cold_elem_bytes, 0);
     std::vector<uint32_t> bases(total_groups, 0u);
     std::vector<uint4> units((size_t)nunits * 3);
-    std::vector<uint32_t> hub_rows((size_t)nblocks * kMaxHubRows, 0);
     std::vector<unsigned char> hot_bytes((size_t)(hot_elems + 1) * hot_elem_bytes, 0);
     {
         uint16_t *rows16 = reinterpret_cast<uint16_t *>(hot_bytes.data() + (size_t)hot_elems * hot_elem_bytes);
@@ -369,33 +411,20 @@
                     const uint32_t c = h_indices[i];
                     const uint32_t v = __builtin_bit_cast(uint32_t, h_data[i]);
                     if (diag_mode && c == r && v != colbits[c]) continue;
-                    if (colmap[c] >> 31) hot.push_back(Rec{colmap[c] & 0x7fffffffu, r - r0, v});
-                    else recs.push_back(Rec{colmap[c], r - r0, v});
+                    if (colmap[c] >> 31) hot.push_back(Rec{colmap[c] & 0x7fffffffu, row_slot[r - a.row_begin], v});
+                    else recs.push_back(Rec{colmap[c], row_slot[r - a.row_begin], v});
                 }
             sort_by_col(recs, tmp, gather_cols);
             if (!hot_rows) sort_by_col(hot, tmp, nhot_table ? nhot_table : 1u);
             hot_nnz += hot.size();
-            const uint64_t mcb = recs.size(), m = mcb + hot.size();
-            std::vector<uint32_t> cnt(r1 - r0, 0);
-            for (const Rec &rc : recs) cnt[rc.row_local]++;
-            for (const Rec &rc : hot) cnt[rc.row_local]++;
-            std::vector<int> hub_of(r1 - r0, -1);
-            {
-                const uint64_t thr = std::max<uint64_t>(256, m / (uint64_t)eg.hub_div);
-                uint32_t nh = 0;
-                for (uint32_t i = 0; i < r1 - r0 && nh < kMaxHubRows; i++)
-                    if (cnt[i] >= thr) {
-                        hub_of[i] = (int)nh;
-                        hub_rows[(size_t)b * kMaxHubRows + nh] = i;
-                        nh++;
-                    }
-                hub_count[b] = nh;
-            }
-            const uint32_t nrows_b = r1 - r0;
-            const uint32_t pad_slot = nrows_b + kHubSlots * hub_count[b];
+            const uint64_t mcb = recs.size();
+            const uint32_t nlive_b = lv.nlive[b];
+            std::vector<int> hub_of(nlive_b, -1);
+            for (uint32_t h = 0; h < hub_count[b]; h++) hub_of[hub_rows[(size_t)b * kMaxHubRows + h]] = (int)h;
+            const uint32_t pad_slot = nlive_b + kHubSlots * hub_count[b];
             auto slot_of = [&](const Rec &rc, uint32_t fill) -> uint32_t {
                 const int hb = hub_of[rc.row_local];
-                return hb < 0 ? rc.row_local : nrows_b + kHubSlots * (uint32_t)hb + (fill & (kHubSlots - 1u));
+                return hb < 0 ? rc.row_local : nlive_b + kHubSlots * (uint32_t)hb + (fill & (kHubSlots - 1u));
             };
             const uint32_t S = seg[b];
             for (uint32_t s = 0; s < S; s++) {
@@ -465,7 +494,7 @@
                     }
                     units[3 * u] = make_uint4((uint32_t)goff, ncold, r0, (r1 - r0) | (all_direct ? 0x80000000u : 0u));
                     units[3 * u + 1] = make_uint4((uint32_t)((size_t)b * kMaxHubRows), hub_count[b], nel, s);
-                    units[3 * u + 2] = make_uint4((uint32_t)e0, 0u, nhot_table, 0u);
+                    units[3 * u + 2] = make_uint4((uint32_t)e0, 0u, nhot_table, nlive_b);
                     continue;
                 }
                 const uint64_t h0 = hot.size() * s / S, h1 = hot.size() * (s + 1) / S, e0 = ul.hot_e0[u];
@@ -497,7 +526,7 @@
                 const uint32_t nhotg = (uint32_t)(ul.hot_e0[u + 1] - e0) * hot_groups;
                 units[3 * u] = make_uint4((uint32_t)goff, ncold, r0, (r1 - r0) | (all_direct ? 0x80000000u : 0u));
                 units[3 * u + 1] = make_uint4((uint32_t)((size_t)b * kMaxHubRows), hub_count[b], nhotg, s);
-                units[3 * u + 2] = make_uint4((uint32_t)e0, (uint32_t)ul.present_off[u], np, 0u);
+                units[3 * u + 2] = make_uint4((uint32_t)e0, (uint32_t)ul.present_off[u], np, nlive_b);
             }
         }
     }
@@ -624,6 +653,9 @@
         diag_mode = p->pattern && exceptions > 0;
     }
 
+    const LiveRows live = live_rows(bp, a.indptr, a.row_begin, a.row_end, diag_mode ? diag_has.data() : nullptr,
+                                    (uint32_t)std::max<long>(1, k.hub_div));
+
     std::vector<uint32_t> deg, hot_cols, ccols, colmap(num_cols);
     for (uint32_t c = 0; c < num_cols; c++) colmap[c] = c;
     if (nnz > 0) {
@@ -631,7 +663,8 @@
         rc = on_device ? fmt_column_degrees(staged.c, num_cols, deg, &bad) : column_degrees_host(a, deg, &bad);
         if (rc != GL_OK) return rc;
         if (bad) return column_error(num_cols);
-        if (k.hot != 0) choose_hot_columns(k, p->flags, nnz, deg, p->max_plain_rows, bp.nblocks, p->pattern, hot_cols, colmap);
+        const uint32_t sized_by = p->pattern ? live.max_slots : p->max_plain_rows + kHubSlots * kMaxHubRows;
+        if (k.hot != 0) choose_hot_columns(k, p->flags, nnz, deg, sized_by, bp.nblocks, p->pattern, hot_cols, colmap);
     }
     const uint32_t nhot_table = (uint32_t)((hot_cols.size() + 63) / 64 * 64);
     if (nhot_table) hot_cols.resize(nhot_table, hot_cols[0]);
@@ -649,18 +682,21 @@
     eg.diag_mode = diag_mode, eg.colbits = colbits.data(), eg.diag_has = diag_has.data();
     eg.pattern = p->pattern;
     eg.group_mult = p->pattern ? kColdGroupsPattern : kColdGroupsGeneral;
-    eg.hub_div = (uint32_t)std::max<long>(1, k.hub_div);
     eg.h_indptr = a.indptr, eg.num_cols = num_cols;
-    std::vector<uint32_t> hub_count(bp.nblocks, 0);
+    eg.live = &live;
     uint64_t hot_nnz = 0;
-    rc = on_device ? fmt_emit_general(staged.c, eg, p, hub_count, &hot_nnz) : emit_general_host(a, eg, p, hub_count, &hot_nnz);
+    rc = on_device ? fmt_emit_general(staged.c, eg, p, &hot_nnz) : emit_general_host(a, eg, p, &hot_nnz);
     if (rc != GL_OK) return rc;
+    if ((rc = plan_upload(p, p->d_live_bits, live.bits.data(), live.bits.size() * sizeof(uint32_t))) != GL_OK ||
+        (rc = plan_upload(p, p->d_live_rank, live.rank.data(), live.rank.size() * sizeof(uint16_t))) != GL_OK)
+        return rc;
+    p->b_live_bits = live.bits.size() * sizeof(uint32_t);
+    p->b_live_rank = live.rank.size() * sizeof(uint16_t);
 
     p->nblocks = bp.nblocks;
     p->segments = bp.Smax;
     p->nunits = bp.nunits;
-    for (uint32_t b = 0; b < bp.nblocks; b++)
-        p->max_block_rows = std::max(p->max_block_rows, bp.bstart[b + 1] - bp.bstart[b] + kHubSlots * hub_count[b]);
+    p->max_block_rows = live.max_slots;
     p->nhot = nhot_table;
     p->hot_nnz = hot_nnz;
     p->ncompact = compact ? gather_cols : 0u;
@@ -728,6 +764,8 @@
     (void)hipFree(p->d_bases);
     (void)hipFree(p->d_units);
     (void)hipFree(p->d_hub_rows);
+    (void)hipFree(p->d_live_bits);
+    (void)hipFree(p->d_live_rank);
     (void)hipFree(p->d_hot);
     (void)hipFree(p->d_hot_hdr);
     (void)hipFree(p->d_present);
@@ -806,6 +844,8 @@
         case GL_PLAN_ARRAY_HOT: src = p->d_hot, n = p->b_hot; break;
         case GL_PLAN_ARRAY_HOT_HDR: src = p->d_hot_hdr, n = p->b_hot_hdr; break;
         case GL_PLAN_ARRAY_PRESENT: src = p->d_present, n = p->b_present; break;
+        case GL_PLAN_ARRAY_LIVE_BITS: src = p->d_live_bits, n = p->b_live_bits; break;
+        case GL_PLAN_ARRAY_LIVE_RANK: src = p->d_live_rank, n = p->b_live_rank; break;
         default: return gl::set_error(GL_ERR_INVALID_ARG, "gl_spmv_plan_export: unknown array %d", array);
     }
     *bytes = n;
diff --git a/graphlily_amd/csrc/gl_spmv_plan.h b/graphlily_amd/csrc/gl_spmv_plan.h
--- a/graphlily_amd/csrc/gl_spmv_plan.h
+++ b/graphlily_amd/csrc/gl_spmv_plan.h
@@ -82,6 +82,19 @@
 
 BlockPlan plan_blocks(Shape shape, const uint32_t *h_indptr, uint32_t row_begin, uint32_t row_end, uint32_t max_rows,
                       uint32_t align = 1);
+
+struct LiveRows {
+    std::vector<uint32_t> slot;
+    std::vector<uint32_t> nlive;
+    std::vector<uint32_t> bits;
+    std::vector<uint16_t> rank;
+    std::vector<uint32_t> hub_rows;
+    std::vector<uint32_t> hub_count;
+    uint32_t max_slots = 0;
+};
+__host__ __device__ inline uint32_t live_word0(uint32_t local_row0, uint32_t block) { return local_row0 / 32u + block; }
+LiveRows live_rows(const BlockPlan &bp, const uint32_t *h_indptr, uint32_t row_begin, uint32_t row_end, const uint32_t *diag_has,
+                   uint32_t hub_div);
 
 struct UnitLayout {
     std::vector<uint64_t> cold_goff;
@@ -130,7 +143,8 @@
 struct gl_spmv_plan_s {
     uint32_t num_rows = 0, num_cols = 0, row_begin = 0, row_end = 0;
     uint64_t nnz = 0;
-    uint32_t nunits = 0, nblocks = 0, segments = 1, max_block_rows = 0;
+    uint32_t nunits = 0, nblocks = 0, segments = 1;
+    uint32_t max_block_rows = 0;
     uint64_t ngroups = 0;
     uint2 *d_entries = nullptr;
     uint32_t *d_bases = nullptr;
@@ -141,6 +155,8 @@
     uint32_t nhot_lds = 0;
     uint64_t nhot_elems = 0;
     uint32_t *d_hub_rows = nullptr;
+    uint32_t *d_live_bits = nullptr;
+    uint16_t *d_live_rank = nullptr;
     uint32_t flags = 0;
     uint32_t nhot = 0;
     uint64_t hot_nnz = 0;
@@ -201,7 +217,7 @@
     float *d_csr_data = nullptr;
     uint64_t device_bytes = 0;
     size_t b_entries = 0, b_bases = 0, b_units = 0, b_hub_rows = 0, b_spans = 0;
-    size_t b_hot = 0, b_hot_hdr = 0, b_present = 0;
+    size_t b_hot = 0, b_hot_hdr = 0, b_present = 0, b_live_bits = 0, b_live_rank = 0;
 };
 
 namespace gl {
@@ -246,11 +262,11 @@
     const uint32_t *diag_has;
     bool pattern;
     uint32_t group_mult;
-    uint32_t hub_div;
     const uint32_t *h_indptr;
     uint32_t num_cols;
-};
-int fmt_emit_general(DevCsr *c, const EmitGeneral &e, gl_spmv_plan p, std::vector<uint32_t> &hub_count, uint64_t *hot_nnz);
+    const LiveRows *live;
+};
+int fmt_emit_general(DevCsr *c, const EmitGeneral &e, gl_spmv_plan p, uint64_t *hot_nnz);
 struct EmitBool {
     const BlockPlan *bp;
     const uint32_t *h_indptr;
diff --git a/include/graphlily_hip.h b/include/graphlily_hip.h
--- a/include/graphlily_hip.h
+++ b/include/graphlily_hip.h
@@ -106,6 +106,8 @@
 #define GL_PLAN_ARRAY_HOT 5
 #define GL_PLAN_ARRAY_HOT_HDR 6
 #define GL_PLAN_ARRAY_PRESENT 7
+#define GL_PLAN_ARRAY_LIVE_BITS 8
+#define GL_PLAN_ARRAY_LIVE_RANK 9
 int gl_spmv_plan_export(gl_spmv_plan plan, int array, void *h_dst, size_t capacity, size_t *bytes);
 int gl_spmv_plan_bits_words(gl_spmv_plan plan, uint64_t *words);
 int gl_pack_bits(const float *d_x, uint32_t n, uint32_t *d_bits);
```
